# engcang/FAST-LIO-SAM-QN

Hardware: AMD Instinct MI355X
Metric: scan-pair registrations/sec on 100k-pt clouds (higher is better)
Workload: dtype f32 search / f64 accumulate

## Files before the change

fast-lio-sam-qn_amd/csrc/qn_batch.inc:

```

namespace {

template <class F> void lanes_launch(const void* tab, dim3 grid, hipStream_t s, uint32_t shmem) {
  hipLaunchKernelGGL(HIP_KERNEL_NAME(k_lanes<F>), grid, dim3(F::TB), shmem, s, (const LaneEntry<typename F::Args>*)tab);
}
template <class A> void lane_push(std::vector<LaneEntry<A>>& v, const A& a, uint32_t nbx) {
  LaneEntry<A> e; memset((void*)&e, 0, sizeof(e)); e.a = a; e.nbx = nbx; v.push_back(e);
}

struct LanePlan {
  qn_ctx* c; size_t off = 0; bool overflow = false; int flush_rc = QN_OK;
  struct Item { void (*fn)(const void*, dim3, hipStream_t, uint32_t); size_t off; dim3 grid; int family; uint32_t shmem; };
  std::vector<Item> items;
  explicit LanePlan(qn_ctx* c_) : c(c_) {}
  template <class F> void add(const std::vector<LaneEntry<typename F::Args>>& e, int family, uint32_t shmem = 0) {
    if (e.empty()) return;
    const size_t bytes = sizeof(LaneEntry<typename F::Args>) * e.size();
    const size_t a = reserve(bytes);
    if (a == SIZE_MAX) return;
    put<F>(e, a, family, shmem);
  }
  template <class F, class Fix> void add(std::vector<LaneEntry<typename F::Args>>& e, int family, const void* blob, size_t blob_bytes, Fix fix) {
    if (e.empty()) return;
    const size_t head = (blob_bytes + 255) & ~(size_t)255, bytes = head + sizeof(LaneEntry<typename F::Args>) * e.size();
// ... 53 lines not shown

int lane_set_cloud(qn_ctx* c, int which, const float* xyz, uint32_t n, uint32_t stride, bool on_device, hipStream_t s, GridLaunch* out) {
  CloudBuf& b = c->cloud[which];
  b.n = 0; b.has_grid = b.has_cov = false;
  if (n == 0) return QN_ERR_EMPTY_CLOUD;
  if (!xyz || stride < 12 || (stride & 3)) return QN_ERR_INVALID_ARG;
  if (n > c->max_points) return QN_ERR_CAPACITY;
  const char* dsrc = (const char*)xyz;
  if (!on_device) { const int rc = upload_host_cloud(c, xyz, n, stride, s, &dsrc); if (rc != QN_OK) return rc; }
  b.n = n;
  *out = prep_grid(c, b, dsrc, stride, true);
  return QN_OK;
}

bool batch_supported(const qn_ctx* c) {
  const qn_gicp_params& p = c->params;
  const int maxit = p.force_iterations > 0 ? p.force_iterations : p.max_iterations;
  return c->batch_lanes >= 2 && !c->lanes_failed && maxit > 0 && c->fused_ticks && c->fused_final && c->far_enabled && c->knn_hist && !c->verify_track && !c->clk_probe && !c->list_probe &&
         c->tick_tb == 512 && c->tick_occ >= 4 && !c->dbg_counters;
}

int lane_args_arena(qn_ctx* c) {
  if (c->args_h) return QN_OK;
  c->args_cap = (size_t)4 << 20;
  HIPCHK(c, hipHostMalloc(&c->args_h, c->args_cap, hipHostMallocDefault));
  HIPCHK(c, hipMalloc(&c->args_d, c->args_cap));
  return QN_OK;
}

int batch_ensure_lanes(qn_ctx* c) {
  HIPCHK(c, hipSetDevice(c->device));
  const int B = std::max(1, std::min(c->batch_lanes, 64));
  if (c->lanes.empty()) c->lanes.push_back(c);
  while ((int)c->lanes.size() < B) {
    qn_ctx* l = nullptr;
    const int rc = (c->fail_lane_create > 0 && (int)c->lanes.size() >= c->fail_lane_create) ? QN_ERR_HIP : ctx_create(c->device, c->max_points, c->stream, &l);
    if (rc != QN_OK) {
      c->last_error = "batch: lane context creation failed (lanes need batch_lanes x the context's device memory)";
      while (c->lanes.size() > 1) { qn_ctx_destroy(c->lanes.back()); c->lanes.pop_back(); }
      (void)hipGetLastError();
      c->lanes_failed = true;
      return rc;
    }
    c->lanes.push_back(l);
  }
  { const int rc = lane_args_arena(c); if (rc != QN_OK) return rc; }
  for (qn_ctx* l : c->lanes) {
    if (l == c) continue;
    if (l->params.k_correspondences != c->params.k_correspondences) l->cloud[0].has_cov = l->cloud[1].has_cov = false;
    l->params = c->params;
    l->cell_override = c->cell_override; l->margin_nn = c->margin_nn; l->margin_nn_t0 = c->margin_nn_t0; l->margin_knn = c->margin_knn; l->big_blocks0 = c->big_blocks0; l->fb_blocks0 = c->fb_blocks0;
    l->big_ratio = c->big_ratio; l->nn_rounds = c->nn_rounds; l->knn_rounds = c->knn_rounds; l->knn_trips = c->knn_trips; l->knn_mm = c->knn_mm; l->knn_single_all = c->knn_single_all; l->bbox_blocks = c->bbox_blocks; l->stable_cells = c->stable_cells;
    l->unseeded_cap = c->unseeded_cap; l->track_from_tick = c->track_from_tick; l->fused_from_tick = c->fused_from_tick; l->ticks_per_chunk = c->ticks_per_chunk; l->far_chunk = c->far_chunk; l->far_group = c->far_group; l->far_ranked = c->far_ranked;
    l->list_small = c->list_small; l->tick_ppt_min = c->tick_ppt_min; l->tick_rpb = c->tick_rpb; l->nn_lane = c->nn_lane;
  }
  return QN_OK;
}

int batch_register(qn_ctx* owner, const qn_pair_desc* pairs, const uint32_t* idx, uint32_t m, double thr, qn_gicp_result* results, int* valid, int* status,
                   std::vector<const float*>& last_src, std::vector<uint64_t>& last_key, const float* guesses16) {
  hipStream_t s = owner->stream;
  const auto t_call = std::chrono::steady_clock::now();
  const qn_gicp_params& p = owner->params;
  const int k = p.k_correspondences;
  LanePlan plan(owner);
  std::vector<LaneRun> L(m);
  struct AliasGuard {
    std::vector<LaneRun>& L; std::vector<CloudBuf> saved; std::vector<double*> saved_nrm; std::vector<const float*>& last_src;
    AliasGuard(std::vector<LaneRun>& L_, std::vector<const float*>& ls) : L(L_), saved(L_.size()), saved_nrm(L_.size(), nullptr), last_src(ls) {}
    void borrow(size_t l, qn_ctx* from) { qn_ctx* c = L[l].c; saved[l] = c->cloud[0]; saved_nrm[l] = c->nrm_s_sorted; c->cloud[0] = from->cloud[0]; c->nrm_s_sorted = from->nrm_s_sorted; }
    ~AliasGuard() { for (size_t l = 0; l < L.size(); l++) if (L[l].alias >= 0 && saved_nrm[l]) { qn_ctx* c = L[l].c; c->cloud[0] = saved[l]; c->nrm_s_sorted = saved_nrm[l]; c->cloud[0].has_grid = c->cloud[0].has_cov = false; c->cloud[0].n = 0; c->cloud[0].knn_tab = nullptr; last_src[l] = nullptr; } }
  } alias_guard(L, last_src);
  struct FailGuard { std::vector<LaneRun>& L; int* status; bool armed = true; ~FailGuard() { if (armed) for (const LaneRun& R : L) if (R.active) status[R.pair] = QN_ERR_HIP; } } fail_guard{L, status};
  std::vector<LaneEntry<PackBBoxK::Args>> v_pack; std::vector<LaneEntry<CellCountK::Args>> v_count; std::vector<LaneEntry<ScanLookbackK::Args>> v_scan;
  std::vector<LaneEntry<ScatterK::Args>> v_scat; std::vector<LaneEntry<StableCellsK::Args>> v_stab;
  std::vector<LaneEntry<KnnHistArgs>> v_sel, v_lst; std::vector<LaneEntry<KnnSingleK::Args>> v_single; std::vector<LaneEntry<KnnCovArgs>> v_tail; std::vector<LaneEntry<CovFromIdxK::Args>> v_cov;
  auto push_grid = [&](const GridLaunch& G) {
    lane_push(v_pack, G.pack, G.pack_nb); lane_push(v_count, G.count, G.nb); lane_push(v_scan, G.scan, G.scan_nb); lane_push(v_scat, G.scat, G.nb);
    if (G.stable) lane_push(v_stab, G.stab, G.nb);
  };
  auto push_knn = [&](const KnnLaunch& K) {
    lane_push(v_sel, K.sel, K.sel_nb); lane_push(v_lst, K.lst, K.lst_nb); lane_push(v_single, K.single, K.single_nb); lane_push(v_tail, K.tail, K.tail_nb); lane_push(v_cov, K.cov, K.cov_nb);
  };
  for (uint32_t l = 0; l < m; l++) {
    LaneRun& R = L[l]; R.c = owner->lanes[l]; R.pair = idx[l];
    qn_ctx* c = R.c;
    const qn_pair_desc& pd = pairs[R.pair];
    qn_gicp_result* out = &results[R.pair];
    valid[R.pair] = 0; memset(out, 0, sizeof(*out)); out->fitness = DBL_MAX;
    for (int i = 0; i < 4; i++) { out->T[5 * i] = 1.f; out->T64[5 * i] = 1.0; }
    c->pair_pipeline = false; c->persist_batch_off = true; c->tgt_pending = false; c->tgt_on_stream2 = false;
    const uint64_t key = ((uint64_t)pd.ns << 32) ^ ((uint64_t)pd.stride_bytes << 1) ^ (uint64_t)(pd.on_device ? 1 : 0);
    R.build_source = !(owner->batch_share_source && last_src[l] == pd.src && last_key[l] == key && pd.src != nullptr && c->cloud[0].has_grid && c->cloud[0].has_cov && c->cloud[0].n == pd.ns);
    if (R.build_source && owner->batch_share_source && pd.src != nullptr && pd.ns > 0) {
      for (uint32_t j = 0; j < l; j++) {
        const qn_pair_desc& pj = pairs[L[j].pair];
        if (L[j].active && L[j].alias < 0 && pj.src == pd.src && pj.ns == pd.ns && pj.stride_bytes == pd.stride_bytes && pj.on_device == pd.on_device) { R.alias = (int)j; break; }
      }
      if (R.alias >= 0) { alias_guard.borrow(l, L[R.alias].c); R.build_source = false; }
    }
    int rc = QN_OK; GridLaunch gs, gt;
    if (R.build_source) { last_src[l] = nullptr; rc = lane_set_cloud(c, QN_SOURCE, pd.src, pd.ns, pd.stride_bytes, pd.on_device != 0, s, &gs); }
    if (rc == QN_OK) { ScratchSwap sw(c); rc = lane_set_cloud(c, QN_TARGET, pd.dst, pd.nt, pd.stride_bytes, pd.on_device != 0, s, &gt); }
    if (rc == QN_ERR_HIP) return rc;
    status[R.pair] = rc;
    if (rc != QN_OK) {
      if (R.build_source) { c->cloud[0].has_grid = c->cloud[0].has_cov = false; c->cloud[0].n = 0; }
// ... 14 lines not shown
    else { plan.add<KnnHistK<false, 48, false>>(v_sel, QN_K_KNN_SELECT); plan.add<KnnHistK<true, 48, false>>(v_lst, QN_K_KNN_COV); }
  }
  plan.add<KnnSingleK>(v_single, QN_K_KNN_COV);
  if (k <= 16) plan.add<KnnCovK<16, true, 4>>(v_tail, QN_K_KNN_COV); else if (k <= 20) plan.add<KnnCovK<20, true, 4>>(v_tail, QN_K_KNN_COV); else if (k <= 24) plan.add<KnnCovK<24, true, 4>>(v_tail, QN_K_KNN_COV); else plan.add<KnnCovK<32, true, 4>>(v_tail, QN_K_KNN_COV);
  plan.add<CovFromIdxK>(v_cov, QN_K_KNN_COV);

  const int per_outer = p.optimizer == QN_OPT_LM ? 2 : 1;
  const int maxit = p.force_iterations > 0 ? p.force_iterations : p.max_iterations;
  const int fixed_unseeded = std::max(1, std::min(owner->track_from_tick, owner->fused_from_tick)) * per_outer;
  const bool exact_ticks = p.force_iterations > 0 && p.optimizer == QN_OPT_GN;
  {
    std::vector<LaneEntry<InitStateK::Args>> v_init; std::vector<float> g16;
    for (LaneRun& R : L) {
      if (!R.active) continue;
      qn_ctx* c = R.c;
      c->gen = 0; c->part_rows = 0; c->far_mode = 2; c->clear_far_now = true; c->unseeded_until = fixed_unseeded; c->count_far_now = false;
      c->result_host->phase = 0;
      R.ticks_left = exact_ticks ? maxit : 1 << 30;
      R.chunk = std::min(fixed_unseeded, R.ticks_left); R.chunk_start = 0; R.next = R.chunk; R.first_chunk = true;
      R.budget = (long)maxit * (p.optimizer == QN_OPT_LM ? (p.lm_max_iterations + 1) : 1) + 2;
      lane_push(v_init, InitStateK::Args{st_cur(c), c->guess_tmp, guesses16 ? 1 : 0, 0, c->far_stats}, 1u);
      if (guesses16) g16.insert(g16.end(), guesses16 + 16 * (size_t)R.pair, guesses16 + 16 * (size_t)R.pair + 16);
    }
    if (!guesses16) plan.add<InitStateK>(v_init, QN_K_SOLVE);
    else
      plan.add<InitStateK>(v_init, QN_K_SOLVE, g16.data(), sizeof(float) * g16.size(), [](std::vector<LaneEntry<InitStateK::Args>>& e, const char* d) {
        for (size_t j = 0; j < e.size(); j++) e[j].a.guess = (const float*)(d + sizeof(float) * 16 * j);
      });
  }
  auto finish_lane = [&](LaneRun& R, int rc) {
    qn_ctx* c = R.c;
    R.active = false;
    status[R.pair] = rc;
    if (rc != QN_OK) return;
    results[R.pair] = c->result_host->r;
    c->trace_len = c->result_host->trace_len; c->aligned_valid = true;
    valid[R.pair] = (results[R.pair].converged && results[R.pair].fitness < thr) ? 1 : 0;
  };
  struct ProfFlush { qn_ctx* c; ~ProfFlush() { c->prof_collect(); } } prof_flush{owner};
  int tick_no = 0;
  for (;;) {
    int stop = 1 << 30; bool any = false;
    for (const LaneRun& R : L) if (R.active) { any = true; stop = std::min(stop, R.next); }
    if (!any) break;
    for (; tick_no < stop; tick_no++) {
      {
        std::vector<LaneEntry<NnSearchArgs>> v_g, v_l; std::vector<LaneEntry<AccumulateK::Args>> v_acc;
        bool group = true, lane = true;
        for (LaneRun& R : L) {
          if (!R.active || tick_no >= R.c->unseeded_until) continue;
          qn_ctx* c = R.c;
          const int t = tick_no - R.chunk_start;
          c->count_far_now = R.first_chunk && (t / per_outer == (R.chunk - 1) / per_outer);
          const NnLaunch N = prep_nn(c, 0, c->sqd, false, tick_no / per_outer, 0);
          group = group && N.group; lane = lane && N.lane;
          lane_push(v_g, N.grid, N.grid_nb); lane_push(v_l, N.list, N.list_nb);
          const uint32_t nb = acc_blocks(c);
          lane_push(v_acc, prep_accumulate(c, 0, true), nb);
          c->count_far_now = false;
        }
        if (lane) plan.add<NnLaneK<0>>(v_g, QN_K_NN_SEARCH); else plan.add<NnSearchK<0, false, QN_NN_BLOCK>>(v_g, QN_K_NN_SEARCH);
        if (group) plan.add<NnSearchK<0, true, QN_BLOCK, true>>(v_l, QN_K_NN_FALLBACK); else plan.add<NnSearchK<0, true, QN_BLOCK>>(v_l, QN_K_NN_FALLBACK);
        plan.add<AccumulateK>(v_acc, QN_K_ACCUMULATE);
      }
      {
        std::vector<LaneEntry<TickArgs>> v_t; std::vector<LaneEntry<FarArgs>> v_f; std::vector<LaneEntry<FarReduceK::Args>> v_r;
        for (LaneRun& R : L) {
          if (!R.active || tick_no < R.c->unseeded_until) continue;
          qn_ctx* c = R.c;
          const TickArgs a = tick_args(c);
          lane_push(v_t, a, tick_blocks(c));
          if (a.far_mode == 1) { lane_push(v_f, far_args(c), (uint32_t)QN_FAR_BLOCKS); lane_push(v_r, far_reduce_args(c), 1u); }
          c->gen++; c->part_rows = -1;
        }
        plan.add<TickK<512, 4, 0, false>>(v_t, QN_K_GN_TICK_FUSED, (uint32_t)owner->tick_lds_pad); plan.add<FarK>(v_f, QN_K_FAR); plan.add<FarReduceK>(v_r, QN_K_FAR);
      }
    }
    {
      std::vector<LaneEntry<FinalizeK::Args>> v_fin; std::vector<LaneEntry<TickArgs>> v_close; std::vector<LaneEntry<FinalizeFitK::Args>> v_fit;
      for (LaneRun& R : L) {
        if (!R.active || R.next != stop) continue;
        qn_ctx* c = R.c;
        if (exact_ticks && R.ticks_left > R.chunk) lane_push(v_fin, FinalizeK::Args{st_cur(c), c->result_host, c->far_stats}, 1u);
        else {
          const TickArgs a = tick_args(c, 1);
          const uint32_t nb = tick_blocks(c);
          lane_push(v_close, a, nb);
          lane_push(v_fit, FinalizeFitK::Args{st_cur(c), c->result_host, c->far_stats, c->fit_psum, c->fit_pcnt, (int)tick_rows(c)}, 1u);
        }
      }
      plan.add<FinalizeK>(v_fin, QN_K_SOLVE); plan.add<TickK<512, 4, 1, false>>(v_close, QN_K_FITNESS); plan.add<FinalizeFitK>(v_fit, QN_K_FITNESS);
    }
    const auto tt0 = std::chrono::steady_clock::now();
    int rc = plan.run();
    if (rc != QN_OK) return rc;
    const auto tt1 = std::chrono::steady_clock::now();
    HIPCHK(owner, hipStreamSynchronize(s));
    if (owner->batch_trace) { const auto tt2 = std::chrono::steady_clock::now();
      fprintf(stderr, "qn batch %p: segment to tick %d  prep+enqueue %.0f us  sync %.0f us  (since call %.0f us)\n", (void*)owner, stop, std::chrono::duration<double, std::micro>(tt1 - tt0).count(),
              std::chrono::duration<double, std::micro>(tt2 - tt1).count(), std::chrono::duration<double, std::micro>(tt2 - t_call).count()); }
    for (LaneRun& R : L) {
      if (!R.active || R.next != stop) continue;
      qn_ctx* c = R.c;
      if (R.first_chunk && (rc = clouds_valid(c)) != QN_OK) { last_src[&R - &L[0]] = nullptr; finish_lane(R, rc); continue; }
      R.budget -= std::max(R.chunk, 1); R.ticks_left -= R.chunk;
      if (c->result_host->phase == 2) { finish_lane(R, QN_OK); continue; }
      if (R.budget <= 0) { c->last_error = "align: device state machine did not terminate"; owner->last_error = c->last_error; finish_lane(R, QN_ERR_HIP); continue; }
// ... 60 lines not shown
```

fast-lio-sam-qn_amd/csrc/qn_context.h:

```cpp
#pragma once
#include <hip/hip_runtime.h>
#include <string>
#include <vector>
#include "qn_gicp_kernels.cuh"

struct CloudBuf {
  uint32_t n = 0, ncells = 0;
  bool has_grid = false, has_cov = false;
  float4* raw = nullptr;
  float4* sorted = nullptr;
  float4* sorted_tmp = nullptr;
  uint32_t* cell_of_pt = nullptr;
  uint32_t* cell_start = nullptr;
  uint32_t* counts = nullptr;
  double* nrm = nullptr;
  qn::GridView grid{};
  qn::GridDims* dims = nullptr;
  qn::GridDims* dims_host = nullptr;
  const int32_t* knn_tab = nullptr; int knn_k = 0;
};

struct ProfSpan { int family; hipEvent_t a, b; int count; };

struct qn_ctx {
  int device = 0;
  uint32_t max_points = 0, max_cells = 0;
  hipStream_t stream = nullptr; bool owns_stream = true;
  std::vector<qn_ctx*> lanes; int batch_lanes = 8; char* args_h = nullptr; char* args_d = nullptr; size_t args_cap = 0; uint64_t batch_launches = 0, batch_pairs = 0; bool is_lane = false, batch_trace = false, batch_share_source = true;
  bool lanes_failed = false; int fail_lane_create = 0;
  void* slab = nullptr;
  qn_gicp_params params{};
  CloudBuf cloud[2];
  qn::BBoxAcc* bbox_acc = nullptr; qn::BBoxAcc* bbox_acc2 = nullptr;
  unsigned long long* scan_status = nullptr; unsigned long long* scan_status2 = nullptr; uint32_t build_epoch = 0;
  int far_group = -1;
  int far_chunk = 2;
  bool batch_look = false;
  bool far_ranked = true;
  unsigned long long* list_probe = nullptr;
  bool device_look = true;
  bool clear_far_now = false;
  char* staging2 = nullptr;
  struct PinZone { char* h = nullptr; hipEvent_t ev = nullptr; bool busy = false; } pin_up, pin_up2;
  char* staging = nullptr;
  uint32_t* scan_sums = nullptr;

  qn::GicpState* state = nullptr;
  uint32_t gen = 0; int part_rows = 0;
  double* partials = nullptr;
  uint32_t* tail_ticket = nullptr;
  double* fit_psum = nullptr; uint32_t* fit_pcnt = nullptr;
  qn_iter_trace* trace = nullptr; uint32_t trace_len = 0;
  int32_t* corr = nullptr; int32_t* nn_idx = nullptr; int32_t* knn_idx = nullptr; float4* nn_ref = nullptr; double* nrm_s_sorted = nullptr; qn::TargetRec* tgt_rec = nullptr; float* sqd = nullptr; float* sqd_fit = nullptr;
  int32_t* far_cand = nullptr; float4* far_cand_ref = nullptr; float2* far_cand_b = nullptr; unsigned long long* far_req = nullptr; uint32_t* far_stats = nullptr; double* far_rows = nullptr; int far_mode = 2; bool far_enabled = true;
  uint2* fb_list = nullptr; uint2* big_list = nullptr; uint32_t* fb_count2 = nullptr;
  float4* aligned = nullptr; bool aligned_valid = false;
  double* pose_tmp = nullptr; float* guess_tmp = nullptr;
  qn::ResultBlock* result_host = nullptr; double* scalar_host = nullptr;
  int32_t* dbg_knn_idx = nullptr; float* dbg_knn_d2 = nullptr;
  qn_quatro_params qparams{}; bool qparams_set = false, q_ready = false; double q_last_scale = 1.0;
  float4* q_normals[2] = {nullptr, nullptr}; float* q_spfh[2] = {nullptr, nullptr}; float* q_fpfh_s[2] = {nullptr, nullptr}; float* q_fpfh[2] = {nullptr, nullptr};
  unsigned long long* q_key[2] = {nullptr, nullptr};
  float* q_pair[2] = {nullptr, nullptr}; uint32_t* q_pair_hash[2] = {nullptr, nullptr};
  uint32_t* q_hit = nullptr; uint32_t* q_list = nullptr; uint32_t* q_sel = nullptr; uint2* q_pairs = nullptr; uint32_t* q_counts = nullptr; double* q_T = nullptr;
  void* q_mm_c = nullptr; void* q_mm_q = nullptr; float* q_mm_qn = nullptr; uint32_t* q_mm_L = nullptr; unsigned long long* q_mm_table = nullptr; unsigned long long* q_mm_table_q = nullptr; bool feat_query_dedupe = false;
  uint32_t q_mm_mask = 0;
  uint2* q_mm_pairs = nullptr; uint32_t* q_mm_cnt = nullptr; uint32_t q_mm_cap = 0, q_mm_ncnt = 0; bool feat_mfma = true, feat_mm_retry = false; int feat_sample = 4 ; bool feat_verify = false; int feat_min_blocks = 1536; double q_wall_ms[3] = {0, 0, 0}; unsigned long long* q_mm_vkeys = nullptr; uint32_t* q_mm_vcnt = nullptr; uint32_t feat_fallbacks = 0, feat_survivors = 0;
  bool c2f_overlap = false;
  bool c2f_lanes_fpfh = false;
  bool tgt_early = true;
  bool quatro_fused = true;
  int normals_fg = 0, fpfh_fg = 0;
  float4* c2f_src = nullptr; float4* c2f_dst = nullptr;
  float* q_mean = nullptr; double* q_mean_psum = nullptr; void* q_host = nullptr;
  double cell_override = 0.0;
  int list_small = 6000;
  float big_ratio = 2.5f;
  bool fused_ticks = true;
  int nn_rounds = 1;
  int nn_lane = -1;
  int track_from_tick = 3;
  int fused_from_tick = 3;
  int unseeded_until = 3; bool count_far_now = false; int last_extra_unseeded = 0;
  int unseeded_cap = 10;
  int single_from_tick = 2;
  bool fused_final = true;
  int knn_rounds = 2;
  int knn_mm = 1;
  int knn_trips = 3;
  int knn_hist = 1;
  int big_blocks0 = 4096, fb_blocks0 = 512;
  float margin_nn_t0 = 0.f;
  float margin_nn = 1.f, margin_knn = 0.f;
  int margin_nn_cap = 3, margin_knn_cap = 5, ticks_per_chunk = 8; bool knn_single_all = false, stable_cells = true; int bbox_blocks = 64;
  hipStream_t stream2 = nullptr; hipEvent_t ev_pair = nullptr; bool pair_pipeline = true, pair_failed = false, tgt_on_stream2 = false, tgt_pending = false, no_pipe = false;
  uint32_t* scan_sums2 = nullptr; uint2* fb_list2 = nullptr; uint2* big_list2 = nullptr; uint32_t* fb_count2b = nullptr; int32_t* knn_idx2 = nullptr;
  uint32_t tick_ppt_min = 1;
  uint32_t tick_rpb = 2;
  uint32_t tick_tb = 512;
  int batch_min_share = 4;
  int knn_lds_pad = 0;
  int tick_lds_pad = 0;
  int tick_occ = 4;
  unsigned long long* pg_rows = nullptr; unsigned long long* pg_bc = nullptr; unsigned long long* pg_fit = nullptr; uint32_t* pg_status = nullptr; uint32_t* pg_status_host = nullptr;
  unsigned long long* pg_clk = nullptr; uint32_t pg_epoch = 0; bool prof_persist = false, persist = true, persist_batch_off = false, persist_fits = true; int persist_resident_blocks = 0; uint32_t persist_launches = 0, persist_gave_up = 0; unsigned long long persist_timeout = 25000000ull;
  uint32_t* dbg_counters = nullptr;
  unsigned long long* clk_probe = nullptr; uint32_t clk_n = 0;
  bool verify_track = false; int32_t* v_corr = nullptr; int32_t* v_nn_idx = nullptr; float* v_sqd = nullptr; float4* v_nn_ref = nullptr; uint32_t* v_counters = nullptr;
  bool prof_on = false, prof_open = false; int prof_depth = 0;
  std::vector<ProfSpan> spans;
  qn_kernel_stat stats[QN_K_COUNT] = {};
  std::string last_error;

  void set_error(const char* what, hipError_t e, int line);
  void prof_begin(int family, int count = 1); void prof_end(); void prof_collect();
  int quatro_normals_width() const { const int g = normals_fg > 0 ? normals_fg : 8; return g >= 16 ? 16 : (g >= 8 ? 8 : 1); }
  int quatro_fpfh_width() const { const int g = fpfh_fg > 0 ? fpfh_fg : 8; return g >= 16 ? 16 : 8; }
};
```

fast-lio-sam-qn_amd/csrc/qn_device.cuh:

```cuda
#pragma once
#include <hip/hip_runtime.h>
#include <stdint.h>
#include "qn_eig3.cuh"
#include "qn_step_math.cuh"

namespace qn {

#define QN_TX 8
#define QN_TY 4
#define QN_TZ 4
#define QN_TILE_CELLS 128

struct GridDims {
  float ox, oy, oz, cell, inv_cell, eps;
  int nx, ny, nz, ntx, nty, ntz;
  uint32_t n;
  uint32_t ncells, nonfinite, pad;
};
struct GridView {
  const float4* pts;
  const uint32_t* cell_start;
  uint32_t* dbg;
  float ox, oy, oz, cell, inv_cell, eps;
  int nx, ny, nz;
  int ntx, nty, ntz;
  uint32_t n;
  const GridDims* dims;
};
__device__ __forceinline__ int uni(int v) { return __builtin_amdgcn_readfirstlane(v); }
__device__ __forceinline__ uint32_t uni(uint32_t v) { return (uint32_t)__builtin_amdgcn_readfirstlane((int)v); }
__device__ __forceinline__ float uni(float v) { return __int_as_float(__builtin_amdgcn_readfirstlane(__float_as_int(v))); }
__device__ __forceinline__ double uni(double v) { union { double d; int i[2]; } u; u.d = v; u.i[0] = __builtin_amdgcn_readfirstlane(u.i[0]); u.i[1] = __builtin_amdgcn_readfirstlane(u.i[1]); return u.d; }
__device__ __forceinline__ GridView grid_resolve(GridView g) {
  const GridDims d = *g.dims;
  g.ox = uni(d.ox); g.oy = uni(d.oy); g.oz = uni(d.oz); g.cell = uni(d.cell); g.inv_cell = uni(d.inv_cell); g.eps = uni(d.eps);
  g.nx = uni(d.nx); g.ny = uni(d.ny); g.nz = uni(d.nz); g.ntx = uni(d.ntx); g.nty = uni(d.nty); g.ntz = uni(d.ntz); g.n = uni(d.n);
  return g;
}

template <class A> struct alignas(16) LaneEntry { A a; uint32_t nbx; uint32_t pad_[3]; };
template <class F>
__global__ void __launch_bounds__(F::TB, F::OCC) k_lanes(const LaneEntry<typename F::Args>* __restrict__ tab) {
  const LaneEntry<typename F::Args>* e = tab + blockIdx.y;
  const uint32_t nbx = e->nbx;
  if (blockIdx.x >= nbx) return;
  F::run(e->a, blockIdx.x, nbx);
}

#define QN_INF_KEY 0xFFFFFFFFFFFFFFFFull

__device__ __forceinline__ int clampi(int v, int lo, int hi) { return v < lo ? lo : (v > hi ? hi : v); }
__device__ __forceinline__ int cell_coord(float v, float o, float inv, int n) {
  return clampi((int)floorf((v - o) * inv), 0, n - 1);
}
__device__ __forceinline__ uint32_t cell_key(const GridView& g, int x, int y, int z) {
  const uint32_t tile = ((uint32_t)(z >> 2) * g.nty + (y >> 2)) * g.ntx + (x >> 3);
  return (tile << 7) | ((z & 3) << 5) | ((y & 3) << 3) | (x & 7);
}
__device__ __forceinline__ unsigned long long pack_key(float d2, uint32_t idx) {
  return ((unsigned long long)__float_as_uint(d2) << 32) | idx;
}
__device__ __forceinline__ float key_d2(unsigned long long k) { return __uint_as_float((uint32_t)(k >> 32)); }
__device__ __forceinline__ uint32_t key_idx(unsigned long long k) { return (uint32_t)k; }

typedef float qn_f2 __attribute__((ext_vector_type(2)));
__device__ __forceinline__ float sqdist(float qx, float qy, float qz, float px, float py, float pz) {
  const qn_f2 q = {qx, qy}, p = {px, py};
  const qn_f2 d = q - p;
  const qn_f2 d2 = d * d;
  const float dz = qz - pz;
  return (d2.x + d2.y) + dz * dz;
}

__device__ __forceinline__ int rfl(int v) { return __builtin_amdgcn_readfirstlane(v); }
__device__ __forceinline__ uint32_t rflu(uint32_t v) { return (uint32_t)__builtin_amdgcn_readfirstlane((int)v); }
// ... 227 lines not shown
  __device__ __forceinline__ void consider(bool on, float d2, uint32_t idx) {
    const unsigned long long key = pack_key(d2, idx);
    if (on && key < w) { pend[cnt][threadIdx.x & 63] = key; cnt++; }
    if (__any(cnt == QN_PEND_CAP)) flush();
  }
  __device__ __forceinline__ void merge_from(int lane_xor, bool recv) {
    if (KMAX > 24) {
      unsigned long long tmp[KMAX];
#pragma unroll
      for (int j = 0; j < KMAX; j++) tmp[j] = __shfl_xor(a[j], lane_xor);
#pragma unroll 1
      for (int j = 0; j < KMAX; j++) {
        unsigned long long other = QN_INF_KEY;
#pragma unroll
        for (int u = 0; u < KMAX; u++) other = (u == j) ? tmp[u] : other;
        if (__any(j >= KMAX - k)) insert((recv && j >= KMAX - k) ? other : QN_INF_KEY);
      }
      return;
    }
#pragma unroll
    for (int j = 0; j < KMAX; j++) {
      const unsigned long long other = __shfl_xor(a[j], lane_xor);
      if (__any(j >= KMAX - k)) insert((recv && j >= KMAX - k) ? other : QN_INF_KEY);
    }
  }
  template <int S>
  __device__ __forceinline__ void finish(bool on) {
    if (__any(cnt > 0)) flush();
    if (S == 1) return;
    const int lane = threadIdx.x & 63;
    merge_from(32, on && (lane & 32) == 0);
    if (S == 4) merge_from(16, on && (lane & 48) == 0);
    refresh();
    const unsigned long long w0 = __shfl(w, lane & (64 / S - 1));
    if (on) w = w0;
  }
  __device__ __forceinline__ bool full() const { return w != QN_INF_KEY; }
  __device__ __forceinline__ float worst_d2() const { return key_d2(w); }
  __device__ __forceinline__ int found() const {
    int f = 0;
#pragma unroll
    for (int j = 0; j < KMAX; j++) f += (j >= KMAX - k && a[j] != QN_INF_KEY) ? 1 : 0;
    return f;
  }
  __device__ __forceinline__ int wanted() const { return k; }
};

__device__ __forceinline__ float tile_box_d2(const GridView& g, int tx, int ty, int tz, float qx, float qy, float qz) {
  const float xl = g.ox + (float)(tx << 3) * g.cell, xh = g.ox + (float)min((tx << 3) + 8, g.nx) * g.cell;
  const float yl = g.oy + (float)(ty << 2) * g.cell, yh = g.oy + (float)min((ty << 2) + 4, g.ny) * g.cell;
  const float zl = g.oz + (float)(tz << 2) * g.cell, zh = g.oz + (float)min((tz << 2) + 4, g.nz) * g.cell;
  const float dx = fmaxf(fmaxf(xl - qx, qx - xh) - g.eps, 0.f), dy = fmaxf(fmaxf(yl - qy, qy - yh) - g.eps, 0.f), dz = fmaxf(fmaxf(zl - qz, qz - zh) - g.eps, 0.f);
  return ((dx * dx + dy * dy) + dz * dz) * 0.999998f;
}

__device__ __forceinline__ void divmod_small(int n, int d, int& q, int& r) {
  q = (int)((float)n * __builtin_amdgcn_rcpf((float)d));
  r = n - q * d;
  if (r < 0) { q--; r += d; }
  if (r >= d) { q++; r -= d; }
}

template <class Body>
__device__ __forceinline__ uint32_t stream_box(const GridView& g, int x0, int x1, int y0, int y1, int z0, int z1, const bool tile_mode, WaveLds* lds, Body&& body,
                                               const float bqx = 0.f, const float bqy = 0.f, const float bqz = 0.f, const float ball_r2 = -1.f) {
  const int lane = threadIdx.x & 63;
  const int tx0 = x0 >> 3, ntr = (x1 >> 3) - tx0 + 1, nyr = y1 - y0 + 1;
  const int ty0 = y0 >> 2, ntyr = (y1 >> 2) - ty0 + 1;
  const int nseg = tile_mode ? ntr * ntyr * ((z1 >> 2) - (z0 >> 2) + 1) : ntr * nyr * (z1 - z0 + 1);
  uint32_t grand = 0;
  for (int sb = 0; sb < nseg; sb += 64) {
    const int sidx = sb + lane;
    uint32_t s = 0, len = 0;
    if (sidx < nseg) {
      int t, r; divmod_small(sidx, ntr, r, t);
      if (tile_mode) {
        int qz_, ry_; divmod_small(r, ntyr, qz_, ry_);
        const int tzz = (z0 >> 2) + qz_, tyy = ty0 + ry_, txx = tx0 + t;
        const uint32_t tile = ((uint32_t)tzz * g.nty + tyy) * g.ntx + txx;
        if (!(ball_r2 >= 0.f && tile_box_d2(g, txx, tyy, tzz, bqx, bqy, bqz) > ball_r2)) { s = g.cell_start[tile << 7]; len = g.cell_start[(tile + 1) << 7] - s; }
      } else {
        int qz_, ry_; divmod_small(r, nyr, qz_, ry_);
        const int ry = y0 + ry_, rz = z0 + qz_, tx = tx0 + t;
        const int xa = max(x0, tx << 3), xb = min(x1, (tx << 3) + 7);
        const uint32_t k0 = cell_key(g, xa, ry, rz);
        s = g.cell_start[k0]; len = g.cell_start[k0 + (xb - xa) + 1] - s;
      }
    }
    const uint32_t incl = wave_incl_scan_u32(len, lane);
    const uint32_t total = rdlane(incl, 63);
    if (total == 0) continue;
    wave_lds_fence();
    lds->seg_excl[lane] = incl - len; lds->seg_start[lane] = s;
    wave_lds_fence();
    for (uint32_t cb = 0; cb < total; cb += 64) {
      const uint32_t slot = cb + lane;
      const bool valid = slot < total;
      const int j = chunk_segment(lds->tile_cid, cb, incl - len, incl);
      float4 p = make_float4(0.f, 0.f, 0.f, 0.f);
      if (valid) p = g.pts[lds->seg_start[j] + (slot - lds->seg_excl[j])];
      body(p, valid, min(64u, total - cb));
    }
    grand += total;
  }
  return grand;
}

#define QN_CL_DX 8
#define QN_CL_DY 4
#define QN_CL_DZ 4

template <int S>
__device__ __forceinline__ void build_clusters(const GridView& g, WaveLds* lds, unsigned long long todo, int cx, int cy, int cz,
                                               float qx, float qy, float qz, float r, uint32_t& cid, int& ncl, uint32_t& nseg_all) {
  const int lane = threadIdx.x & 63;
  const bool mine = (todo >> lane) & 1ull;
  cid = 0xffffffffu; ncl = 0;
  for (unsigned long long rem = todo; rem != 0; ncl++) {
    const int leader = __ffsll((long long)rem) - 1;
    const int ax = rdlane(cx, leader), ay = rdlane(cy, leader), az = rdlane(cz, leader);
    const bool in = ((rem >> lane) & 1ull) && abs(cx - ax) <= QN_CL_DX && abs(cy - ay) <= QN_CL_DY && abs(cz - az) <= QN_CL_DZ;
    if (in) cid = ncl;
    rem &= ~__ballot(in);
  }
  wave_lds_fence();
  if (lane < ncl) { lds->box[lane][0] = 0x3fffffff; lds->box[lane][1] = -1; lds->box[lane][2] = 0x3fffffff; lds->box[lane][3] = -1; lds->box[lane][4] = 0x3fffffff; lds->box[lane][5] = -1; }
  wave_lds_fence();
  if (mine && lane < 64 / S) {
    atomicMin(&lds->box[cid][0], cell_coord(qx - r, g.ox, g.inv_cell, g.nx)); atomicMax(&lds->box[cid][1], cell_coord(qx + r, g.ox, g.inv_cell, g.nx));
    atomicMin(&lds->box[cid][2], cell_coord(qy - r, g.oy, g.inv_cell, g.ny)); atomicMax(&lds->box[cid][3], cell_coord(qy + r, g.oy, g.inv_cell, g.ny));
    atomicMin(&lds->box[cid][4], cell_coord(qz - r, g.oz, g.inv_cell, g.nz)); atomicMax(&lds->box[cid][5], cell_coord(qz + r, g.oz, g.inv_cell, g.nz));
  }
  wave_lds_fence();
// ... 112 lines not shown
      const int* b = lds->box[cid];
      const int ex0 = b[0], ex1 = b[1], ey0 = b[2], ey1 = b[3], ez0 = b[4], ez1 = b[5];
      const float INF = __int_as_float(0x7f800000);
      float d = INF;
      if (ex0 > 0) d = fminf(d, qx - (g.ox + ex0 * g.cell));
      if (ex1 < g.nx - 1) d = fminf(d, (g.ox + (ex1 + 1) * g.cell) - qx);
      if (ey0 > 0) d = fminf(d, qy - (g.oy + ey0 * g.cell));
      if (ey1 < g.ny - 1) d = fminf(d, (g.oy + (ey1 + 1) * g.cell) - qy);
      if (ez0 > 0) d = fminf(d, qz - (g.oz + ez0 * g.cell));
      if (ez1 < g.nz - 1) d = fminf(d, (g.oz + (ez1 + 1) * g.cell) - qz);
      if (d == INF || !(r == r)) { certified = true; d_unseen = INF; }
      else { d -= g.eps; d_unseen = d; certified = d > 0.f && sink.full() && sink.worst_d2() < d * d; }
      if (!certified) {
        if (sink.full()) r = fmaxf(sqrtf(sink.worst_d2()) * 1.000001f + g.eps, r + g.eps);
        else {
          const int f = sink.found();
          r = f > 0 ? fmaxf(r * sqrtf((float)sink.wanted() / (float)f) * 1.25f, r + g.cell) : 2.f * r + g.cell;
        }
        r = fminf(r, r_cap);
        if (round + 1 < max_rounds) { retry = true; sink.reset(); }
      }
    }
    todo = __ballot(retry);
    if (g.dbg && lane == 0 && todo) atomicAdd(&g.dbg[3], (uint32_t)__popcll(todo));
  }
  return certified;
}

struct CapBox {
  float o2[3];
  float S;
};
__device__ __forceinline__ CapBox cap_of(const GridView& g, float qx, float qy, float qz) {
  CapBox c;
  const float ox = fmaxf(fmaxf(g.ox - qx, qx - (g.ox + g.nx * g.cell)), 0.f);
  const float oy = fmaxf(fmaxf(g.oy - qy, qy - (g.oy + g.ny * g.cell)), 0.f);
  const float oz = fmaxf(fmaxf(g.oz - qz, qz - (g.oz + g.nz * g.cell)), 0.f);
  c.o2[0] = ox * ox; c.o2[1] = oy * oy; c.o2[2] = oz * oz; c.S = (c.o2[0] + c.o2[1]) + c.o2[2];
  return c;
}
__device__ __forceinline__ float cap_extent(const GridView& g, const CapBox& c, float r, int axis) {
  const float rest = c.S - c.o2[axis];
  if (rest <= 0.f) return r;
  const float v = r * r - rest * 0.999999f;
  return v > 0.f ? sqrtf(v) * 1.000001f + g.eps : g.eps;
}
__device__ __forceinline__ float cap_face_dist(const CapBox& c, float f, int axis) {
  const float rest = (c.S - c.o2[axis]) * 0.999999f;
  return rest > 0.f ? sqrtf(f * f + rest) * 0.999999f : f;
}

struct SingleStats { uint32_t rounds, cand, segs; float r_first, r_last; };
__device__ __forceinline__ void wave_search_single(const GridView& g, float qx, float qy, float qz, float r, const float r_cap,
                                                   unsigned long long& best_out, float& second_out, float& d_unseen, WaveLds* lds, SingleStats& st_out, const bool stats) {
  const int lane = threadIdx.x & 63;
  const float INF = __int_as_float(0x7f800000);
  const CapBox cap = cap_of(g, qx, qy, qz);
  if (cap.S > 0.f) r = fminf(fmaxf(r, sqrtf(cap.S) + g.cell), fmaxf(r_cap, r));
  if (stats) { st_out.rounds = 0; st_out.cand = 0; st_out.segs = 0; st_out.r_first = r; }
  float done2 = -1.f;
  int ptx0 = 0, ptx1 = -1, pty0 = 0, pty1 = -1, ptz0 = 0, ptz1 = -1;
  unsigned long long best = QN_INF_KEY; float second = INF;
  for (int round = 0;; round++) {
    const float rx = cap_extent(g, cap, r, 0), ry = cap_extent(g, cap, r, 1), rz = cap_extent(g, cap, r, 2);
    int x0 = rfl(cell_coord(qx - rx, g.ox, g.inv_cell, g.nx)), x1 = rfl(cell_coord(qx + rx, g.ox, g.inv_cell, g.nx));
    int y0 = rfl(cell_coord(qy - ry, g.oy, g.inv_cell, g.ny)), y1 = rfl(cell_coord(qy + ry, g.oy, g.inv_cell, g.ny));
    int z0 = rfl(cell_coord(qz - rz, g.oz, g.inv_cell, g.nz)), z1 = rfl(cell_coord(qz + rz, g.oz, g.inv_cell, g.nz));
    const int tx0 = x0 >> 3, ntr = (x1 >> 3) - tx0 + 1;
    int nseg = ntr * (y1 - y0 + 1) * (z1 - z0 + 1);
    const bool tile_mode = nseg > 128;
    int ty0 = 0, ntyr = 1;
    if (tile_mode) {
      x0 = (x0 >> 3) << 3; x1 = min(((x1 >> 3) << 3) + 7, g.nx - 1);
      y0 = (y0 >> 2) << 2; y1 = min(((y1 >> 2) << 2) + 3, g.ny - 1);
      z0 = (z0 >> 2) << 2; z1 = min(((z1 >> 2) << 2) + 3, g.nz - 1);
      ty0 = y0 >> 2; ntyr = (y1 >> 2) - ty0 + 1;
      nseg = ntr * ntyr * ((z1 >> 2) - (z0 >> 2) + 1);
    }
    const int nyr = y1 - y0 + 1;
    if (!tile_mode || done2 < 0.f) { best = QN_INF_KEY; second = INF; done2 = -1.f; }
    const float in2 = r * r * 1.000002f;
    for (int sb = 0; sb < nseg; sb += 64) {
      const int sidx = sb + lane;
      uint32_t s = 0, len = 0;
      if (sidx < nseg) {
        int t, rr; divmod_small(sidx, ntr, rr, t);
        if (tile_mode) {
          int qz_, ry_; divmod_small(rr, ntyr, qz_, ry_);
          const int tzz = (z0 >> 2) + qz_, tyy = ty0 + ry_, txx = tx0 + t;
          const uint32_t tile = ((uint32_t)tzz * g.nty + tyy) * g.ntx + txx;
          const float tb2 = tile_box_d2(g, txx, tyy, tzz, qx, qy, qz);
          const bool seen = tb2 <= done2 && txx >= ptx0 && txx <= ptx1 && tyy >= pty0 && tyy <= pty1 && tzz >= ptz0 && tzz <= ptz1;
          if (!(tb2 > in2) && !seen) { s = g.cell_start[tile << 7]; len = g.cell_start[(tile + 1) << 7] - s; }
        } else {
          int qz_, ry_; divmod_small(rr, nyr, qz_, ry_);
          const int ry = y0 + ry_, rz = z0 + qz_, tx = tx0 + t;
          const int xa = max(x0, tx << 3), xb = min(x1, (tx << 3) + 7);
          const uint32_t k0 = cell_key(g, xa, ry, rz);
          s = g.cell_start[k0]; len = g.cell_start[k0 + (xb - xa) + 1] - s;
        }
      }
      const uint32_t incl = wave_incl_scan_u32(len, lane);
      const uint32_t total = rdlane(incl, 63);
      if (total == 0) continue;
      if (g.dbg && lane == 0) atomicAdd(&g.dbg[11], total);
      if (stats) st_out.cand += total;
      wave_lds_fence();
      lds->seg_excl[lane] = incl - len; lds->seg_start[lane] = s;
      wave_lds_fence();
      for (uint32_t cb = 0; cb < total; cb += 64) {
        const uint32_t slot = cb + lane;
        const int j = chunk_segment(lds->tile_cid, cb, incl - len, incl);
        if (slot < total) {
          const float4 p = g.pts[lds->seg_start[j] + (slot - lds->seg_excl[j])];
          const float d2 = sqdist(qx, qy, qz, p.x, p.y, p.z);
          const unsigned long long k = pack_key(d2, __float_as_uint(p.w));
          if (k < best) { if (best != QN_INF_KEY) second = key_d2(best); best = k; }
          else if (d2 < second) second = d2;
        }
      }
    }
    if (g.dbg && lane == 0) { atomicAdd(&g.dbg[10], 1u); atomicAdd(&g.dbg[12], (uint32_t)nseg); if (round == 0) atomicAdd(&g.dbg[13], 1u); }
    if (stats) { st_out.rounds++; st_out.segs += (uint32_t)nseg; st_out.r_last = r; }
    if (tile_mode) { done2 = in2; ptx0 = tx0; ptx1 = tx0 + ntr - 1; pty0 = ty0; pty1 = ty0 + ntyr - 1; ptz0 = z0 >> 2; ptz1 = z1 >> 2; }
    const unsigned long long b = wave_min_u64(best);
    float c = (best == b) ? second : key_d2(best);
    if (best == QN_INF_KEY) c = INF;
    c = wave_min_f(c);
    float d = INF;
    if (x0 > 0) d = fminf(d, cap_face_dist(cap, qx - (g.ox + x0 * g.cell), 0));
    if (x1 < g.nx - 1) d = fminf(d, cap_face_dist(cap, (g.ox + (x1 + 1) * g.cell) - qx, 0));
    if (y0 > 0) d = fminf(d, cap_face_dist(cap, qy - (g.oy + y0 * g.cell), 1));
    if (y1 < g.ny - 1) d = fminf(d, cap_face_dist(cap, (g.oy + (y1 + 1) * g.cell) - qy, 1));
    if (z0 > 0) d = fminf(d, cap_face_dist(cap, qz - (g.oz + z0 * g.cell), 2));
    if (z1 < g.nz - 1) d = fminf(d, cap_face_dist(cap, (g.oz + (z1 + 1) * g.cell) - qz, 2));
    bool cert;
    if (tile_mode && r == r && round <= 160) d = fminf(d, r * 0.999998f + g.eps);
    if (d == INF || !(r == r) || round > 160) { cert = true; d_unseen = INF; }
    else { d -= g.eps; d_unseen = d; cert = d > 0.f && b != QN_INF_KEY && key_d2(b) < d * d; }
    if (cert) { best_out = b; second_out = c; return; }
    r = (b != QN_INF_KEY) ? fmaxf(sqrtf(key_d2(b)) * 1.000001f + g.eps, r + g.eps) : (r > 6.f * g.cell ? r + (2.f + round) * g.cell : 2.f * r + g.cell);
    r = fminf(r, r_cap);
  }
}

__device__ __forceinline__ void wave_search_single(const GridView& g, float qx, float qy, float qz, float r, const float r_cap,
                                                   unsigned long long& best_out, float& second_out, float& d_unseen, WaveLds* lds) {
  SingleStats none;
  wave_search_single(g, qx, qy, qz, r, r_cap, best_out, second_out, d_unseen, lds, none, false);
}

__device__ __forceinline__ void wave_search_far16(const GridView& g, float qx_in, float qy_in, float qz_in, bool member_in, float r_in,
                                                  unsigned long long& best_out, float& second_out, float& d_unseen_out, WaveLds* lds) {
  const int lane = threadIdx.x & 63;
  const float INF = __int_as_float(0x7f800000);
  const unsigned long long mm = __ballot(member_in) & 0xffffull;
  const int m = __popcll(mm);
  int m2 = 1; while (m2 < m) m2 <<= 1;
  const int S = 64 / m2;
  const int my_rank = __popcll(mm & ((1ull << (lane & 15)) - 1ull));
  wave_lds_fence();
  if (member_in && lane < 16) lds->seg_cid[my_rank] = (uint32_t)lane;
  wave_lds_fence();
  const int rk = lane & (m2 - 1);
  const bool has_q = rk < m;
  const int src_lane = has_q ? (int)lds->seg_cid[rk] : 0;
  const float qx = __shfl(qx_in, src_lane), qy = __shfl(qy_in, src_lane), qz = __shfl(qz_in, src_lane), r = __shfl(r_in, src_lane);
  const uint32_t sub = (uint32_t)(lane / m2);
  const float cqx = 0.5f * (wave_min_f(has_q ? qx : INF) + wave_max_f(has_q ? qx : -INF));
  const float cqy = 0.5f * (wave_min_f(has_q ? qy : INF) + wave_max_f(has_q ? qy : -INF));
  const float cqz = 0.5f * (wave_min_f(has_q ? qz : INF) + wave_max_f(has_q ? qz : -INF));
  const float off = has_q ? sqrtf(sqdist(qx, qy, qz, cqx, cqy, cqz)) * 1.000002f + 1e-30f : 0.f;
  float R = wave_max_f(has_q ? r + off : 0.f);
  const CapBox cap = cap_of(g, cqx, cqy, cqz);
  if (cap.S > 0.f) R = fmaxf(R, sqrtf(cap.S) + g.cell);
  Best1 sink; sink.init();
  bool open = has_q;
  unsigned long long fin_b = QN_INF_KEY; float fin_s = INF, fin_d = INF;
  float done2 = -1.f; int ptx0 = 0, ptx1 = -1, pty0 = 0, pty1 = -1, ptz0 = 0, ptz1 = -1;
  for (int round = 0;; round++) {
    const float rx = cap_extent(g, cap, R, 0), ry = cap_extent(g, cap, R, 1), rz = cap_extent(g, cap, R, 2);
    int x0 = rfl(cell_coord(cqx - rx, g.ox, g.inv_cell, g.nx)), x1 = rfl(cell_coord(cqx + rx, g.ox, g.inv_cell, g.nx));
    int y0 = rfl(cell_coord(cqy - ry, g.oy, g.inv_cell, g.ny)), y1 = rfl(cell_coord(cqy + ry, g.oy, g.inv_cell, g.ny));
    int z0 = rfl(cell_coord(cqz - rz, g.oz, g.inv_cell, g.nz)), z1 = rfl(cell_coord(cqz + rz, g.oz, g.inv_cell, g.nz));
    x0 = (x0 >> 3) << 3; x1 = min(((x1 >> 3) << 3) + 7, g.nx - 1);
    y0 = (y0 >> 2) << 2; y1 = min(((y1 >> 2) << 2) + 3, g.ny - 1);
    z0 = (z0 >> 2) << 2; z1 = min(((z1 >> 2) << 2) + 3, g.nz - 1);
    const int tx0 = x0 >> 3, ntr = (x1 >> 3) - tx0 + 1, ty0 = y0 >> 2, ntyr = (y1 >> 2) - ty0 + 1, tz0 = z0 >> 2;
    const int nseg = ntr * ntyr * ((z1 >> 2) - tz0 + 1);
    const float in2 = R * R * 1.000002f;
    bool left_out = false;
    for (int sb = 0; sb < nseg; sb += 64) {
      const int sidx = sb + lane;
      uint32_t s = 0, len = 0;
      if (sidx < nseg) {
        int t, rr; divmod_small(sidx, ntr, rr, t);
        int qz_, ry_; divmod_small(rr, ntyr, qz_, ry_);
        const int tzz = tz0 + qz_, tyy = ty0 + ry_, txx = tx0 + t;
        const uint32_t tile = ((uint32_t)tzz * g.nty + tyy) * g.ntx + txx;
        const float tb2 = tile_box_d2(g, txx, tyy, tzz, cqx, cqy, cqz);
        const bool seen = tb2 <= done2 && txx >= ptx0 && txx <= ptx1 && tyy >= pty0 && tyy <= pty1 && tzz >= ptz0 && tzz <= ptz1;
        if (tb2 > in2) left_out = true;
        else if (!seen) { s = g.cell_start[tile << 7]; len = g.cell_start[(tile + 1) << 7] - s; }
      }
      const uint32_t incl = wave_incl_scan_u32(len, lane);
      const uint32_t total = rdlane(incl, 63);
      if (total == 0) continue;
      if (g.dbg && lane == 0) atomicAdd(&g.dbg[11], total);
      wave_lds_fence();
      lds->seg_excl[lane] = incl - len; lds->seg_start[lane] = s;
      wave_lds_fence();
      for (uint32_t cb = 0; cb < total; cb += 64) {
        const uint32_t slot = cb + lane;
        const int j = chunk_segment(lds->tile_cid, cb, incl - len, incl);
        const uint32_t cnt = min(64u, total - cb);
        wave_lds_fence();
        if (slot < total) lds->tile[lane] = g.pts[lds->seg_start[j] + (slot - lds->seg_excl[j])];
        wave_lds_fence();
        for (uint32_t c = 0; c < cnt; c += 4u * (uint32_t)S) {
          float4 cp[4]; uint32_t ci[4];
#pragma unroll
          for (int u = 0; u < 4; u++) { ci[u] = c + (uint32_t)(u * S) + sub; cp[u] = lds->tile[ci[u] & 63u]; }
#pragma unroll
          for (int u = 0; u < 4; u++) sink.consider(open && ci[u] < cnt, sqdist(qx, qy, qz, cp[u].x, cp[u].y, cp[u].z), __float_as_uint(cp[u].w));
        }
      }
    }
    if (g.dbg && lane == 0) { atomicAdd(&g.dbg[10], 1u); atomicAdd(&g.dbg[12], (uint32_t)nseg); if (round == 0) atomicAdd(&g.dbg[13], 1u); }
    done2 = in2; ptx0 = tx0; ptx1 = tx0 + ntr - 1; pty0 = ty0; pty1 = ty0 + ntyr - 1; ptz0 = tz0; ptz1 = z1 >> 2;
    const bool everything = !__any(left_out) && x0 == 0 && x1 == g.nx - 1 && y0 == 0 && y1 == g.ny - 1 && z0 == 0 && z1 == g.nz - 1;
    unsigned long long b = sink.key;
    for (int o = m2; o < 64; o <<= 1) { const unsigned long long t = __shfl_xor(b, o); b = t < b ? t : b; }
    float sc = (sink.key == b) ? sink.second : key_d2(sink.key);
    if (sink.key == QN_INF_KEY) sc = INF;
    for (int o = m2; o < 64; o <<= 1) sc = fminf(sc, __shfl_xor(sc, o));
    float need = 0.f;
    if (open) {
      const float d = R * 0.999998f - off - g.eps;
      bool cert;
      if (everything || round > 160 || !(R == R)) { cert = true; fin_d = INF; }
      else { cert = d > 0.f && b != QN_INF_KEY && key_d2(b) < d * d; fin_d = fmaxf(d, 0.f); }
      if (cert) { fin_b = b; fin_s = sc; open = false; }
      else if (b != QN_INF_KEY) need = sqrtf(key_d2(b)) * 1.000002f + 2.f * g.eps + off;
    }
    if (!__any(open)) break;
    const float want = wave_max_f(need);
    const float grown = want > 0.f ? want : (R > 6.f * g.cell ? R + (2.f + round) * g.cell : 2.f * R + g.cell);
    R = fmaxf(grown, R * 1.0001f + g.eps);
  }
  const unsigned long long ob = __shfl(fin_b, my_rank & 63); const float os = __shfl(fin_s, my_rank & 63), od = __shfl(fin_d, my_rank & 63);
  if (member_in) { best_out = ob; second_out = os; d_unseen_out = od; }
}

template <int KMAX>
__device__ __forceinline__ void lane_ball_knn(const GridView& g, float qx, float qy, float qz, float r, BestK<KMAX>& sink) {
  for (int round = 0;; round++) {
    sink.reset();
    const int bx0 = cell_coord(qx - r, g.ox, g.inv_cell, g.nx), bx1 = cell_coord(qx + r, g.ox, g.inv_cell, g.nx);
    const int by0 = cell_coord(qy - r, g.oy, g.inv_cell, g.ny), by1 = cell_coord(qy + r, g.oy, g.inv_cell, g.ny);
    const int bz0 = cell_coord(qz - r, g.oz, g.inv_cell, g.nz), bz1 = cell_coord(qz + r, g.oz, g.inv_cell, g.nz);
    const bool all = bx0 == 0 && by0 == 0 && bz0 == 0 && bx1 == g.nx - 1 && by1 == g.ny - 1 && bz1 == g.nz - 1;
    for (int rz = bz0; rz <= bz1; rz++) for (int ry = by0; ry <= by1; ry++) for (int tx = bx0 >> 3; tx <= (bx1 >> 3); tx++) {
      const int xa = max(bx0, tx << 3), xb = min(bx1, (tx << 3) + 7);
      const uint32_t k0 = cell_key(g, xa, ry, rz);
      const uint32_t s = g.cell_start[k0], e = g.cell_start[k0 + (xb - xa) + 1];
      for (uint32_t i = s; i < e; i++) {
        const float4 p = g.pts[i];
        const unsigned long long key = pack_key(sqdist(qx, qy, qz, p.x, p.y, p.z), __float_as_uint(p.w));
        if (key < sink.w) { sink.insert(key); sink.refresh(); }
      }
    }
    if (all || round > 160) return;
    if (sink.full()) {
      const float bd = sqrtf(sink.worst_d2()) * 1.000001f + g.eps;
      if (bd <= r) return;
      r = bd;
    } else {
      r = 2.f * r + g.cell;
    }
  }
}



}
```

fast-lio-sam-qn_amd/csrc/qn_engine.hip:

```cpp
#include <hip/hip_runtime.h>
#include <cfloat>
#include <cmath>
#include <cstdio>
#include <cstring>
#include <string>
#include <vector>
#include <atomic>
#include <thread>
#include <chrono>
#include "qn_instances.h"
#include "qn_context.h"
#include "qn_selftest.cuh"
#include "qn_pool.h"

using namespace qn;

#define HIPCHK(ctx, call)                                                                 \
  do { hipError_t e_ = (call);                                                            \
       if (e_ != hipSuccess) { (ctx)->set_error(#call, e_, __LINE__); return QN_ERR_HIP; } \
  } while (0)

void qn_ctx::set_error(const char* what, hipError_t e, int line) {
  char buf[512]; snprintf(buf, sizeof(buf), "%s -> %s (qn_engine.hip:%d)", what, hipGetErrorString(e), line);
  last_error = buf;
// ... 2 lines not shown
void qn_ctx::prof_begin(int family, int count) {
  if (!prof_on) return;
  if (prof_open) { prof_depth++; return; }
  ProfSpan sp; sp.family = family; sp.count = count;
  if (hipEventCreate(&sp.a) != hipSuccess) return;
  if (hipEventCreate(&sp.b) != hipSuccess) { hipEventDestroy(sp.a); return; }
  hipEventRecord(sp.a, stream);
  spans.push_back(sp);
  prof_open = true; prof_depth = 0;
}
void qn_ctx::prof_end() {
  if (!prof_on || spans.empty() || !prof_open) return;
  if (prof_depth > 0) { prof_depth--; return; }
  prof_open = false;
  hipEventRecord(spans.back().b, stream);
}
void qn_ctx::prof_collect() {
  for (auto& sp : spans) {
    float ms = 0; if (hipEventSynchronize(sp.b) == hipSuccess && hipEventElapsedTime(&ms, sp.a, sp.b) == hipSuccess) { stats[sp.family].total_ms += ms; stats[sp.family].launches += sp.count; }
    hipEventDestroy(sp.a); hipEventDestroy(sp.b);
  }
  spans.clear(); prof_open = false; prof_depth = 0;
}
struct ProfScope { qn_ctx* c; ProfScope(qn_ctx* c_, int fam) : c(c_) { c->prof_begin(fam); } ~ProfScope() { c->prof_end(); } };

extern "C" const char* qn_status_str(int s) {
  switch (s) {
    case QN_OK: return "ok"; case QN_ERR_INVALID_ARG: return "invalid argument"; case QN_ERR_EMPTY_CLOUD: return "empty cloud";
    case QN_ERR_CAPACITY: return "cloud exceeds context capacity"; case QN_ERR_NOT_READY: return "clouds/covariances not set";
    case QN_ERR_HIP: return "HIP runtime error"; case QN_ERR_NO_DEVICE: return "no gfx950 device (no CPU fallback)";
    case QN_ERR_INTERNAL: return "internal error (a bounded loop left its bound)";
  }
  return "unknown status";
}
extern "C" const char* qn_last_error(const qn_ctx* ctx) { return ctx ? ctx->last_error.c_str() : "null context"; }

extern "C" void qn_gicp_default_params(qn_gicp_params* p) {
  if (!p) return;
  memset(p, 0, sizeof(*p));
  p->k_correspondences = 20; p->max_iterations = 64; p->max_corr_dist = (double)FLT_MAX;
  p->transformation_epsilon = 5e-4; p->rotation_epsilon = 2e-3; p->optimizer = QN_OPT_LM;
  p->lm_max_iterations = 10; p->lm_init_lambda_factor = 1e-9; p->force_iterations = 0;
  p->ransac_iterations = 0; p->ransac_outlier_threshold = 0.05; p->euclidean_fitness_epsilon = -DBL_MAX;
}

struct Slab {
  char* base = nullptr; size_t off = 0, cap = 0;
  template <class T> void take(T*& p, size_t bytes) {
    const size_t a = (off + 255) & ~(size_t)255;
    if (base) p = (T*)(base + a);
    off = a + bytes;
  }
};
static void carve_cloud(qn_ctx* c, Slab& sl, CloudBuf& b) {
  sl.take(b.raw, sizeof(float4) * c->max_points);
  sl.take(b.sorted, sizeof(float4) * c->max_points);
  sl.take(b.sorted_tmp, sizeof(float4) * c->max_points);
  sl.take(b.cell_of_pt, sizeof(uint32_t) * c->max_points);
  sl.take(b.cell_start, sizeof(uint32_t) * ((size_t)c->max_cells + 1));
  sl.take(b.counts, sizeof(uint32_t) * ((size_t)c->max_cells + 1));
  sl.take(b.nrm, sizeof(double) * 3 * c->max_points);
  sl.take(b.dims, sizeof(GridDims));
}

static int ctx_create(int device, uint32_t max_points, hipStream_t shared_stream, qn_ctx** out);
extern "C" int qn_ctx_create(int device, uint32_t max_points, qn_ctx** out) { return ctx_create(device, max_points, nullptr, out); }
static int ctx_create(int device, uint32_t max_points, hipStream_t shared_stream, qn_ctx** out) {
  if (!out || max_points == 0) return QN_ERR_INVALID_ARG;
  *out = nullptr;
  if (max_points > QN_CTX_MAX_POINTS) return QN_ERR_CAPACITY;
  int ndev = 0;
  if (hipGetDeviceCount(&ndev) != hipSuccess || ndev <= 0 || device < 0 || device >= ndev) return QN_ERR_NO_DEVICE;
  qn_ctx* c = new qn_ctx();
  c->device = device; c->max_points = max_points;
  size_t mc = (size_t)max_points * 16; if (mc < (1u << 18)) mc = 1u << 18; if (mc > (1u << 23)) mc = 1u << 23;
  c->max_cells = (uint32_t)mc;
  qn_gicp_default_params(&c->params);
  int rc = QN_OK;
  auto fail = [&](int code) { qn_ctx_destroy(c); return code; };
  if (hipSetDevice(device) != hipSuccess) return fail(QN_ERR_NO_DEVICE);
  if (shared_stream) { c->stream = shared_stream; c->owns_stream = false; c->is_lane = true; }
  else if (hipStreamCreateWithFlags(&c->stream, hipStreamNonBlocking) != hipSuccess) return fail(QN_ERR_HIP);
#define CA(call) if ((call) != hipSuccess) return fail(QN_ERR_HIP)
  auto carve = [&](Slab& sl) {
    carve_cloud(c, sl, c->cloud[0]);
    carve_cloud(c, sl, c->cloud[1]);
    sl.take(c->staging, (size_t)max_points * 32);
    sl.take(c->scan_sums, sizeof(uint32_t) * (c->max_cells / (QN_BLOCK * QN_SCAN_ITEMS) + 2));
    sl.take(c->state, 2 * sizeof(GicpState));
    sl.take(c->partials, 2 * sizeof(double) * (QN_ACC_MAX_BLOCKS + 8) * QN_NPART);
    sl.take(c->nn_idx, sizeof(int32_t) * max_points);
    sl.take(c->knn_idx, sizeof(int32_t) * (size_t)max_points * 32);
    sl.take(c->nn_ref, sizeof(float4) * max_points);
    sl.take(c->nrm_s_sorted, sizeof(double) * 3 * max_points);
    sl.take(c->tgt_rec, sizeof(TargetRec) * max_points);
    sl.take(c->fit_psum, sizeof(double) * (QN_ACC_MAX_BLOCKS + 8));
    sl.take(c->fit_pcnt, sizeof(uint32_t) * (QN_ACC_MAX_BLOCKS + 8));
    sl.take(c->trace, sizeof(qn_iter_trace) * QN_MAX_TRACE);
    sl.take(c->corr, sizeof(int32_t) * max_points);
    sl.take(c->sqd, sizeof(float) * max_points);
    sl.take(c->sqd_fit, sizeof(float) * max_points);
    sl.take(c->far_cand, sizeof(int32_t) * QN_FAR_M * (size_t)max_points);
    sl.take(c->far_cand_ref, sizeof(float4) * max_points);
    sl.take(c->far_cand_b, sizeof(float2) * max_points);
    sl.take(c->far_req, sizeof(unsigned long long) * (max_points / 64 + 2));
    sl.take(c->far_stats, 4 * sizeof(uint32_t));
    sl.take(c->far_rows, sizeof(double) * QN_FAR_BLOCKS * QN_NPART);
    sl.take(c->fb_list, sizeof(uint2) * max_points);
    sl.take(c->big_list, sizeof(uint2) * max_points);
    sl.take(c->fb_count2, 4 * sizeof(uint32_t));
    sl.take(c->aligned, sizeof(float4) * max_points);
    sl.take(c->pose_tmp, sizeof(double) * 16);
    sl.take(c->guess_tmp, sizeof(float) * 16);
    sl.take(c->scan_sums2, sizeof(uint32_t) * (c->max_cells / (QN_BLOCK * QN_SCAN_ITEMS) + 2));
    sl.take(c->fb_list2, sizeof(uint2) * max_points);
    sl.take(c->big_list2, sizeof(uint2) * max_points);
    sl.take(c->fb_count2b, 4 * sizeof(uint32_t));
    sl.take(c->knn_idx2, sizeof(int32_t) * (size_t)max_points * 32);
    sl.take(c->staging2, (size_t)max_points * 32);
    sl.take(c->bbox_acc, 2 * (QN_BBOX_MAX_BLOCKS + 1) * sizeof(BBoxAcc)); c->bbox_acc2 = c->bbox_acc ? c->bbox_acc + (QN_BBOX_MAX_BLOCKS + 1) : nullptr;
    sl.take(c->scan_status, sizeof(unsigned long long) * 2 * (c->max_cells / (QN_BLOCK * QN_SCAN_ITEMS) + 2)); c->scan_status2 = c->scan_status ? c->scan_status + (c->max_cells / (QN_BLOCK * QN_SCAN_ITEMS) + 2) : nullptr;
    sl.take(c->pg_rows, sizeof(unsigned long long) * 3 * QN_PERSIST_ROWS * QN_PERSIST_RSTRIDE);
    sl.take(c->pg_bc, sizeof(unsigned long long) * 64);
    sl.take(c->pg_fit, sizeof(unsigned long long) * (QN_PERSIST_MAX_BLOCKS + 1) * 4);
    sl.take(c->pg_status, 4 * sizeof(uint32_t));
    sl.take(c->tail_ticket, 4 * sizeof(uint32_t));
  };
  { Slab dry; carve(dry);
    Slab sl; sl.cap = (dry.off + ((size_t)2 << 20) - 1) & ~(((size_t)2 << 20) - 1);
    CA(hipMalloc(&c->slab, sl.cap)); sl.base = (char*)c->slab; carve(sl); }
  CA(hipMemsetAsync(c->far_stats, 0, 4 * sizeof(uint32_t), c->stream));
  CA(hipHostMalloc(&c->result_host, sizeof(ResultBlock), hipHostMallocDefault));
  for (int w = 0; w < 2; w++) { CA(hipHostMalloc(&c->cloud[w].dims_host, sizeof(GridDims), hipHostMallocDefault)); memset(c->cloud[w].dims_host, 0, sizeof(GridDims)); }
  CA(hipHostMalloc(&c->scalar_host, 64 * sizeof(double), hipHostMallocDefault));
  CA(hipHostMalloc(&c->pg_status_host, 4 * sizeof(uint32_t), hipHostMallocDefault));
  CA(hipMemsetAsync(c->pg_rows, 0xFF, sizeof(unsigned long long) * 3 * QN_PERSIST_ROWS * QN_PERSIST_RSTRIDE, c->stream));
  CA(hipMemsetAsync(c->pg_bc, 0, sizeof(unsigned long long) * 64, c->stream));
  CA(hipMemsetAsync(c->pg_fit, 0, sizeof(unsigned long long) * (QN_PERSIST_MAX_BLOCKS + 1) * 4, c->stream));
  CA(hipMemsetAsync(c->pg_status, 0, 4 * sizeof(uint32_t), c->stream));
// ... 63 lines not shown
  if (p->k_correspondences < 1 || p->k_correspondences > 32 || p->max_iterations < 0 || p->lm_max_iterations < 1 ||
      (p->optimizer != QN_OPT_LM && p->optimizer != QN_OPT_GN) || !(p->max_corr_dist > 0) || !(p->lm_init_lambda_factor >= 0)) return QN_ERR_INVALID_ARG;
  if (p->k_correspondences != c->params.k_correspondences) { c->cloud[0].has_cov = c->cloud[1].has_cov = false; }
  c->params = *p;
  return QN_OK;
}

extern "C" int qn_gicp_get_params(const qn_ctx* c, qn_gicp_params* p) { if (!c || !p) return QN_ERR_INVALID_ARG; *p = c->params; return QN_OK; }

static GicpConfig make_cfg(const qn_ctx* c) {
  GicpConfig g; const qn_gicp_params& p = c->params;
  g.k = p.k_correspondences; g.max_iterations = p.max_iterations; g.optimizer = p.optimizer; g.lm_max_iterations = p.lm_max_iterations;
  g.force_iterations = p.force_iterations; g.max_corr_dist_sq = p.max_corr_dist * p.max_corr_dist;
  g.transformation_epsilon = p.transformation_epsilon; g.rotation_epsilon = p.rotation_epsilon; g.lm_init_lambda_factor = p.lm_init_lambda_factor;
  return g;
}

static inline GicpState* st_cur(qn_ctx* c) { return c->state + (c->gen & 1u); }
static inline GicpState* st_nxt(qn_ctx* c) { return c->state + ((c->gen + 1u) & 1u); }
static inline double* part_cur(qn_ctx* c) { return c->partials + (size_t)(c->gen & 1u) * (QN_ACC_MAX_BLOCKS + 8) * QN_NPART; }
static inline double* part_nxt(qn_ctx* c) { return c->partials + (size_t)((c->gen + 1u) & 1u) * (QN_ACC_MAX_BLOCKS + 8) * QN_NPART; }

static bool pair_pipeline_ready(qn_ctx* c) {
  if (c->stream2) return true;
  if (c->pair_failed || !c->knn_idx2) return false;
  const bool ok = hipStreamCreateWithFlags(&c->stream2, hipStreamNonBlocking) == hipSuccess && hipEventCreateWithFlags(&c->ev_pair, hipEventDisableTiming) == hipSuccess;
  if (!ok) { c->pair_failed = true; if (c->stream2) { hipStreamDestroy(c->stream2); c->stream2 = nullptr; } (void)hipGetLastError(); }
  return ok;
}
static void swap_scratch(qn_ctx* c) {
  std::swap(c->stream, c->stream2); std::swap(c->scan_sums, c->scan_sums2); std::swap(c->fb_list, c->fb_list2); std::swap(c->big_list, c->big_list2);
  std::swap(c->fb_count2, c->fb_count2b); std::swap(c->knn_idx, c->knn_idx2);
  std::swap(c->bbox_acc, c->bbox_acc2); std::swap(c->scan_status, c->scan_status2);
  std::swap(c->pin_up, c->pin_up2);
  std::swap(c->staging, c->staging2);
}
struct TargetScope {
  qn_ctx* c; bool on;
  TargetScope(qn_ctx* c_, bool on_) : c(c_), on(on_) { if (on) swap_scratch(c); }
  ~TargetScope() { if (on) { (void)hipEventRecord(c->ev_pair, c->stream); swap_scratch(c); c->tgt_pending = true; } }
};
static int join_target(qn_ctx* c) {
  if (!c->tgt_pending) return QN_OK;
  c->tgt_pending = false;
  return hipStreamWaitEvent(c->stream, c->ev_pair, 0) == hipSuccess ? QN_OK : QN_ERR_HIP;
}

struct GridLaunch { PackBBoxK::Args pack; uint32_t pack_nb; CellCountK::Args count; ScanLookbackK::Args scan; uint32_t scan_nb; ScatterK::Args scat; StableCellsK::Args stab; bool stable; uint32_t nb; };
static GridLaunch prep_grid(qn_ctx* c, CloudBuf& b, const char* dsrc, uint32_t stride, bool lanes = false) {
  const uint32_t n = b.n;
  GridView& g = b.grid;
  memset(&g, 0, sizeof(g));
  g.pts = b.sorted; g.cell_start = b.cell_start; g.dbg = c->dbg_counters; g.n = n; g.dims = b.dims;
  GridLaunch L;
  L.nb = (n + QN_BLOCK - 1) / QN_BLOCK;
  L.scan_nb = (c->max_cells + QN_BLOCK * QN_SCAN_ITEMS - 1) / (QN_BLOCK * QN_SCAN_ITEMS);
  if (((++c->build_epoch) & 0x3fffffffu) == 0u) ++c->build_epoch;
  L.pack_nb = std::min<uint32_t>(L.nb, (uint32_t)std::min(lanes ? QN_BBOX_MAX_BLOCKS : c->bbox_blocks, QN_BBOX_MAX_BLOCKS));
  L.pack = PackBBoxK::Args{dsrc, stride, n, b.raw, c->bbox_acc, c->max_cells, c->cell_override, b.dims, b.dims_host};
  L.count = CellCountK::Args{b.raw, n, g, b.counts, b.cell_of_pt};
  L.scan = ScanLookbackK::Args{b.counts, b.dims, b.cell_start, c->scan_status, c->build_epoch, n};
  L.stable = c->stable_cells;
  L.scat = ScatterK::Args{b.raw, n, b.cell_of_pt, b.cell_start, b.counts, L.stable ? b.sorted_tmp : b.sorted};
  L.stab = StableCellsK::Args{b.sorted_tmp, n, b.cell_of_pt, b.cell_start, b.sorted};
  b.has_grid = true; b.has_cov = false; b.knn_tab = nullptr;
  return L;
}
static int build_grid(qn_ctx* c, CloudBuf& b, const char* dsrc, uint32_t stride) {
  hipStream_t s = c->stream;
  const GridLaunch L = prep_grid(c, b, dsrc, stride);
  { ProfScope ps(c, QN_K_GRID_BUILD);
    hipLaunchKernelGGL(k_pack_bbox_dims, dim3(L.pack_nb), dim3(QN_BLOCK), 0, s, L.pack.in, L.pack.stride, L.pack.n, L.pack.raw, L.pack.acc, L.pack.max_cells, L.pack.cell_override, L.pack.dims_dev, L.pack.dims_host);
    hipLaunchKernelGGL(k_cell_count, dim3(L.nb), dim3(QN_BLOCK), 0, s, L.count.pts, L.count.n, L.count.g, L.count.counts, L.count.cell_of_pt);
    hipLaunchKernelGGL(k_scan_lookback, dim3(L.scan_nb), dim3(QN_BLOCK), 0, s, L.scan.in, L.scan.dims, L.scan.out, L.scan.status, L.scan.epoch, L.scan.total);
    hipLaunchKernelGGL(k_scatter, dim3(L.nb), dim3(QN_BLOCK), 0, s, L.scat.pts, L.scat.n, L.scat.cell_of_pt, L.scat.cell_start, L.scat.counts, L.scat.sorted);
    if (L.stable) hipLaunchKernelGGL(k_stable_cells, dim3(L.nb), dim3(QN_BLOCK), 0, s, L.stab.in, L.stab.n, L.stab.cell_of_pt, L.stab.cell_start, L.stab.out); }
  HIPCHK(c, hipGetLastError());
  return QN_OK;
}
static int clouds_valid(qn_ctx* c) {
  for (int w = 0; w < 2; w++)
    if (c->cloud[w].has_grid && c->cloud[w].dims_host && c->cloud[w].dims_host->nonfinite) {
      c->last_error = w == 0 ? "source cloud contains non-finite coordinates (is_dense == false clouds are not supported)" : "target cloud contains non-finite coordinates (is_dense == false clouds are not supported)";
      c->cloud[w].has_grid = c->cloud[w].has_cov = false;
      return QN_ERR_INVALID_ARG;
    }
  return QN_OK;
}

static int upload_host_cloud(qn_ctx* c, const float* xyz, uint32_t n, uint32_t& stride, hipStream_t s, const char** dsrc) {
  hipPointerAttribute_t at;
  const bool pinned = hipPointerGetAttributes(&at, xyz) == hipSuccess && at.type == hipMemoryTypeHost;
  if (!pinned) (void)hipGetLastError();
  if (pinned) {
    if (stride <= 32) { HIPCHK(c, hipMemcpyAsync(c->staging, xyz, (size_t)(n - 1) * stride + 12, hipMemcpyHostToDevice, s)); }
    else { HIPCHK(c, hipMemcpy2DAsync(c->staging, 16, xyz, stride, 16, n, hipMemcpyHostToDevice, s)); stride = 16; }
    *dsrc = (const char*)c->staging;
    return QN_OK;
  }
  qn_ctx::PinZone& z = c->pin_up;
  if (!z.h) { HIPCHK(c, hipHostMalloc((void**)&z.h, (size_t)c->max_points * 16, hipHostMallocDefault)); HIPCHK(c, hipEventCreateWithFlags(&z.ev, hipEventDisableTiming)); }
  if (z.busy) { HIPCHK(c, hipEventSynchronize(z.ev)); z.busy = false; }
  float* o = (float*)z.h; const char* in = (const char*)xyz;
  for (uint32_t i = 0; i < n; i++, in += stride, o += 3) { const float* p = (const float*)in; o[0] = p[0]; o[1] = p[1]; o[2] = p[2]; }
  HIPCHK(c, hipMemcpyAsync(c->staging, z.h, (size_t)n * 12, hipMemcpyHostToDevice, s));
  HIPCHK(c, hipEventRecord(z.ev, s)); z.busy = true;
  stride = 12; *dsrc = (const char*)c->staging;
  return QN_OK;
}

static int set_cloud(qn_ctx* c, int which, const float* xyz, uint32_t n, uint32_t stride, bool on_device) {
  if (!c || (which != 0 && which != 1)) return QN_ERR_INVALID_ARG;
  CloudBuf& b = c->cloud[which];
  b.n = 0; b.has_grid = b.has_cov = false;
  if (n == 0) return QN_ERR_EMPTY_CLOUD;
  if (!xyz || stride < 12 || (stride & 3)) return QN_ERR_INVALID_ARG;
  if (n > c->max_points) return QN_ERR_CAPACITY;
  HIPCHK(c, hipSetDevice(c->device));
  if (which == QN_SOURCE && join_target(c) != QN_OK) return QN_ERR_HIP;
  c->tgt_on_stream2 = which == QN_TARGET ? (c->pair_pipeline && !c->prof_on && !c->no_pipe && c->cloud[0].has_grid && pair_pipeline_ready(c)) : c->tgt_on_stream2;
  TargetScope scope(c, which == QN_TARGET && c->tgt_on_stream2);
  hipStream_t s = c->stream;
  const char* dsrc = (const char*)xyz;
  if (!on_device) { const int rc = upload_host_cloud(c, xyz, n, stride, s, &dsrc); if (rc != QN_OK) return rc; }
  b.n = n;
  return build_grid(c, b, dsrc, stride);
}

extern "C" int qn_gicp_set_source(qn_ctx* c, const float* xyz, uint32_t n, uint32_t stride) { return set_cloud(c, QN_SOURCE, xyz, n, stride, false); }
// ... 45 lines not shown
    const uint32_t nb = (b.n + QN_BLOCK / 4 - 1) / (QN_BLOCK / 4);
    hipLaunchKernelGGL(HIP_KERNEL_NAME(k_knn_cov<KMAX, false, 4>), dim3(nb), dim3(QN_BLOCK), 0, s, b.grid, b.raw, k, r0, 2, b.nrm, kidx, kd2, c->fb_list, c->fb_count2);
  }
  hipLaunchKernelGGL(HIP_KERNEL_NAME(k_knn_cov<KMAX, true, 4>), dim3(std::min<uint32_t>((b.n + 63) / 64, 512)), dim3(QN_BLOCK), 0, s, b.grid, b.raw, k, r0, 64, b.nrm, kidx, kd2, c->fb_list, c->fb_count2);
  const uint32_t nbp = (b.n + QN_BLOCK - 1) / QN_BLOCK;
  hipLaunchKernelGGL(k_cov_from_idx, dim3(nbp), dim3(QN_BLOCK), 0, s, b.raw, b.sorted, b.n, k, kidx, b.nrm,
                     &b == &c->cloud[0] ? c->nrm_s_sorted : (double*)nullptr, &b == &c->cloud[0] ? (TargetRec*)nullptr : c->tgt_rec, c->fb_count2);
}
static void note_knn_table(qn_ctx* c, CloudBuf& b, const int32_t* kidx, int k) {
  for (CloudBuf& o : c->cloud) if (&o != &b && o.knn_tab == kidx) o.knn_tab = nullptr;
  b.knn_tab = kidx; b.knn_k = k;
}
static int compute_cov(qn_ctx* c, int which, int32_t* kidx, float* kd2) {
  if (!c || (which != 0 && which != 1)) return QN_ERR_INVALID_ARG;
  CloudBuf& b = c->cloud[which];
  if (!b.has_grid) return b.n == 0 ? QN_ERR_EMPTY_CLOUD : QN_ERR_NOT_READY;
  HIPCHK(c, hipSetDevice(c->device));
  const int k = c->params.k_correspondences;
  const bool on2 = which == QN_TARGET && c->tgt_on_stream2 && !c->prof_on && kidx == c->knn_idx && c->stream2 != nullptr;
  if (which == QN_TARGET && !on2 && join_target(c) != QN_OK) return QN_ERR_HIP;
  if (on2) kidx = c->knn_idx2;
  TargetScope scope(c, on2);
  if (k <= 16) launch_knn_cov<16>(c, b, k, kidx, kd2);
  else if (k <= 20) launch_knn_cov<20>(c, b, k, kidx, kd2);
  else if (k <= 24) launch_knn_cov<24>(c, b, k, kidx, kd2);
  else launch_knn_cov<32>(c, b, k, kidx, kd2);
  HIPCHK(c, hipGetLastError());
  b.has_cov = true;
  if (kidx == c->knn_idx || kidx == c->knn_idx2) note_knn_table(c, b, kidx, k);
  return QN_OK;
}
extern "C" int qn_gicp_compute_covariances(qn_ctx* c, int which) { return compute_cov(c, which, c->knn_idx, nullptr); }

struct NnLaunch { NnSearchArgs grid; uint32_t grid_nb; NnSearchArgs list; uint32_t list_nb; bool group; bool lane; };
static NnLaunch prep_nn(qn_ctx* c, int mode , float* sqd_out, bool seeded, int tick, int cond) {
  CloudBuf &S = c->cloud[0], &T = c->cloud[1];
  const uint32_t nb = (S.n + QN_NN_BLOCK / 4 - 1) / (QN_NN_BLOCK / 4);
  const uint32_t nb4 = (S.n + QN_BLOCK / 4 - 1) / (QN_BLOCK / 4);
  const double thr2 = c->params.max_corr_dist * c->params.max_corr_dist;
  GicpState* st = st_cur(c);
  uint32_t* fbc = &st->fb_count; uint32_t* bgc = &st->big_count;
  uint32_t* far_stats = (mode == 0 && !seeded && c->count_far_now) ? c->far_stats : nullptr;
  const bool wide = tick <= 2 || (mode == 0 && !seeded);
  int big_blocks = wide ? c->big_blocks0 : 1024;
  const uint32_t fbb = std::min<uint32_t>(nb4, wide ? (uint32_t)c->fb_blocks0 : 256u);
  const float r0 = -(tick == 0 && mode == 0 && c->margin_nn_t0 > 0.f ? c->margin_nn_t0 : c->margin_nn);
  const float big_ratio = c->big_ratio;
  NnOpt opt; opt.clear_ref = (mode == 0 && !seeded && c->clear_far_now) ? c->far_cand_ref : nullptr; opt.cond = cond;
  const bool batch = c->persist_batch_off;
  opt.group = c->far_group >= 0 ? c->far_group : (batch ? 2048 : 0); opt.group_min = 0;
  if (mode == 0 && opt.group > 0) big_blocks = std::min(big_blocks, std::max(64, (opt.group + QN_BLOCK / 64 - 1) / (QN_BLOCK / 64)));
  opt.probe = (mode == 0 && !seeded) ? c->list_probe : nullptr;
  opt.fb_small = (mode == 0 && !c->persist_batch_off) ? (uint32_t)c->list_small : 0u;
  NnOpt opt0; opt0.clear_ref = nullptr; opt0.cond = 0; opt0.group = 0; opt0.group_min = 0; opt0.probe = nullptr; opt0.fb_small = 0;
  c->clear_far_now = mode == 0 && !seeded ? false : c->clear_far_now;
  const NnOpt& o = mode == 0 ? opt : opt0;
  NnLaunch L;
  L.lane = (c->nn_lane > 0 || (c->nn_lane < 0 && c->persist_batch_off)) && mode == 0 && !seeded;
  L.grid_nb = L.lane ? (S.n + 255u) / 256u : nb; L.list_nb = fbb + (uint32_t)big_blocks; L.group = mode == 0 && opt.group > 0;
  L.grid = NnSearchArgs{S.grid, T.grid, st, thr2, r0, mode == 0 ? c->nn_rounds : 1, c->corr, sqd_out, c->nn_idx, c->nn_ref, c->fb_list, fbc, c->big_list, bgc, 0, big_ratio, far_stats, o};
  L.list = NnSearchArgs{S.grid, T.grid, st, thr2, r0, 64, c->corr, sqd_out, c->nn_idx, c->nn_ref, c->fb_list, fbc, c->big_list, bgc, big_blocks, big_ratio, far_stats, o};
  return L;
}
#define QN_NN_ARGS(A) A.src, A.tgt, A.st, A.thr2, A.r0, A.max_rounds, A.corr, A.sqd, A.nn_idx, A.nn_ref, A.fb_list, A.fb_count, A.big_list, A.big_count, A.big_blocks, A.big_ratio, A.far_stats, A.opt
static void enqueue_nn(qn_ctx* c, int mode , float* sqd_out, bool seeded, int tick = 0, int cond = 0) {
  hipStream_t s = c->stream;
  CloudBuf &S = c->cloud[0], &T = c->cloud[1];
  const uint32_t nbt = (S.n + QN_BLOCK - 1) / QN_BLOCK;
  const NnLaunch L = prep_nn(c, mode, sqd_out, seeded, tick, cond);
  if (L.grid.opt.probe) (void)hipMemsetAsync(c->list_probe, 0, sizeof(unsigned long long) * 4 * 16384, s);
  const NnSearchArgs& G = L.grid; const NnSearchArgs& F = L.list;
  if (mode == 0) {
    { ProfScope ps(c, QN_K_NN_SEARCH);
      if (seeded) hipLaunchKernelGGL(HIP_KERNEL_NAME(k_nn_track<0>), dim3(nbt), dim3(QN_BLOCK), 0, s, S.grid, T.grid, T.raw, G.st, G.thr2, c->corr, sqd_out, c->nn_idx, c->nn_ref, c->fb_list, G.fb_count, c->big_list, G.big_count);
      else if (L.lane) hipLaunchKernelGGL(HIP_KERNEL_NAME(k_nn_lane<0>), dim3(L.grid_nb), dim3(256), 0, s, G);
      else hipLaunchKernelGGL(HIP_KERNEL_NAME(k_nn_search<0, false, QN_NN_BLOCK>), dim3(L.grid_nb), dim3(QN_NN_BLOCK), 0, s, QN_NN_ARGS(G)); }
    { ProfScope ps(c, QN_K_NN_FALLBACK);
      if (L.group) hipLaunchKernelGGL(HIP_KERNEL_NAME(k_nn_search<0, true, QN_BLOCK, true>), dim3(L.list_nb), dim3(QN_BLOCK), 0, s, QN_NN_ARGS(F));
      else hipLaunchKernelGGL(HIP_KERNEL_NAME(k_nn_search<0, true, QN_BLOCK>), dim3(L.list_nb), dim3(QN_BLOCK), 0, s, QN_NN_ARGS(F)); }
  } else {
    ProfScope ps(c, QN_K_FITNESS);
    if (seeded) hipLaunchKernelGGL(HIP_KERNEL_NAME(k_nn_track<1>), dim3(nbt), dim3(QN_BLOCK), 0, s, S.grid, T.grid, T.raw, G.st, G.thr2, c->corr, sqd_out, c->nn_idx, c->nn_ref, c->fb_list, G.fb_count, c->big_list, G.big_count);
    else hipLaunchKernelGGL(HIP_KERNEL_NAME(k_nn_search<1, false, QN_NN_BLOCK>), dim3(L.grid_nb), dim3(QN_NN_BLOCK), 0, s, QN_NN_ARGS(G));
    hipLaunchKernelGGL(HIP_KERNEL_NAME(k_nn_search<1, true, QN_BLOCK>), dim3(L.list_nb), dim3(QN_BLOCK), 0, s, QN_NN_ARGS(F));
  }
}
static void enqueue_verify(qn_ctx* c, bool fused) {
  hipStream_t s = c->stream;
  CloudBuf &S = c->cloud[0], &T = c->cloud[1];
  const uint32_t nb = (S.n + QN_NN_BLOCK / 4 - 1) / (QN_NN_BLOCK / 4), nb4 = (S.n + QN_BLOCK / 4 - 1) / (QN_BLOCK / 4);
  const double thr2 = c->params.max_corr_dist * c->params.max_corr_dist;
  GicpState* st = st_cur(c);
  uint32_t* fbc = &st->fb_count; uint32_t* bgc = &st->big_count;
  const float r0 = -c->margin_nn;
  hipLaunchKernelGGL(k_reset_lists, dim3(1), dim3(64), 0, s, st);
  hipLaunchKernelGGL(HIP_KERNEL_NAME(k_nn_search<0, false, QN_NN_BLOCK>), dim3(nb), dim3(QN_NN_BLOCK), 0, s, S.grid, T.grid, st, thr2, r0, c->nn_rounds, c->v_corr, c->v_sqd, c->v_nn_idx, c->v_nn_ref, c->fb_list, fbc, c->big_list, bgc, 0, c->big_ratio, (uint32_t*)nullptr, NnOpt{nullptr, 0, 0, 0, nullptr, 0});
  hipLaunchKernelGGL(HIP_KERNEL_NAME(k_nn_search<0, true, QN_BLOCK>), dim3(std::min<uint32_t>(nb4, 512) + 4096), dim3(QN_BLOCK), 0, s, S.grid, T.grid, st, thr2, r0, 64, c->v_corr, c->v_sqd, c->v_nn_idx, c->v_nn_ref, c->fb_list, fbc, c->big_list, bgc, 4096, c->big_ratio, (uint32_t*)nullptr, NnOpt{nullptr, 0, 0, 0, nullptr, 0});
  hipLaunchKernelGGL(k_verify_nn, dim3((S.n + 255) / 256), dim3(256), 0, s, S.n, st, c->nn_idx, c->v_nn_idx, fused ? (const float*)nullptr : c->sqd, c->v_sqd, c->corr, c->v_corr, c->v_counters);
  hipLaunchKernelGGL(k_reset_lists, dim3(1), dim3(64), 0, s, st);
}
static uint32_t acc_blocks(const qn_ctx* c) { return std::min<uint32_t>((c->cloud[0].n + QN_BLOCK - 1) / QN_BLOCK, QN_ACC_MAX_BLOCKS); }
static uint32_t tick_ppt(const qn_ctx* c) { return std::max<uint32_t>(c->tick_ppt_min, (c->cloud[0].n + c->tick_tb * QN_ACC_MAX_BLOCKS - 1) / (c->tick_tb * QN_ACC_MAX_BLOCKS)); }
static uint32_t tick_rows(const qn_ctx* c) { const uint32_t per = c->tick_tb * tick_ppt(c); return (c->cloud[0].n + per - 1) / per; }
static uint32_t tick_rpb(const qn_ctx* c) { return c->persist_batch_off ? std::max(1u, c->tick_rpb) : 1u; }
static uint32_t tick_blocks(const qn_ctx* c) { const uint32_t rpb = tick_rpb(c); return (tick_rows(c) + rpb - 1) / rpb; }
static TailArgs tail_args(qn_ctx* c, int enabled, int rows, const LookArgs* look = nullptr) {
  TailArgs t; memset(&t, 0, sizeof(t));
// ... 153 lines not shown
  for (int w = 0; w < 2; w++) { if (c->cloud[w].n == 0) return QN_ERR_EMPTY_CLOUD; if (!c->cloud[w].has_grid || !c->cloud[w].has_cov) return QN_ERR_NOT_READY; }
  return QN_OK;
}

static int gicp_align(qn_ctx* c, const float guess[16], qn_gicp_result* out, bool alone);
extern "C" int qn_gicp_align(qn_ctx* c, const float guess[16], qn_gicp_result* out) {
  const bool alone = g_aligns_in_flight.fetch_add(1) == 0;
  int rc = gicp_align(c, guess, out, alone);
  if (rc == QN_INTERNAL_RETRY) rc = gicp_align(c, guess, out, false);
  g_aligns_in_flight.fetch_sub(1);
  return rc;
}
static int gicp_align(qn_ctx* c, const float guess[16], qn_gicp_result* out, bool alone) {
  if (c && join_target(c) != QN_OK) return QN_ERR_HIP;
  int rc = ready(c); if (rc != QN_OK) return rc;
  if (!out) return QN_ERR_INVALID_ARG;
  HIPCHK(c, hipSetDevice(c->device));
  hipStream_t s = c->stream;
  const qn_gicp_params& p = c->params;
  if (guess) HIPCHK(c, hipMemcpyAsync(c->guess_tmp, guess, sizeof(float) * 16, hipMemcpyHostToDevice, s));
  c->gen = 0; c->part_rows = 0;
  c->far_mode = 2;
  const int maxit = p.force_iterations > 0 ? p.force_iterations : p.max_iterations;
  c->clear_far_now = maxit > 0;
  if (maxit == 0) HIPCHK(c, hipMemsetAsync(c->far_cand_ref, 0, sizeof(float4) * c->cloud[0].n, s));
  hipLaunchKernelGGL(k_init_state, dim3(1), dim3(64), 0, s, st_cur(c), c->guess_tmp, guess ? 1 : 0, 0, c->far_stats);
  if (maxit == 0) hipLaunchKernelGGL(k_set_pose, dim3(1), dim3(64), 0, s, st_cur(c), c->pose_tmp, 2, 2);
  const int per_outer = p.optimizer == QN_OPT_LM ? 2 : 1;
  const bool adaptive = (!c->persist_batch_off || (c->device_look && c->batch_look)) && c->fused_ticks && c->far_enabled && c->single_from_tick > 0 && p.force_iterations > 0 && p.optimizer == QN_OPT_GN && maxit >= 8 &&
                        std::min(c->track_from_tick, c->fused_from_tick) > c->single_from_tick;
  const int fixed_unseeded = std::max(1, std::min(c->track_from_tick, c->fused_from_tick)) * per_outer;
  const int unseeded = adaptive ? std::max(1, std::min(fixed_unseeded / per_outer, c->single_from_tick)) * per_outer : fixed_unseeded;
  const bool exact_ticks = p.force_iterations > 0 && p.optimizer == QN_OPT_GN;
  int ticks_left = exact_ticks ? maxit : 1 << 30;
  int chunk = c->far_enabled ? std::min(unseeded, ticks_left) : (exact_ticks ? ticks_left : c->ticks_per_chunk);
  bool first_chunk = true;
  long budget = (long)maxit * (p.optimizer == QN_OPT_LM ? (p.lm_max_iterations + 1) : 1) + 2;
  c->result_host->phase = 0;
  c->unseeded_until = adaptive ? chunk : fixed_unseeded;
  bool seeded = false; int tick_no = 0;
  bool extending = false;
  for (;;) {
    const bool look = adaptive && first_chunk && !extending && ticks_left > chunk;
    const bool dev_look = look && c->device_look && chunk > 0;
    const bool with_persist = dev_look && persist_usable(c, alone);
    LookArgs la; memset(&la, 0, sizeof(la));
    if (dev_look) {
      la.out = c->result_host; la.far_stats = c->far_stats; la.sdims = c->cloud[0].dims; la.tdims = c->cloud[1].dims; la.enabled = 1;
      la.allow_extra = std::min(ticks_left - chunk - 1, per_outer) > 0 ? 1 : 0;
      c->result_host->look = 0;
    }
    for (int t = 0; t < chunk; t++) {
      c->count_far_now = first_chunk && (t / per_outer == (chunk - 1) / per_outer);
      enqueue_tick(c, seeded, tick_no, (dev_look && t == chunk - 1) ? &la : nullptr); tick_no++; seeded = true;
    }
    c->count_far_now = false;
    bool declined = false;
    if (dev_look) {
      c->unseeded_until = tick_no + 1;
      enqueue_nn(c, 0, c->sqd, false, tick_no / per_outer, QN_LOOK_EXTRA);
      LookArgs la2 = la; la2.enabled = 2; la2.allow_extra = 0;
      enqueue_accumulate(c, QN_LOOK_EXTRA, true, c->unseeded_cap > fixed_unseeded / per_outer ? &la2 : nullptr);
      if (with_persist && (rc = launch_persist(c, (uint32_t)(budget - chunk) + 2u, QN_LOOK_GO)) != QN_OK) return rc;
      HIPCHK(c, hipGetLastError());
      HIPCHK(c, hipStreamSynchronize(s));
      if ((rc = clouds_valid(c)) != QN_OK) return rc;
      const int extra = (c->result_host->look & QN_LOOK_EXTRA) ? per_outer : 0;
      c->last_extra_unseeded = extra;
      if (with_persist && c->result_host->phase == 2) break;
      if (with_persist && c->pg_status_host[0] != 5u) { if ((rc = persist_recover(c)) != QN_OK) return rc; return QN_INTERNAL_RETRY; }
      declined = true;
      if (with_persist) { c->gen--; c->persist_launches--; }
      tick_no += extra; budget -= extra; ticks_left -= extra;
      c->unseeded_until = tick_no;
    } else {
    if (look || (exact_ticks && ticks_left > chunk)) {
      hipLaunchKernelGGL(k_finalize, dim3(1), dim3(64), 0, s, st_cur(c), c->result_host, c->far_stats);
    } else {
      enqueue_epilogue(c, DBL_MAX, maxit > 0 && tick_no > 0);
    }
    HIPCHK(c, hipGetLastError());
    HIPCHK(c, hipStreamSynchronize(s));
    if (first_chunk && (rc = clouds_valid(c)) != QN_OK) return rc;
    }
    budget -= std::max(chunk, 1); ticks_left -= chunk;
    if (c->result_host->phase == 2) {
      if (!look) break;
      enqueue_epilogue(c, DBL_MAX, true);
      HIPCHK(c, hipGetLastError());
      HIPCHK(c, hipStreamSynchronize(s));
      if (c->result_host->phase == 2) break;
      c->last_error = "align: closing pass did not complete"; return QN_ERR_HIP;
    }
    if (c->far_enabled) {
      const qn::ResultBlock* rb = c->result_host;
      if (first_chunk) c->far_mode = rb->far_queries * 16u > c->cloud[0].n ? 1 : 2;
      else c->far_mode = (c->far_mode == 1 ? rb->far_requests : rb->far_misses / (uint32_t)std::max(1, chunk)) > 256u ? 1 : 2;
    }
    if (!exact_ticks) chunk = first_chunk ? c->ticks_per_chunk : std::max(2 * per_outer, c->ticks_per_chunk / 2);
    else chunk = c->far_mode == 1 ? std::min(ticks_left, c->far_chunk) : ticks_left;
    if (budget <= 0) { c->last_error = "align: device state machine did not terminate"; return QN_ERR_HIP; }
    if (first_chunk && (!adaptive || declined || extending) && unseeded_goes_on(c, tick_no, per_outer, ticks_left, adaptive)) {
      c->unseeded_until = tick_no + per_outer; chunk = per_outer; extending = true;
      continue;
    }
    if (look && !declined) {
      const GridDims& sg = *c->cloud[0].dims_host;
      double reach2 = 0; const double lo[3] = {sg.ox, sg.oy, sg.oz}, ext[3] = {sg.nx * (double)sg.cell, sg.ny * (double)sg.cell, sg.nz * (double)sg.cell};
      for (int d = 0; d < 3; d++) { const double m = std::max(std::fabs(lo[d]), std::fabs(lo[d] + ext[d])); reach2 += m * m; }
// ... 296 lines not shown
}
extern "C" int qn_debug_set(qn_ctx* c, const char* key, double v) {
  if (!c || !key) return QN_ERR_INVALID_ARG;
  std::string k(key);
  if (k == "cell") { c->cell_override = v; c->cloud[0].has_grid = c->cloud[1].has_grid = false; }
  else if (k == "margin_nn") c->margin_nn = (float)v;
  else if (k == "margin_nn_t0") c->margin_nn_t0 = (float)v;
  else if (k == "big_blocks0") c->big_blocks0 = v < 64 ? 64 : (int)v;
  else if (k == "fb_blocks0") c->fb_blocks0 = v < 64 ? 64 : (int)v;
  else if (k == "margin_knn") c->margin_knn = (float)v;
  else if (k == "knn_single_all") c->knn_single_all = v != 0;
  else if (k == "bbox_blocks") c->bbox_blocks = std::max(1, (int)v);
  else if (k == "device_look") c->device_look = v != 0;
  else if (k == "far_group") c->far_group = (int)v;
  else if (k == "c2f_overlap") c->c2f_overlap = v != 0;
  else if (k == "quatro_fused") c->quatro_fused = v != 0;
  else if (k == "tgt_early") c->tgt_early = v != 0;
  else if (k == "c2f_lanes_fpfh") c->c2f_lanes_fpfh = v != 0;
  else if (k == "normals_fg") c->normals_fg = (int)v;
  else if (k == "fpfh_fg") c->fpfh_fg = (int)v;
  else if (k == "list_small") c->list_small = std::max(0, (int)v);
  else if (k == "far_chunk") c->far_chunk = std::max(1, (int)v);
  else if (k == "far_ranked") c->far_ranked = v != 0;
  else if (k == "batch_look") c->batch_look = v != 0;
  else if (k == "unseeded_cap") c->unseeded_cap = (int)v;
  else if (k == "pair_pipeline") c->pair_pipeline = v != 0;
  else if (k == "persist") c->persist = v != 0;
  else if (k == "persist_timeout") c->persist_timeout = v < 1 ? 1ull : (unsigned long long)v;
  else if (k == "prof_persist") c->prof_persist = v != 0;
  else if (k == "persist_probe") {
    if (v != 0 && !c->pg_clk) { if (hipMalloc(&c->pg_clk, 8 * (64 * 16 + 16)) != hipSuccess) return QN_ERR_HIP; }
    if (c->pg_clk) (void)hipMemset(c->pg_clk, 0, 8 * (64 * 16 + 16));
    if (v == 0) { (void)hipFree(c->pg_clk); c->pg_clk = nullptr; }
  }
  else if (k == "batch_lanes") {
    const int b = std::max(1, std::min((int)v, 64));
    if (b < (int)c->lanes.size()) { if (hipStreamSynchronize(c->stream) != hipSuccess) return QN_ERR_HIP; while ((int)c->lanes.size() > std::max(b, 1)) { qn_ctx* l = c->lanes.back(); c->lanes.pop_back(); if (l != c) qn_ctx_destroy(l); } }
    c->batch_lanes = b; c->lanes_failed = false;
  }
  else if (k == "fail_lane_create") c->fail_lane_create = (int)v;
  else if (k == "batch_share_source") c->batch_share_source = v != 0;
  else if (k == "batch_trace") c->batch_trace = v != 0;
  else if (k == "batch_member") c->persist_batch_off = v != 0;
  else if (k == "stable_cells") c->stable_cells = v != 0;
  else if (k == "knn_hist") c->knn_hist = v != 0;
  else if (k == "nn_rounds") c->nn_rounds = v < 1 ? 1 : (int)v;
  else if (k == "nn_lane") c->nn_lane = v < 0 ? -1 : (v != 0 ? 1 : 0);
  else if (k == "track_from_tick") c->track_from_tick = v < 1 ? 1 : (int)v;
  else if (k == "single_from_tick") c->single_from_tick = v < 1 ? 1 : (int)v;
  else if (k == "fused_from_tick") c->fused_from_tick = v < 1 ? 1 : (int)v;
  else if (k == "knn_rounds") c->knn_rounds = v < 1 ? 1 : (int)v;
  else if (k == "knn_trips") c->knn_trips = v < 1 ? 1 : (int)v;
  else if (k == "knn_mm") c->knn_mm = v != 0;
  else if (k == "fused_ticks") c->fused_ticks = v != 0;
  else if (k == "big_ratio") c->big_ratio = (float)v;
  else if (k == "margin_nn_cap") c->margin_nn_cap = (int)v;
  else if (k == "margin_knn_cap") c->margin_knn_cap = (int)v;
  else if (k == "dbg_counters") {
    if (v != 0 && !c->dbg_counters) { if (hipMalloc(&c->dbg_counters, 16 * sizeof(uint32_t)) != hipSuccess) return QN_ERR_HIP; }
    if (c->dbg_counters) (void)hipMemset(c->dbg_counters, 0, 16 * sizeof(uint32_t));
    if (v == 0) { (void)hipFree(c->dbg_counters); c->dbg_counters = nullptr; }
    for (int w = 0; w < 2; w++) c->cloud[w].grid.dbg = c->dbg_counters;
  }
  else if (k == "ticks_per_chunk") c->ticks_per_chunk = std::max(1, (int)v);
  else if (k == "tick_occ") c->tick_occ = (int)v;
  else if (k == "far") c->far_enabled = v != 0;
  else if (k == "fused_final") c->fused_final = v != 0;
  else if (k == "feat_mfma") c->feat_mfma = v != 0;
  else if (k == "feat_sample") c->feat_sample = (int)v;
  else if (k == "feat_query_dedupe") c->feat_query_dedupe = v != 0;
  else if (k == "feat_min_blocks") c->feat_min_blocks = (int)v;
  else if (k == "feat_verify") { c->feat_verify = v != 0; if (c->q_mm_vcnt) (void)hipMemset(c->q_mm_vcnt, 0, 16); }
  else if (k == "list_probe") {
    if (v != 0 && !c->list_probe) { if (hipMalloc(&c->list_probe, sizeof(unsigned long long) * 4 * 16384) != hipSuccess) return QN_ERR_HIP; }
    if (v == 0 && c->list_probe) { (void)hipFree(c->list_probe); c->list_probe = nullptr; }
  }
  else if (k == "clk_probe") {
    if (v != 0 && !c->clk_probe) { if (hipMalloc(&c->clk_probe, 8 * 8 * 256 + 8 * 12 * 1024) != hipSuccess) return QN_ERR_HIP; }
    if (c->clk_probe) (void)hipMemset(c->clk_probe, 0, 8 * 8 * 256 + 8 * 12 * 1024);
    c->clk_n = 0; if (v == 0) { (void)hipFree(c->clk_probe); c->clk_probe = nullptr; }
  }
  else if (k == "tick_tb") c->tick_tb = v >= 512 ? 512 : 256;
  else if (k == "tick_ppt_min") c->tick_ppt_min = v < 1 ? 1u : (uint32_t)v;
  else if (k == "tick_rpb") c->tick_rpb = v < 1 ? 1u : (uint32_t)v;
  else if (k == "tick_lds_pad") c->tick_lds_pad = v < 0 ? 0 : (int)v;
  else if (k == "knn_lds_pad") c->knn_lds_pad = v < 0 ? 0 : (int)v;
  else if (k == "batch_min_share") c->batch_min_share = v < 1 ? 1 : (int)v;
  else if (k == "verify_track") {
    if (v != 0 && !c->v_counters) {
      const size_t n = c->max_points;
      if (hipMalloc(&c->v_corr, 4 * n) != hipSuccess || hipMalloc(&c->v_nn_idx, 4 * n) != hipSuccess || hipMalloc(&c->v_sqd, 4 * n) != hipSuccess ||
          hipMalloc(&c->v_nn_ref, 16 * n) != hipSuccess || hipMalloc(&c->v_counters, 16) != hipSuccess) return QN_ERR_HIP;
    }
    if (c->v_counters) (void)hipMemset(c->v_counters, 0, 16);
    c->verify_track = v != 0;
  }
  else return QN_ERR_INVALID_ARG;
  return QN_OK;
}
extern "C" int qn_debug_selftest(qn_ctx* c, uint32_t n_waves, uint32_t seed, uint32_t* mismatches) {
  if (!c || !mismatches || n_waves == 0 || n_waves > 65536) return QN_ERR_INVALID_ARG;
  HIPCHK(c, hipSetDevice(c->device));
  std::vector<uint32_t> h((size_t)n_waves * 128);
  uint64_t x = 0x9e3779b97f4a7c15ull ^ seed;
  for (auto& v : h) { x ^= x << 13; x ^= x >> 7; x ^= x << 17; v = (uint32_t)(x >> 16); }
  uint32_t* d = nullptr;
// ... 73 lines not shown
  }
  if (n == 0) return QN_OK;
  HIPCHK(c, hipSetDevice(c->device));
  double* d = nullptr;
  HIPCHK(c, hipMalloc(&d, (n_in + n_out) * sizeof(double)));
  double* d_out = d + n_in;
  int rc = QN_OK;
  if (hipMemcpyAsync(d, in, n_in * sizeof(double), hipMemcpyHostToDevice, c->stream) != hipSuccess || hipMemsetAsync(d_out, 0, n_out * sizeof(double), c->stream) != hipSuccess) rc = QN_ERR_HIP;
  if (rc == QN_OK) {
    if (qn::debug_launch_linearize(which, d, n, arg, d_out, c->stream) != hipSuccess || hipMemcpyAsync(out, d_out, n_out * sizeof(double), hipMemcpyDeviceToHost, c->stream) != hipSuccess ||
        hipStreamSynchronize(c->stream) != hipSuccess) rc = QN_ERR_HIP;
  }
  (void)hipFree(d);
  if (rc != QN_OK) { c->last_error = "debug_linearize: HIP call failed"; return rc; }
  return QN_OK;
}
namespace qn { hipError_t debug_launch_search(int which, const GridView& g, uint32_t ncells, const uint32_t* in, uint32_t n, uint32_t arg, uint32_t* out, hipStream_t stream); }
static bool ds_finite(uint32_t w) { return (w & 0x7f800000u) != 0x7f800000u; }
static float ds_f(uint32_t w) { float f; memcpy(&f, &w, 4); return f; }
static bool kmax_ok(uint32_t km) { return km == 16 || km == 20 || km == 24 || km == 32; }
extern "C" int qn_debug_search(qn_ctx* c, int which, int grid, const void* in_v, uint32_t n, uint32_t arg, void* out_v) {
  if (!c || !in_v || !out_v || which < 0 || which >= QN_DEBUG_SEARCH_WHICH || (grid != 0 && grid != 1)) return QN_ERR_INVALID_ARG;
  const uint32_t* in = static_cast<const uint32_t*>(in_v);
  const bool needs_grid = which != QN_DS_BEST1 && which != QN_DS_DIVMOD;
  GridView g{}; GridDims d{};
  if (needs_grid) {
    CloudBuf& b = c->cloud[grid];
    if (!b.has_grid || !b.dims_host) return QN_ERR_NOT_READY;
    HIPCHK(c, hipSetDevice(c->device));
    if (join_target(c) != QN_OK || hipStreamSynchronize(c->stream) != hipSuccess || (c->stream2 && hipStreamSynchronize(c->stream2) != hipSuccess)) return QN_ERR_HIP;
    d = *b.dims_host;
    if (d.nonfinite || d.n == 0 || d.n != b.n) return QN_ERR_EMPTY_CLOUD;
    if (d.ncells >= (1u << 22) || d.ncells > c->max_cells) return QN_ERR_CAPACITY;
    g = b.grid; g.dbg = nullptr;
  }
  size_t w_in = 0, w_out = 0;
  const uint32_t ncells = d.ncells;
  auto finite_rec = [&](const uint32_t* r, int a, int b_) { for (int i = a; i < b_; i++) if (!ds_finite(r[i])) return false; return true; };
  switch (which) {
    case QN_DS_DUMP:
      if (n != d.n || arg != ncells) return QN_ERR_INVALID_ARG;
      w_in = 0; w_out = (size_t)ncells + 1 + 4 * (size_t)n; break;
    case QN_DS_BEST1: {
      const uint32_t L = arg >> 16, S = arg & 7u;
      if (n == 0 || n > QN_DEBUG_SEARCH_MAX_WAVES || L > QN_DEBUG_SEARCH_MAX_STEPS || (S != 1 && S != 2 && S != 4) || (arg & 0xfef8u)) return QN_ERR_INVALID_ARG;
      w_in = ((size_t)L * 192 + 64) * n; w_out = 256 * (size_t)n; break; }
    case QN_DS_BOUNDS:
      if (n == 0 || n > QN_DEBUG_SEARCH_MAX_QUERIES || arg != 0) return QN_ERR_INVALID_ARG;
      for (uint32_t i = 0; i < n; i++) {
        const uint32_t* r = in + 8 * (size_t)i;
        if (r[0] >= (uint32_t)d.ntx || r[1] >= (uint32_t)d.nty || r[2] >= (uint32_t)d.ntz || !finite_rec(r, 3, 8) || !(ds_f(r[6]) > 0.f)) return QN_ERR_INVALID_ARG;
      }
      w_in = 8 * (size_t)n; w_out = 16 * (size_t)n; break;
    case QN_DS_DIVMOD:
      if (n != 0 || arg != 0) return QN_ERR_INVALID_ARG;
      w_in = 0; w_out = 6; break;
    case QN_DS_STREAM_BOX:
      if (n == 0 || n > QN_DEBUG_SEARCH_MAX_WAVES || arg == 0 || arg > QN_DEBUG_SEARCH_MAX_RECORDED) return QN_ERR_INVALID_ARG;
      for (uint32_t i = 0; i < n; i++) {
        const uint32_t* r = in + 12 * (size_t)i;
        const int x0 = (int)r[0], x1 = (int)r[1], y0 = (int)r[2], y1 = (int)r[3], z0 = (int)r[4], z1 = (int)r[5];
        if (x0 < 0 || x0 > x1 || x1 >= d.nx || y0 < 0 || y0 > y1 || y1 >= d.ny || z0 < 0 || z0 > z1 || z1 >= d.nz || r[6] > 2u || !finite_rec(r, 7, 11)) return QN_ERR_INVALID_ARG;
        if (r[6] != 0u) {
          if ((x0 & 7) || (y0 & 3) || (z0 & 3) || x1 != std::min((x1 | 7), d.nx - 1) || y1 != std::min((y1 | 3), d.ny - 1) || z1 != std::min((z1 | 3), d.nz - 1)) return QN_ERR_INVALID_ARG;
          if (r[6] == 2u && !(ds_f(r[10]) >= 0.f)) return QN_ERR_INVALID_ARG;
        }
      }
      w_in = 12 * (size_t)n; w_out = (4 + (size_t)arg) * n; break;
    case QN_DS_WAVE_SEARCH1:
      if (n == 0 || n > QN_DEBUG_SEARCH_MAX_QUERIES || arg < 1 || arg > 64) return QN_ERR_INVALID_ARG;
      for (uint32_t i = 0; i < n; i++) {
        const uint32_t* r = in + 8 * (size_t)i;
        if (!finite_rec(r, 0, 4) || !(ds_f(r[3]) > 0.f) || !(ds_f(r[4]) > 0.f) || r[4] > 0x7f800000u) return QN_ERR_INVALID_ARG;
      }
      w_in = 8 * (size_t)n; w_out = 8 * (size_t)n; break;
    case QN_DS_WAVE_SEARCH_SINGLE:
      if (n == 0 || n > QN_DEBUG_SEARCH_MAX_QUERIES || arg != 0) return QN_ERR_INVALID_ARG;
      for (uint32_t i = 0; i < n; i++) {
        const uint32_t* r = in + 8 * (size_t)i;
        if (!finite_rec(r, 0, 4) || !(ds_f(r[3]) > 0.f) || r[4] > 0x7f800000u || !(ds_f(r[4]) >= ds_f(r[3]))) return QN_ERR_INVALID_ARG;
      }
      w_in = 8 * (size_t)n; w_out = 8 * (size_t)n; break;
    case QN_DS_WAVE_SEARCH_FAR16:
      if (n == 0 || n > QN_DEBUG_SEARCH_MAX_QUERIES || (n & 15u) || arg != 0) return QN_ERR_INVALID_ARG;
      for (uint32_t i = 0; i < n; i++) {
        const uint32_t* r = in + 8 * (size_t)i;
        if (!finite_rec(r, 0, 4) || !(ds_f(r[3]) > 0.f)) return QN_ERR_INVALID_ARG;
      }
      w_in = 8 * (size_t)n; w_out = 8 * (size_t)n; break;
    case QN_DS_BESTK: {
      const uint32_t KM = arg & 63u, k = (arg >> 8) & 63u, S = (arg >> 14) & 7u, L = arg >> 17;
      if (n == 0 || n > QN_DEBUG_SEARCH_MAX_WAVES || L > QN_DEBUG_SEARCH_MAX_STEPS || !kmax_ok(KM) || k < 1 || k > KM || (S != 1 && S != 4) || (arg & 0xc0u)) return QN_ERR_INVALID_ARG;
      w_in = ((size_t)L * 192 + 64) * n; w_out = 64 * (size_t)(2 * k + 4) * n; break; }
    case QN_DS_WAVE_SEARCH_K: {
      const uint32_t rounds = arg & 255u, KM = (arg >> 8) & 63u, k = (arg >> 16) & 63u;
      if (n == 0 || n > QN_DEBUG_SEARCH_MAX_QUERIES || rounds < 1 || rounds > 64 || !kmax_ok(KM) || k < 1 || k > KM || (arg & 0xffc0c000u)) return QN_ERR_INVALID_ARG;
      for (uint32_t i = 0; i < n; i++) {
        const uint32_t* r = in + 8 * (size_t)i;
        if (!finite_rec(r, 0, 4) || !(ds_f(r[3]) > 0.f) || !(ds_f(r[4]) > 0.f) || r[4] > 0x7f800000u) return QN_ERR_INVALID_ARG;
      }
      w_in = 8 * (size_t)n; w_out = (size_t)(2 * k + 4) * n; break; }
    case QN_DS_STREAM_CLUSTERS: {
      const uint32_t S = arg >> 24, cap = arg & 0xffffffu;
      if (n == 0 || n > QN_DEBUG_SEARCH_MAX_WAVES || (S != 1 && S != 4) || cap == 0 || cap > QN_DEBUG_SEARCH_MAX_RECORDED) return QN_ERR_INVALID_ARG;
      for (size_t i = 0; i < (size_t)n * 64; i++) {
        const uint32_t* r = in + 8 * i;
// ... 113 lines not shown
```

fast-lio-sam-qn_amd/csrc/qn_gicp_kernels.cuh:

```cuda
#pragma once
#include "qn_device.cuh"
#include "qn_step_math.cuh"
#include "qn_linearize.cuh"
#include "qn_knn_hist.cuh"
#include "../../include/qn_engine.h"
#include "qn_util_kernels.cuh"

namespace qn {

#define QN_ACC_MAX_BLOCKS 512
#define QN_MAX_TRACE 1024

struct GicpState {
  double x0[16], xi[16], delta[16];
  double H[36], b[6], d[6];
  double y0, yi, den;
  double lambda, nu;
  double final_H[36];
  double fitness;
  int outer, inner, phase, converged, lm_failed;
  uint32_t fb_count;
  uint32_t trace_len;
  uint32_t big_count;
  int pending;
// ... 70 lines not shown
      raw[i] = p;
      if (!(isfinite(p.x) && isfinite(p.y) && isfinite(p.z))) { bad = 1; continue; }
      const int ox = f2ord(p.x), oy = f2ord(p.y), oz = f2ord(p.z);
      mn[0] = min(mn[0], ox); mn[1] = min(mn[1], oy); mn[2] = min(mn[2], oz);
      mx[0] = max(mx[0], ox); mx[1] = max(mx[1], oy); mx[2] = max(mx[2], oz);
    }
#pragma unroll
    for (int d = 0; d < 3; d++) { mn[d] = wave_min_i(mn[d]); mx[d] = wave_max_i(mx[d]); }
    bad = wave_max_i(bad);
    const int wid = threadIdx.x >> 6;
    if ((threadIdx.x & 63) == 0) { for (int d = 0; d < 3; d++) { smn[wid][d] = mn[d]; smx[wid][d] = mx[d]; } sbad[wid] = bad; }
    __syncthreads();
    __shared__ int s_last;
    if (threadIdx.x == 0) {
      for (int w = 1; w < QN_BLOCK / 64; w++) { for (int d = 0; d < 3; d++) { mn[d] = min(mn[d], smn[w][d]); mx[d] = max(mx[d], smx[w][d]); } bad |= sbad[w]; }
      BBoxAcc* mine = acc + 1 + bx;
      for (int d = 0; d < 3; d++) { __hip_atomic_store(&mine->mn[d], mn[d], __ATOMIC_RELAXED, __HIP_MEMORY_SCOPE_AGENT); __hip_atomic_store(&mine->mx[d], mx[d], __ATOMIC_RELAXED, __HIP_MEMORY_SCOPE_AGENT); }
      __hip_atomic_store(&mine->nonfinite, (uint32_t)bad, __ATOMIC_RELAXED, __HIP_MEMORY_SCOPE_AGENT);
      asm volatile("s_waitcnt vmcnt(0)" ::: "memory");
      s_last = __hip_atomic_fetch_add(&acc->ticket, 1u, __ATOMIC_RELAXED, __HIP_MEMORY_SCOPE_AGENT) == nbx - 1u ? 1 : 0;
    }
    __syncthreads();
    if (!s_last) return;
    if (threadIdx.x >= 64) return;
    for (int d = 0; d < 3; d++) { mn[d] = 0x7fffffff; mx[d] = (int)0x80000000; }
    int nf = 0;
    for (uint32_t b = threadIdx.x; b < nbx; b += 64) {
      const BBoxAcc* o = acc + 1 + b;
      for (int d = 0; d < 3; d++) { mn[d] = min(mn[d], __hip_atomic_load(&o->mn[d], __ATOMIC_RELAXED, __HIP_MEMORY_SCOPE_AGENT)); mx[d] = max(mx[d], __hip_atomic_load(&o->mx[d], __ATOMIC_RELAXED, __HIP_MEMORY_SCOPE_AGENT)); }
      nf |= (int)__hip_atomic_load(&o->nonfinite, __ATOMIC_RELAXED, __HIP_MEMORY_SCOPE_AGENT);
    }
#pragma unroll
    for (int d = 0; d < 3; d++) { mn[d] = wave_min_i(mn[d]); mx[d] = wave_max_i(mx[d]); }
    nf = wave_max_i(nf);
    if (threadIdx.x != 0) return;
    const GridDims g = grid_dims_from_bbox(mn, mx, nf != 0, n, a.max_cells, a.cell_override);
    *a.dims_dev = g; *a.dims_host = g;
    __hip_atomic_store(&acc->ticket, 0u, __ATOMIC_RELAXED, __HIP_MEMORY_SCOPE_AGENT);
  }
};
static __global__ void __launch_bounds__(QN_BLOCK) k_pack_bbox_dims(const char* __restrict__ in, uint32_t stride, uint32_t n, float4* __restrict__ raw, BBoxAcc* acc,
                                                                    uint32_t max_cells, double cell_override, GridDims* __restrict__ dims_dev, GridDims* __restrict__ dims_host) {
  const PackBBoxK::Args a{in, stride, n, raw, acc, max_cells, cell_override, dims_dev, dims_host};
  PackBBoxK::run(a, blockIdx.x, gridDim.x);
}
static __global__ void k_bbox_acc_init(BBoxAcc* acc, int count) {
  for (int i = threadIdx.x; blockIdx.x == 0 && i < count; i += blockDim.x) { BBoxAcc a; for (int d = 0; d < 3; d++) { a.mn[d] = 0x7fffffff; a.mx[d] = (int)0x80000000; } a.nonfinite = 0; a.ticket = 0; acc[i] = a; }
}

#define QN_LB_STATE_AGG 1ull
#define QN_LB_STATE_INC 2ull
struct ScanLookbackK {
  static constexpr int TB = QN_BLOCK, OCC = 1;
  struct Args { const uint32_t* in; const GridDims* dims; uint32_t* out; unsigned long long* status; uint32_t epoch, total; };
  static __device__ __forceinline__ void run(const Args& a, const uint32_t bx, const uint32_t) {
    __shared__ uint32_t wsum[QN_BLOCK / 64];
    __shared__ uint32_t s_prefix;
    const uint32_t* __restrict__ in = a.in; uint32_t* __restrict__ out = a.out; unsigned long long* status = a.status;
    const uint32_t total = a.total;
    const uint32_t m = uni(a.dims->ncells);
    const uint32_t tile = bx;
    if (tile * (uint32_t)(QN_BLOCK * QN_SCAN_ITEMS) >= m) return;
    const uint32_t base = (tile * QN_BLOCK + threadIdx.x) * QN_SCAN_ITEMS;
    uint32_t v[QN_SCAN_ITEMS], s = 0;
    if (base + QN_SCAN_ITEMS <= m) {
      const uint4* q = (const uint4*)(in + base);
#pragma unroll
      for (int j = 0; j < QN_SCAN_ITEMS / 4; j++) { const uint4 x = q[j]; v[4 * j] = x.x; v[4 * j + 1] = x.y; v[4 * j + 2] = x.z; v[4 * j + 3] = x.w; }
    } else {
#pragma unroll
      for (int j = 0; j < QN_SCAN_ITEMS; j++) v[j] = (base + j < m) ? in[base + j] : 0u;
    }
#pragma unroll
    for (int j = 0; j < QN_SCAN_ITEMS; j++) s += v[j];
    uint32_t inc = s;
    const int lane = threadIdx.x & 63, wid = threadIdx.x >> 6;
#pragma unroll
    for (int o = 1; o < 64; o <<= 1) { uint32_t t = __shfl_up(inc, o); if (lane >= o) inc += t; }
    if (lane == 63) wsum[wid] = inc;
    __syncthreads();
    uint32_t woff = 0, agg = 0;
    for (int w = 0; w < QN_BLOCK / 64; w++) { if (w < wid) woff += wsum[w]; agg += wsum[w]; }
    const unsigned long long tag = (unsigned long long)(a.epoch & 0x3fffffffu) << 34;
    if (wid == 0) {
      uint32_t prefix = 0;
      if (tile == 0) {
        if (lane == 0) __hip_atomic_store(status, tag | (QN_LB_STATE_INC << 32) | agg, __ATOMIC_RELAXED, __HIP_MEMORY_SCOPE_AGENT);
      } else {
        if (lane == 0) __hip_atomic_store(status + tile, tag | (QN_LB_STATE_AGG << 32) | agg, __ATOMIC_RELAXED, __HIP_MEMORY_SCOPE_AGENT);
        int look = (int)tile - 1;
        for (;;) {
          const int mine = look - lane;
          unsigned long long x = 0;
          if (mine >= 0) { do { x = __hip_atomic_load(status + mine, __ATOMIC_RELAXED, __HIP_MEMORY_SCOPE_AGENT); } while ((x >> 34) != (tag >> 34)); }
          const bool is_inc = mine >= 0 && ((x >> 32) & 3ull) == QN_LB_STATE_INC;
          const unsigned long long incs = __ballot(is_inc);
          const int first = incs ? __ffsll((long long)incs) - 1 : 64;
          uint32_t part = (mine >= 0 && lane <= first) ? (uint32_t)x : 0u;
#pragma unroll
          for (int o = 32; o > 0; o >>= 1) part += __shfl_xor(part, o);
          prefix += part;
          if (incs || look - 64 < 0) break;
          look -= 64;
        }
        if (lane == 0) __hip_atomic_store(status + tile, tag | (QN_LB_STATE_INC << 32) | (prefix + agg), __ATOMIC_RELAXED, __HIP_MEMORY_SCOPE_AGENT);
      }
      if (lane == 0) s_prefix = prefix;
    }
    __syncthreads();
    uint32_t run = s_prefix + woff + inc - s;
    if (base + QN_SCAN_ITEMS <= m) {
      uint4* q = (uint4*)(out + base);
#pragma unroll
      for (int j = 0; j < QN_SCAN_ITEMS / 4; j++) { uint4 x; x.x = run; run += v[4 * j]; x.y = run; run += v[4 * j + 1]; x.z = run; run += v[4 * j + 2]; x.w = run; run += v[4 * j + 3]; q[j] = x; }
    } else {
#pragma unroll
      for (int j = 0; j < QN_SCAN_ITEMS; j++) { if (base + j < m) out[base + j] = run; run += v[j]; }
    }
    if (base <= m && m < base + QN_SCAN_ITEMS) out[m] = total;
    if (m == (tile + 1u) * (uint32_t)(QN_BLOCK * QN_SCAN_ITEMS) && threadIdx.x == QN_BLOCK - 1) out[m] = total;
  }
};
static __global__ void __launch_bounds__(QN_BLOCK) k_scan_lookback(const uint32_t* __restrict__ in, const GridDims* __restrict__ dims, uint32_t* __restrict__ out,
                                                                   unsigned long long* status, uint32_t epoch, uint32_t total) {
  const ScanLookbackK::Args a{in, dims, out, status, epoch, total};
  ScanLookbackK::run(a, blockIdx.x, gridDim.x);
}

struct ScatterK {
  static constexpr int TB = QN_BLOCK, OCC = 1;
  struct Args { const float4* pts; uint32_t n; const uint32_t* cell_of_pt; const uint32_t* cell_start; uint32_t* counts; float4* sorted; };
  static __device__ __forceinline__ void run(const Args& a, const uint32_t bx, const uint32_t) {
    const uint32_t i = bx * QN_BLOCK + threadIdx.x;
    if (i >= a.n) return;
    const uint32_t c = a.cell_of_pt[i];
    const uint32_t slot = a.cell_start[c] + atomicSub(&a.counts[c], 1u) - 1u;
    float4 p = a.pts[i];
    p.w = __uint_as_float(i);
    a.sorted[slot] = p;
  }
};
static __global__ void __launch_bounds__(QN_BLOCK) k_scatter(const float4* __restrict__ pts, uint32_t n, const uint32_t* __restrict__ cell_of_pt,
                          const uint32_t* __restrict__ cell_start, uint32_t* __restrict__ counts, float4* __restrict__ sorted) {
  const ScatterK::Args a{pts, n, cell_of_pt, cell_start, counts, sorted};
  ScatterK::run(a, blockIdx.x, gridDim.x);
}

struct StableCellsK {
  static constexpr int TB = QN_BLOCK, OCC = 1;
  struct Args { const float4* in; uint32_t n; const uint32_t* cell_of_pt; const uint32_t* cell_start; float4* out; };
  static __device__ __forceinline__ void run(const Args& a, const uint32_t bx, const uint32_t) {
    const float4* __restrict__ in = a.in; float4* __restrict__ out = a.out;
    const uint32_t t = bx * QN_BLOCK + threadIdx.x;
    if (t >= a.n) return;
    const float4 p = in[t];
    const uint32_t i = __float_as_uint(p.w), c = a.cell_of_pt[i];
    const uint32_t s = a.cell_start[c], e = a.cell_start[c + 1];
    if (e - s > 256u) { out[t] = p; return; }
    uint32_t rank = 0;
    for (uint32_t u = s; u < e; u++) rank += __float_as_uint(in[u].w) < i ? 1u : 0u;
    out[s + rank] = p;
  }
};
static __global__ void __launch_bounds__(QN_BLOCK) k_stable_cells(const float4* __restrict__ in, uint32_t n, const uint32_t* __restrict__ cell_of_pt, const uint32_t* __restrict__ cell_start,
                                      float4* __restrict__ out) {
  const StableCellsK::Args a{in, n, cell_of_pt, cell_start, out};
  StableCellsK::run(a, blockIdx.x, gridDim.x);
}

struct __attribute__((aligned(64))) TargetRec { float4 p; double n[3]; double pad[3]; };
static_assert(sizeof(TargetRec) == 64, "TargetRec is one 64-byte line");
#define QN_COV_BATCH 10
#define QN_COV_REG 20
struct CovFromIdxK {
  static constexpr int TB = QN_BLOCK, OCC = 1;
  struct Args { const float4* raw; const float4* sorted; uint32_t n; int k; const int32_t* knn_idx; double* nrm; double* nrm_sorted; TargetRec* rec; uint32_t* list_counts; };
  static __device__ __forceinline__ void run(const Args& a, const uint32_t bx, const uint32_t nbx) {
    const float4* __restrict__ raw = a.raw; const int32_t* __restrict__ knn_idx = a.knn_idx;
    double* __restrict__ nrm = a.nrm; double* __restrict__ nrm_sorted = a.nrm_sorted; TargetRec* __restrict__ rec = a.rec;
    const int k = a.k;
    if (bx == 0 && threadIdx.x < 4) a.list_counts[threadIdx.x] = 0u;
    const uint32_t spos = xcd_block(bx, nbx) * QN_BLOCK + threadIdx.x;
    if (spos >= a.n) return;
    const uint32_t i = __float_as_uint(a.sorted[spos].w);
    const int32_t* nb = knn_idx + (size_t)i * k;
    int found = 0;
    double mean[3] = {0, 0, 0};
    double nv[3] = {0, 0, 0};
    auto store = [&]() __attribute__((always_inline)) {
#pragma unroll
      for (int u = 0; u < 3; u++) nrm[(size_t)i * 3 + u] = nv[u];
      if (nrm_sorted) {
#pragma unroll
        for (int u = 0; u < 3; u++) nrm_sorted[(size_t)spos * 3 + u] = nv[u];
      }
      if (rec) { TargetRec r; r.p = raw[i];
#pragma unroll
        for (int u = 0; u < 3; u++) { r.n[u] = nv[u]; r.pad[u] = 0; }
        rec[i] = r; }
    };
    double c[6] = {0, 0, 0, 0, 0, 0};
    if (k <= QN_COV_REG) {
      int32_t u[QN_COV_REG]; float4 q[QN_COV_REG];
      static_assert(QN_COV_REG % 4 == 0, "the index row is fetched four entries at a time");
      if ((k & 3) == 0) {
        const int4* __restrict__ nb4 = (const int4*)nb;
#pragma unroll
        for (int e = 0; e < QN_COV_REG; e += 4) {
          const int4 v = e < k ? nb4[e >> 2] : make_int4(-1, -1, -1, -1);
          u[e] = v.x; u[e + 1] = v.y; u[e + 2] = v.z; u[e + 3] = v.w;
        }
      } else {
#pragma unroll
        for (int e = 0; e < QN_COV_REG; e++) u[e] = e < k ? nb[e] : -1;
      }
#pragma unroll
      for (int e = 0; e < QN_COV_REG; e++) q[e] = raw[u[e] < 0 ? 0 : u[e]];
#pragma unroll
      for (int e = 0; e < QN_COV_REG; e++) if (u[e] >= 0) { mean[0] += (double)q[e].x; mean[1] += (double)q[e].y; mean[2] += (double)q[e].z; found++; }
// ... 103 lines not shown
  static constexpr int TB = QN_BLOCK, OCC = 1;
  struct Args { GridView g; int k; int32_t* knn_idx; float* knn_d2; const uint2* list; const uint32_t* count; uint2* gen_list; uint32_t* gen_count; };
  static __device__ __forceinline__ void run(const Args& a, const uint32_t bx, const uint32_t nbx) {
    __shared__ WaveLdsH1 lds[QN_BLOCK / 64];
    const GridView g = grid_resolve(a.g);
    const int k = a.k;
    int32_t* __restrict__ knn_idx = a.knn_idx; float* __restrict__ knn_d2 = a.knn_d2; const uint2* __restrict__ list = a.list; uint2* __restrict__ gen_list = a.gen_list; uint32_t* __restrict__ gen_count = a.gen_count;
    WaveLdsH1* my = &lds[threadIdx.x >> 6];
    const uint32_t nq = uni(*a.count);
    if (g.dbg && bx == 0 && threadIdx.x == 0) atomicAdd(&g.dbg[8], nq);
    const uint32_t wave0 = bx * (QN_BLOCK / 64) + (threadIdx.x >> 6), nwaves = nbx * (QN_BLOCK / 64);
    for (uint32_t e = wave0; e < nq; e += nwaves) {
      const uint2 rec = list[e];
      const float4 q = g.pts[rec.x];
      const uint32_t i = __float_as_uint(q.w);
      const int st = wave_knn_single(g, q.x, q.y, q.z, __uint_as_float(rec.y & 0x7fffffffu), k, my, knn_idx + (size_t)i * k, knn_d2 ? knn_d2 + (size_t)i * k : nullptr);
      if (st != 0 && (threadIdx.x & 63) == 0) { if (g.dbg) atomicAdd(&g.dbg[9], 1u); const uint32_t fs = atomicAdd(gen_count, 1u); gen_list[fs] = make_uint2(rec.x, rec.y & 0x7fffffffu); }
    }
  }
};
static __global__ void __launch_bounds__(QN_BLOCK) k_knn_single(GridView g, int k, int32_t* __restrict__ knn_idx, float* __restrict__ knn_d2,
                                                                const uint2* __restrict__ list, const uint32_t* __restrict__ count, uint2* __restrict__ gen_list, uint32_t* __restrict__ gen_count) {
  const KnnSingleK::Args a{g, k, knn_idx, knn_d2, list, count, gen_list, gen_count};
  KnnSingleK::run(a, blockIdx.x, gridDim.x);
}

template <int MODE>
__device__ __forceinline__ void xform_query(const float Tf[12], float x, float y, float z, float& qx, float& qy, float& qz) {
  if (MODE == 0) {
    qx = ((Tf[0] * x + Tf[1] * y) + Tf[2] * z) + Tf[3];
    qy = ((Tf[4] * x + Tf[5] * y) + Tf[6] * z) + Tf[7];
    qz = ((Tf[8] * x + Tf[9] * y) + Tf[10] * z) + Tf[11];
  } else {
    qx = Tf[0] * x + (Tf[1] * y + (Tf[2] * z + Tf[3]));
    qy = Tf[4] * x + (Tf[5] * y + (Tf[6] * z + Tf[7]));
    qz = Tf[8] * x + (Tf[9] * y + (Tf[10] * z + Tf[11]));
  }
}

__device__ __forceinline__ uint32_t late(uint32_t v) { asm volatile("" : "+v"(v)); return v; }
template <int MODE>
__device__ __forceinline__ void store_nn(unsigned long long key, uint32_t i, uint32_t t, double thr2, int32_t* __restrict__ corr, float* __restrict__ sqd, int32_t* __restrict__ nn_idx) {
  const float d2 = key_d2(key);
  if (MODE == 0) nn_idx[t] = key != QN_INF_KEY ? (int32_t)key_idx(key) : -1;
  if (MODE == 0) {
    const bool found = key != QN_INF_KEY;
    sqd[i] = found ? d2 : 0.f;
    corr[i] = (found && (double)d2 < thr2) ? (int32_t)key_idx(key) : -1;
  } else {
    sqd[i] = key != QN_INF_KEY ? d2 : __int_as_float(0x7f800000);
  }
}

struct NnOpt { float4* clear_ref; int cond; int group, group_min; unsigned long long* probe; uint32_t fb_small; };
struct NnSearchArgs { GridView src, tgt; const GicpState* st; double thr2; float r0; int max_rounds; int32_t* corr; float* sqd; int32_t* nn_idx; float4* nn_ref;
                      uint2* fb_list; uint32_t* fb_count; uint2* big_list; uint32_t* big_count; int big_blocks; float big_ratio; uint32_t* far_stats; NnOpt opt; };
template <int MODE, bool LIST, int BLOCK, bool GROUP = false>
struct NnSearchK {
  static constexpr int TB = BLOCK, OCC = GROUP ? 5 : 6;
  using Args = NnSearchArgs;
  static __device__ __forceinline__ void run(const Args& a, const uint32_t bx, const uint32_t nbx) {
    GridView src = a.src, tgt = a.tgt; const GicpState* __restrict__ st = a.st; const double thr2 = a.thr2; float r0 = a.r0; const int max_rounds = a.max_rounds;
    int32_t* __restrict__ corr = a.corr; float* __restrict__ sqd = a.sqd; int32_t* __restrict__ nn_idx = a.nn_idx; float4* __restrict__ nn_ref = a.nn_ref;
    uint2* __restrict__ fb_list = a.fb_list; uint32_t* __restrict__ fb_count = a.fb_count; uint2* __restrict__ big_list = a.big_list; uint32_t* __restrict__ big_count = a.big_count;
    const int big_blocks = a.big_blocks; const float big_ratio = a.big_ratio; uint32_t* __restrict__ far_stats = a.far_stats; const NnOpt opt = a.opt;

  __shared__ WaveLds lds[BLOCK / 64];
  if (MODE == 0 && uni(st->phase) != 0) return;
  if (MODE == 1 && uni(st->phase) != 2) return;
  if (opt.cond && !(uni(st->reserved) & opt.cond)) return;
  src = grid_resolve(src); tgt = grid_resolve(tgt); if (r0 < 0.f) r0 = -r0 * tgt.cell;
  __shared__ float sTf[12];
  if (threadIdx.x < 12) sTf[threadIdx.x] = (float)st->x0[threadIdx.x];
  __syncthreads();
  if (LIST && (int)bx >= (int)nbx - big_blocks) {
    const uint32_t nbig = uni(*big_count);
    if (tgt.dbg && bx == nbx - 1 && threadIdx.x == 0) atomicAdd(&tgt.dbg[7], nbig);
    uint32_t nfar = 0;
    const uint32_t bw0 = (bx - (nbx - big_blocks)) * (BLOCK / 64) + (threadIdx.x >> 6), nbw = big_blocks * (BLOCK / 64);
    const uint32_t E = (GROUP && opt.group && nbig >= (uint32_t)opt.group_min) ? min(16u, (nbig + (uint32_t)opt.group - 1u) / (uint32_t)opt.group) : 1u;
    if (GROUP && E > 1u) {
      const int lane = threadIdx.x & 63, qs = lane & 15;
      WaveLds* wl = &lds[threadIdx.x >> 6];
      const float INF = __int_as_float(0x7f800000);
      for (uint32_t w0 = bw0 * E; w0 < nbig; w0 += nbw * E) {
        const uint32_t slot = w0 + (uint32_t)qs;
        const bool active = (uint32_t)qs < E && slot < nbig;
        const uint2 rec = active ? big_list[slot] : make_uint2(0u, 0u);
        const float4 p = active ? src.pts[rec.x] : make_float4(0.f, 0.f, 0.f, 0.f);
        float qx, qy, qz; { float Tf[12];
#pragma unroll
          for (int j = 0; j < 12; j++) Tf[j] = sTf[j];
          xform_query<MODE>(Tf, p.x, p.y, p.z, qx, qy, qz); }
        const float v = __uint_as_float(rec.y);
        const float r = v > 0.f ? v * 1.1f + 0.5f * tgt.cell : -v;
        const bool finite_q = (qx - qx == 0.f) && (qy - qy == 0.f) && (qz - qz == 0.f) && (r - r == 0.f);
        unsigned long long key = QN_INF_KEY; float second = INF, d_unseen = INF;
        unsigned long long todo = __ballot(active);
        while (todo) {
          const int al = __ffsll((long long)todo) - 1;
          const float ax = rdlane(qx, al), ay = rdlane(qy, al), az = rdlane(qz, al), ar = rdlane(r, al);
          const bool afin = rdlane((int)finite_q, al) != 0;
          const bool open_q = (todo >> lane) & 1ull;
          const bool member = open_q && (qs == (al & 15) || (afin && finite_q && sqdist(qx, qy, qz, ax, ay, az) <= 0.25f * ar * ar));
          const unsigned long long mm = __ballot(member);
          if (__popcll(mm) <= 4) {
            unsigned long long k1; float s1, du1;
            wave_search_single(tgt, ax, ay, az, ar, INF, k1, s1, du1, wl);
            if (member) { key = k1; second = s1; d_unseen = du1; }
          } else {
            wave_search_far16(tgt, qx, qy, qz, member, r, key, second, d_unseen, wl);
          }
          todo &= ~mm;
        }
        if (active && lane < 16) {
          const uint32_t tl = late(rec.x);
          store_nn<MODE>(key, late(__float_as_uint(p.w)), tl, thr2, corr, sqd, nn_idx);
          if (MODE == 0) nn_ref[tl] = make_float4(qx, qy, qz, key != QN_INF_KEY ? sqrtf(key_d2(key)) : INF);
        }
        if (far_stats && MODE == 0) {
          const unsigned long long fm = __ballot(active && lane < 16 && key != QN_INF_KEY && key_d2(key) > 36.f * tgt.cell * tgt.cell);
          if (lane == 0) nfar += (uint32_t)__popcll(fm);
        }
      }
      if (far_stats && MODE == 0 && (threadIdx.x & 63) == 0 && nfar) atomicAdd(&far_stats[3], nfar);
      return;
    }
    unsigned long long pr_sum = 0, pr_max = 0, pr_a = 0, pr_b = 0; uint32_t pr_n = 0;
    const uint32_t nfb_all = uni(*fb_count);
    const uint32_t nfb1 = (opt.fb_small && nfb_all <= opt.fb_small) ? nfb_all : 0u;
    for (uint32_t w = bw0; w < nbig + nfb1; w += nbw) {
      const uint2 rec = w < nbig ? big_list[w] : fb_list[w - nbig];
      const float4 p = src.pts[rec.x];
      float qx, qy, qz; { float Tf[12];
#pragma unroll
          for (int j = 0; j < 12; j++) Tf[j] = sTf[j];
          xform_query<MODE>(Tf, p.x, p.y, p.z, qx, qy, qz); }
      const float v = __uint_as_float(rec.y);
      const float r = v > 0.f ? v * 1.1f + 0.5f * tgt.cell : -v;
      unsigned long long key; float second, d_unseen;
      const unsigned long long pt0 = opt.probe ? wall_clock64() : 0ull;
      SingleStats sst;
      wave_search_single(tgt, qx, qy, qz, r, __int_as_float(0x7f800000), key, second, d_unseen, &lds[threadIdx.x >> 6], sst, opt.probe != nullptr);
      if (opt.probe) { const unsigned long long dt = wall_clock64() - pt0; pr_sum += dt; pr_n++;
        if (dt > pr_max) { pr_max = dt; pr_a = ((unsigned long long)sst.rounds << 48) | ((unsigned long long)min(sst.segs, 0xffffffu) << 24) | (unsigned long long)min(sst.cand, 0xffffffu);
          pr_b = ((unsigned long long)__float_as_uint(sst.r_first) << 32) | __float_as_uint(key != QN_INF_KEY ? sqrtf(key_d2(key)) : -1.f); } }
      if ((threadIdx.x & 63) == 0) {
        const uint32_t tl = late(rec.x);
        store_nn<MODE>(key, late(__float_as_uint(p.w)), tl, thr2, corr, sqd, nn_idx);
        if (MODE == 0) nn_ref[tl] = make_float4(qx, qy, qz, fminf(sqrtf(second), d_unseen));
        if (key != QN_INF_KEY && key_d2(key) > 36.f * tgt.cell * tgt.cell) nfar++;
      }
    }
    if (far_stats && MODE == 0 && (threadIdx.x & 63) == 0 && nfar) atomicAdd(&far_stats[3], nfar);
    if (opt.probe && (threadIdx.x & 63) == 0 && bw0 < 16384u) { opt.probe[4 * bw0] = (pr_max << 32) | pr_n; opt.probe[4 * bw0 + 1] = pr_sum; opt.probe[4 * bw0 + 2] = pr_a; opt.probe[4 * bw0 + 3] = pr_b; }
    return;
  }
  const uint32_t nq = LIST ? uni(*fb_count) : src.n;
  if (LIST && opt.fb_small && nq <= opt.fb_small) return;
  if (LIST && tgt.dbg && bx == 0 && threadIdx.x == 0) atomicAdd(&tgt.dbg[5], nq);
  const uint32_t wave0 = bx * (BLOCK / 64) + (threadIdx.x >> 6), nwaves = (nbx - (LIST ? big_blocks : 0)) * (BLOCK / 64);
  for (uint32_t base = wave0 * 16; base < nq; base += nwaves * 16) {
    const uint32_t slot = base + (threadIdx.x & 15);
    const bool active = slot < nq;
    uint32_t t = slot; float r = r0, r_cap = __int_as_float(0x7f800000);
    if (LIST && active) {
      const uint2 rec = fb_list[slot]; t = rec.x;
      const float v = __uint_as_float(rec.y);
      if (v < 0.f) r = -v; else { r_cap = v; r = fminf(v, r0); }
    }
    const float4 p = active ? src.pts[t] : make_float4(0, 0, 0, 0);
    float qx, qy, qz; { float Tf[12];
#pragma unroll
          for (int j = 0; j < 12; j++) Tf[j] = sTf[j];
          xform_query<MODE>(Tf, p.x, p.y, p.z, qx, qy, qz); }
    Best1 sink; sink.init();
    float d_unseen;
    const bool cert = wave_search<4>(tgt, qx, qy, qz, active, r, r_cap, max_rounds, sink, &lds[threadIdx.x >> 6], d_unseen);
    const bool mine = active && (threadIdx.x & 48) == 0;
    const bool done = cert || LIST;
    if (!LIST && MODE == 0 && opt.clear_ref && mine) opt.clear_ref[t] = make_float4(0.f, 0.f, 0.f, 0.f);
    if (mine && done) {
      const uint32_t tl = late(t);
      store_nn<MODE>(sink.key, late(__float_as_uint(p.w)), tl, thr2, corr, sqd, nn_idx);
      if (MODE == 0) nn_ref[tl] = make_float4(qx, qy, qz, fminf(sqrtf(sink.second), d_unseen));
    }
    if (!LIST) {
      const float rn = r;
      const bool far = rn > big_ratio * r0;
      wave_append(big_list, big_count, mine && !done && far, make_uint2(t, __float_as_uint(-rn)));
      wave_append(fb_list, fb_count, mine && !done && !far, make_uint2(t, __float_as_uint(-rn)));
    }
  }
  }
};
template <int MODE, bool LIST, int BLOCK, bool GROUP = false>
// ... 546 lines not shown
```

fast-lio-sam-qn_amd/csrc/qn_search_debug.hip:

```cpp
#include <hip/hip_runtime.h>
#include <stdint.h>
#include "qn_ball_walk.cuh"

namespace qn {

#define QN_DS_INF __int_as_float(0x7f800000)
__device__ __forceinline__ float dsf(uint32_t w) { return __uint_as_float(w); }
__device__ __forceinline__ uint32_t dsu(float f) { return __float_as_uint(f); }

static __global__ void __launch_bounds__(256) k_dbg_dump(GridView g0, uint32_t ncells, uint32_t npts, uint32_t* __restrict__ out) {
  const uint32_t i = blockIdx.x * 256u + threadIdx.x;
  if (i <= ncells) out[i] = g0.cell_start[i];
  if (i < npts) { const float4 p = g0.pts[i]; uint32_t* o = out + (ncells + 1) + 4 * (size_t)i; o[0] = dsu(p.x); o[1] = dsu(p.y); o[2] = dsu(p.z); o[3] = dsu(p.w); }
}

static __global__ void __launch_bounds__(64) k_dbg_best1(const uint32_t* __restrict__ in, int L, int unique, int S, uint32_t* __restrict__ out) {
  const int lane = threadIdx.x;
  const uint32_t* w = in + (size_t)blockIdx.x * ((size_t)L * 192 + 64);
  Best1 s; s.init();
  for (int e = 0; e < L; e++) {
    const uint32_t* r = w + ((size_t)e * 64 + lane) * 3;
    if (unique) s.consider<true>(r[0] != 0u, dsf(r[1]), r[2]); else s.consider<false>(r[0] != 0u, dsf(r[1]), r[2]);
  }
  const bool on = w[(size_t)L * 192 + lane] != 0u;
// ... 162 lines not shown
  lane_ball_knn<KMAX>(g, dsf(r[0]), dsf(r[1]), dsf(r[2]), dsf(r[3]), sink);
  if (qi >= n) return;
  uint32_t* o = out + (size_t)qi * (size_t)(2 * k + 4);
  store_bestk<KMAX>(sink, o);
  o[2 * k] = (uint32_t)sink.found(); o[2 * k + 1] = 0u; o[2 * k + 2] = 0u; o[2 * k + 3] = 0u;
}

template <int S>
static __global__ void __launch_bounds__(64) k_dbg_stream_clusters(GridView g0, const uint32_t* __restrict__ in, uint32_t cap, uint32_t* __restrict__ out) {
  __shared__ WaveLds lds;
  const GridView g = grid_resolve(g0);
  const int lane = threadIdx.x;
  const uint32_t* r = in + ((size_t)blockIdx.x * 64 + lane) * 8;
  uint32_t* hdr = out + (size_t)blockIdx.x * (8 + 64 * (4 + 2 * (size_t)cap));
  uint32_t* o = hdr + 8 + (size_t)lane * (4 + 2 * (size_t)cap);
  const float qx = dsf(r[0]), qy = dsf(r[1]), qz = dsf(r[2]), rad = dsf(r[3]);
  const unsigned long long todo = __ballot(r[4] != 0u);
  const bool mine = (todo >> lane) & 1ull;
  const int cx = cell_coord(qx, g.ox, g.inv_cell, g.nx), cy = cell_coord(qy, g.oy, g.inv_cell, g.ny), cz = cell_coord(qz, g.oz, g.inv_cell, g.nz);
  uint32_t cid; int ncl; uint32_t nseg_all;
  build_clusters<S>(g, &lds, todo, cx, cy, cz, qx, qy, qz, rad, cid, ncl, nseg_all);
  const uint32_t tmode = mine ? lds.cl_tile_mode[cid & 63u] : 0u;
  uint32_t n1 = 0, n2 = 0, over = 0;
  const uint32_t ret1 = stream_clusters<S>(g, &lds, ncl, nseg_all, [&](const float4& cp, bool in_tile, uint32_t ccid) __attribute__((always_inline)) {
    if (mine && in_tile && ccid == cid) { if (n1 < cap) o[4 + n1] = dsu(cp.w); else over = 1u; n1++; }
  });
  const uint32_t ret2 = stream_clusters<S, true>(g, &lds, ncl, nseg_all, [&](const float4& cp, bool in_tile, uint32_t ccid) __attribute__((always_inline)) {
    if (mine && in_tile && ccid == cid) { if (n2 < cap) o[4 + cap + n2] = dsu(cp.w); else over = 1u; n2++; }
  }, ret1);
  o[0] = cid; o[1] = tmode; o[2] = n1; o[3] = n2;
  const bool any_over = __any(over != 0u);
  if (lane == 0) { hdr[0] = (uint32_t)ncl; hdr[1] = nseg_all; hdr[2] = ret1; hdr[3] = ret2; hdr[4] = any_over ? 1u : 0u; hdr[5] = 0u; hdr[6] = 0u; hdr[7] = 0u; }
}

template <int VARIANT>
static __global__ void __launch_bounds__(64) k_dbg_ball_cells(GridView g0, const uint32_t* __restrict__ in, uint32_t n, uint32_t cap, uint32_t* __restrict__ out) {
  constexpr int FG = VARIANT == 0 ? 1 : (VARIANT == 3 ? 16 : 8);
  __shared__ uint2 seg_tab[VARIANT == 0 ? 1 : 64 / FG][QN_SEG_CAP];
  const GridView g = grid_resolve(g0);
  const uint32_t lane_all = blockIdx.x * 64u + threadIdx.x;
  const uint32_t qi = lane_all / FG;
  const int gl = (int)(threadIdx.x % FG);
  const bool have = qi < n;
  const uint32_t* r = in + 8 * (size_t)(have ? qi : 0u);
  const bool on = have && r[4] != 0u;
  uint32_t* o = out + (size_t)lane_all * (2 + (size_t)cap);
  uint32_t cnt = 0, over = 0;
  auto body = [&](uint32_t u, float4) __attribute__((always_inline)) { if (cnt < cap) o[2 + cnt] = u; else over = 1u; cnt++; };
  const float qx = dsf(r[0]), qy = dsf(r[1]), qz = dsf(r[2]), rad = dsf(r[3]);
  if (VARIANT == 0) { if (on) for_each_in_ball_cells(g, qx, qy, qz, rad, body); }
  else if (VARIANT == 1) { if (on) for_each_in_ball_cells_group<8>(g, qx, qy, qz, rad, gl, body); }
  else for_each_in_ball_cells_group_pre<FG>(g, on, qx, qy, qz, rad, gl, seg_tab[VARIANT == 0 ? 0 : threadIdx.x / FG], body);
  o[0] = cnt; o[1] = over;
}

#define QN_DS_BY_KMAX(KM, CALL) do { if ((KM) == 16) { CALL(16); } else if ((KM) == 20) { CALL(20); } else if ((KM) == 24) { CALL(24); } else { CALL(32); } } while (0)

hipError_t debug_launch_search(int which, const GridView& g, uint32_t ncells, const uint32_t* in, uint32_t n, uint32_t arg, uint32_t* out, hipStream_t stream) {
  switch (which) {
    case 0: { const uint32_t m = (ncells + 1 > n ? ncells + 1 : n); hipLaunchKernelGGL(k_dbg_dump, dim3((m + 255) / 256), dim3(256), 0, stream, g, ncells, n, out); break; }
    case 1: hipLaunchKernelGGL(k_dbg_best1, dim3(n), dim3(64), 0, stream, in, (int)(arg >> 16), (int)((arg >> 8) & 1u), (int)(arg & 7u), out); break;
    case 2: hipLaunchKernelGGL(k_dbg_bounds, dim3((n + 63) / 64), dim3(64), 0, stream, g, in, n, out); break;
    case 3: hipLaunchKernelGGL(k_dbg_divmod, dim3(2048), dim3(256), 0, stream, reinterpret_cast<unsigned long long*>(out)); break;
    case 4: hipLaunchKernelGGL(k_dbg_stream_box, dim3(n), dim3(64), 0, stream, g, in, arg, out); break;
    case 5: hipLaunchKernelGGL(k_dbg_wave_search1, dim3((n + 15) / 16), dim3(64), 0, stream, g, in, n, (int)arg, out); break;
    case 6: hipLaunchKernelGGL(k_dbg_wave_search_single, dim3(n), dim3(64), 0, stream, g, in, out); break;
    case 7: hipLaunchKernelGGL(k_dbg_wave_search_far16, dim3(n / 16), dim3(64), 0, stream, g, in, out); break;
    case 8: {
      const int KM = (int)(arg & 63u), k = (int)((arg >> 8) & 63u), S = (int)((arg >> 14) & 7u), L = (int)(arg >> 17);
#define QN_DS_CALL(K_) hipLaunchKernelGGL(k_dbg_bestk<K_>, dim3(n), dim3(64), 0, stream, in, L, k, S, out)
      QN_DS_BY_KMAX(KM, QN_DS_CALL);
#undef QN_DS_CALL
      break; }
    case 9: {
      const int rounds = (int)(arg & 255u), KM = (int)((arg >> 8) & 63u), k = (int)((arg >> 16) & 63u);
#define QN_DS_CALL(K_) hipLaunchKernelGGL(k_dbg_wave_search_k<K_>, dim3((n + 15) / 16), dim3(64), 0, stream, g, in, n, rounds, k, out)
      QN_DS_BY_KMAX(KM, QN_DS_CALL);
#undef QN_DS_CALL
      break; }
    case 10: {
      const int KM = (int)(arg & 63u), k = (int)((arg >> 8) & 63u);
#define QN_DS_CALL(K_) hipLaunchKernelGGL(k_dbg_lane_ball_knn<K_>, dim3((n + 63) / 64), dim3(64), 0, stream, g, in, n, k, out)
      QN_DS_BY_KMAX(KM, QN_DS_CALL);
#undef QN_DS_CALL
      break; }
    case 11:
      if ((arg >> 24) == 1u) hipLaunchKernelGGL(k_dbg_stream_clusters<1>, dim3(n), dim3(64), 0, stream, g, in, arg & 0xffffffu, out);
      else hipLaunchKernelGGL(k_dbg_stream_clusters<4>, dim3(n), dim3(64), 0, stream, g, in, arg & 0xffffffu, out);
      break;
    default: {
      const uint32_t v = arg >> 24, cap = arg & 0xffffffu, fg = v == 0u ? 1u : (v == 3u ? 16u : 8u);
      const dim3 grid((unsigned)(((size_t)n * fg + 63) / 64));
      if (v == 0u) hipLaunchKernelGGL(k_dbg_ball_cells<0>, grid, dim3(64), 0, stream, g, in, n, cap, out);
      else if (v == 1u) hipLaunchKernelGGL(k_dbg_ball_cells<1>, grid, dim3(64), 0, stream, g, in, n, cap, out);
      else if (v == 2u) hipLaunchKernelGGL(k_dbg_ball_cells<2>, grid, dim3(64), 0, stream, g, in, n, cap, out);
      else hipLaunchKernelGGL(k_dbg_ball_cells<3>, grid, dim3(64), 0, stream, g, in, n, cap, out);
      break; }
  }
  return hipGetLastError();
}

}
```

fast-lio-sam-qn_amd/qn_amd/engine.py:

```python
import ctypes as C
import math
import os
import numpy as np
from . import build as _build

QN_OK, QN_ERR_INVALID_ARG, QN_ERR_EMPTY_CLOUD, QN_ERR_CAPACITY, QN_ERR_NOT_READY, QN_ERR_HIP, QN_ERR_NO_DEVICE, QN_ERR_INTERNAL = range(8)
QN_SOURCE, QN_TARGET = 0, 1
QN_VERIFY_SRC, QN_VERIFY_DST, QN_VERIFY_COARSE, QN_VERIFY_FINAL = 0, 1, 2, 3
FLOAT_MAX = 3.4028234663852886e38
KERNEL_FAMILIES = ["grid_build", "knn_cov", "nn_search", "nn_fallback", "accumulate", "solve", "fitness", "transform",
                   "fpfh_normals", "fpfh_spfh", "fpfh_fpfh", "feat_match", "gn_tick_fused", "knn_select", "match_tail", "far_refresh", "align_persist"]


class GicpParams(C.Structure):
    _fields_ = [("k_correspondences", C.c_int32), ("max_iterations", C.c_int32), ("max_corr_dist", C.c_double),
                ("transformation_epsilon", C.c_double), ("rotation_epsilon", C.c_double), ("optimizer", C.c_int32),
                ("lm_max_iterations", C.c_int32), ("lm_init_lambda_factor", C.c_double), ("force_iterations", C.c_int32),
                ("ransac_iterations", C.c_int32), ("ransac_outlier_threshold", C.c_double),
                ("euclidean_fitness_epsilon", C.c_double)]


class GicpResult(C.Structure):
    _fields_ = [("T", C.c_float * 16), ("T64", C.c_double * 16), ("H", C.c_double * 36), ("fitness", C.c_double),
                ("iterations", C.c_int32), ("converged", C.c_int32), ("lm_failed", C.c_int32), ("reserved", C.c_int32)]
# ... 86 lines not shown
    def debug_get(self, key):
        v = C.c_double()
        self.check(self._l.qn_debug_get(self.h, key.encode(), C.byref(v)))
        return v.value

    def debug_eig3(self, which, a6):
        a = np.ascontiguousarray(a6, dtype=np.float64).reshape(-1, 6)
        n = len(a)
        if n == 0:
            a = np.zeros((1, 6))
        w = np.zeros((max(n, 1), 3)); V = np.zeros((max(n, 1), 3, 3))
        self._l.qn_debug_eig3.argtypes = [C.c_void_p, C.c_int, C.c_void_p, C.c_uint32, C.c_void_p, C.c_void_p]
        self.check(self._l.qn_debug_eig3(self.h, C.c_int(which), _p(a), C.c_uint32(n), _p(w), _p(V)))
        return w[:n], V[:n]

    STEP_MATH_STRIDES = ((43, 7), (43, 6), (59, 39), (3, 9), (9, 9), (18, 3))

    def debug_step_math(self, which, records):
        if not 0 <= which < len(self.STEP_MATH_STRIDES):
            raise ValueError("debug_step_math: which = %r" % (which,))
        si, so = self.STEP_MATH_STRIDES[which]
        a = np.ascontiguousarray(records, dtype=np.float64).reshape(-1, si)
        n = len(a)
        if n == 0:
            a = np.zeros((1, si))
        out = np.zeros((max(n, 1), so))
        self._l.qn_debug_step_math.argtypes = [C.c_void_p, C.c_int, C.c_void_p, C.c_uint32, C.c_void_p]
        self.check(self._l.qn_debug_step_math(self.h, C.c_int(which), _p(a), C.c_uint32(n), _p(out)))
        return out[:n]

    LIN_POINT, LIN_EMIT, LIN_ROWS = 0, 1, 2
    LIN_POINT_STRIDE, LIN_HEAD, LIN_LANE, LIN_BLOCK, LIN_NPART = 37, 25, 13, 256, 28

    def debug_linearize(self, which, data, arg=0):
        if which == self.LIN_POINT:
            si, shape = self.LIN_POINT_STRIDE, lambda n: (n, self.LIN_NPART)
        elif which == self.LIN_EMIT:
            if arg not in (1, 2, 3, 4):
                raise ValueError("debug_linearize: %r trips" % (arg,))
            si, shape = self.LIN_HEAD + arg * self.LIN_BLOCK * self.LIN_LANE, lambda n: (n, 5, self.LIN_NPART)
        elif which == self.LIN_ROWS:
            si, shape = self.LIN_NPART, lambda n: (min(n, 1) * self.LIN_NPART,)
        else:
            raise ValueError("debug_linearize: which = %r" % (which,))
        a = np.ascontiguousarray(data, dtype=np.float64).reshape(-1, si)
        n = len(a)
        if n == 0:
            a = np.zeros((1, si))
        out = np.zeros(max(int(np.prod(shape(n))), 1))
        self._l.qn_debug_linearize.argtypes = [C.c_void_p, C.c_int, C.c_void_p, C.c_uint32, C.c_uint32, C.c_void_p]
        self.check(self._l.qn_debug_linearize(self.h, C.c_int(which), _p(a), C.c_uint32(n), C.c_uint32(arg), _p(out)))
        return out[:int(np.prod(shape(n)))].reshape(shape(n))

    DS_DUMP, DS_BEST1, DS_BOUNDS, DS_DIVMOD, DS_STREAM_BOX, DS_WAVE_SEARCH1, DS_WAVE_SEARCH_SINGLE, DS_WAVE_SEARCH_FAR16, DS_BESTK, DS_WAVE_SEARCH_K, DS_LANE_BALL_KNN, DS_STREAM_CLUSTERS, DS_BALL_CELLS = range(13)

    def debug_search(self, which, grid, words, n, arg, n_out):
        a = np.ascontiguousarray(words, dtype=np.uint32).reshape(-1)
        if a.size == 0:
            a = np.zeros(1, dtype=np.uint32)
        out = np.zeros(max(int(n_out), 1), dtype=np.uint32)
        self._l.qn_debug_search.argtypes = [C.c_void_p, C.c_int, C.c_int, C.c_void_p, C.c_uint32, C.c_uint32, C.c_void_p]
        self.check(self._l.qn_debug_search(self.h, C.c_int(which), C.c_int(grid), _p(a), C.c_uint32(n), C.c_uint32(arg), _p(out)))
        return out[:int(n_out)]

    def grid_info(self, which):
        out = np.zeros(8)
        self.check(self._l.qn_debug_get_grid(self.h, C.c_int(which), _p(out)))
        return dict(origin=out[:3], cell=out[3], dims=out[4:7].astype(int), eps=out[7])

    def prof_enable(self, on=True):
        self.check(self._l.qn_prof_enable(self.h, C.c_int(1 if on else 0)))

    def prof_reset(self):
        self.check(self._l.qn_prof_reset(self.h))

    def prof_stats(self):
        out = {}
        for i, name in enumerate(KERNEL_FAMILIES):
            ks = KernelStat()
            self.check(self._l.qn_prof_get(self.h, C.c_int(i), C.byref(ks)))
            out[name] = (ks.total_ms, ks.launches)
        return out


def _cloud_arg(xyz):
    a = np.ascontiguousarray(xyz, dtype=np.float32)
    if a.ndim != 2 or a.shape[1] < 3:
        raise ValueError("cloud must be (n, >=3) float32")
    return a, a.shape[0], a.shape[1] * 4


class NanoGICP:

    def __init__(self, ctx):
        self.ctx = ctx
        self._l = ctx._l
        self.p = GicpParams()
        self._l.qn_gicp_default_params(C.byref(self.p))
        self._res = None
        self._n = [0, 0]
        self._push()

    def _push(self):
        self.ctx.check(self._l.qn_gicp_set_params(self.ctx.h, C.byref(self.p)))

    def bind(self):
        self._push()
# ... 1507 lines not shown
```

include/qn_engine.h:

```cpp
#ifndef QN_ENGINE_H
#define QN_ENGINE_H

#include <stdint.h>

#ifdef __cplusplus
extern "C" {
#endif

typedef struct qn_ctx qn_ctx;

enum {
  QN_OK = 0,
  QN_ERR_INVALID_ARG = 1,
  QN_ERR_EMPTY_CLOUD = 2,
  QN_ERR_CAPACITY = 3,
  QN_ERR_NOT_READY = 4,
  QN_ERR_HIP = 5,
  QN_ERR_NO_DEVICE = 6,
  QN_ERR_INTERNAL = 7
};

enum { QN_SOURCE = 0, QN_TARGET = 1 };
enum { QN_OPT_LM = 0, QN_OPT_GN = 1 };

// ... 357 lines not shown
} qn_sim_prim;
typedef struct {
  uint32_t n_beams, n_cols;
  const double *cos_el, *sin_el;
  const double *cos_az, *sin_az;
  double min_range, max_range, sigma;
} qn_sim_sensor;
int  qn_sim_lidar_to_store(qn_kf_store*, const qn_sim_prim* prims, uint32_t n_prims, const qn_sim_sensor* sensor, const double* poses16,
                           const uint32_t* seeds, uint32_t n_scans, int32_t* ids_out, uint32_t* n_out);

#define QN_SC_MAX_RINGS 64u
#define QN_SC_MAX_SECTORS 360u
#define QN_SC_MAX_BINS 8192u
#define QN_SC_MAX_PREFILTER 1024u
#define QN_SC_MAX_TOP_K 1024u
#define QN_SC_MAX_RESULTS (1u << 26)
typedef struct {
  uint32_t n_rings;
  uint32_t n_sectors;
  double max_radius;
  double lidar_height;
  uint32_t ringkey_prefilter;
  uint32_t pad_;
} qn_sc_params;
int  qn_kf_sc_set_params(qn_kf_store*, const qn_sc_params* p);
int  qn_kf_sc_get_params(qn_kf_store*, qn_sc_params* p);
int  qn_kf_sc_describe(qn_kf_store*, const int32_t* ids, uint32_t count);
int  qn_kf_sc_get(qn_kf_store*, int32_t id, float* desc , double* ringkey , double* colnorm );
int  qn_kf_sc_query(qn_kf_store*, const int32_t* query_ids, uint32_t nq, const double* stamps, uint32_t n_stamps, double tdiff, uint32_t top_k,
                    int32_t* ids_out, double* dist_out, int32_t* shift_out, uint32_t* n_out);

int  qn_gicp_get_covariances(qn_ctx*, int which, double* cov9_out);
int  qn_gicp_knn(qn_ctx*, int which, int k, int32_t* idx_out, float* d2_out);
int  qn_gicp_linearize(qn_ctx*, const double T[16], double H[36], double b[6], double* err,
                       int32_t* corr_out, float* sqd_out);
int  qn_gicp_compute_error(qn_ctx*, const double T[16], double* err);

int  qn_prof_enable(qn_ctx*, int on);
int  qn_prof_reset(qn_ctx*);
int  qn_prof_get(qn_ctx*, int kernel_family, qn_kernel_stat* out);
int  qn_debug_set(qn_ctx*, const char* key, double value);
int  qn_debug_get_counters(qn_ctx*, uint32_t out[16]);
int  qn_debug_selftest(qn_ctx*, uint32_t n_waves, uint32_t seed, uint32_t* mismatches);
#define QN_DEBUG_EIG3_MAX (1u << 24)
int  qn_debug_eig3(qn_ctx*, int which, const double* a6, uint32_t n, double* w_out, double* v_out);
#define QN_DEBUG_STEP_MATH_WHICH 6
#define QN_DEBUG_STEP_MATH_MAX (1u << 20)
int  qn_debug_step_math(qn_ctx*, int which, const double* in, uint32_t n, double* out);
#define QN_DEBUG_LINEARIZE_WHICH 3
#define QN_DEBUG_LINEARIZE_MAX_POINTS (1u << 20)
#define QN_DEBUG_LINEARIZE_MAX_BLOCKS (1u << 11)
#define QN_DEBUG_LINEARIZE_MAX_ROWS (1u << 16)
int  qn_debug_linearize(qn_ctx*, int which, const double* in, uint32_t n, uint32_t arg, double* out);
#define QN_DEBUG_SEARCH_WHICH 13
#define QN_DS_DUMP 0
#define QN_DS_BEST1 1
#define QN_DS_BOUNDS 2
#define QN_DS_DIVMOD 3
#define QN_DS_STREAM_BOX 4
#define QN_DS_WAVE_SEARCH1 5
#define QN_DS_WAVE_SEARCH_SINGLE 6
#define QN_DS_WAVE_SEARCH_FAR16 7
#define QN_DS_BESTK 8
#define QN_DS_WAVE_SEARCH_K 9
#define QN_DS_LANE_BALL_KNN 10
#define QN_DS_STREAM_CLUSTERS 11
#define QN_DS_BALL_CELLS 12
#define QN_DEBUG_SEARCH_MAX_WAVES (1u << 12)
#define QN_DEBUG_SEARCH_MAX_QUERIES (1u << 16)
#define QN_DEBUG_SEARCH_MAX_STEPS 64u
#define QN_DEBUG_SEARCH_MAX_RECORDED (1u << 16)
#define QN_DEBUG_SEARCH_MAX_WORDS (1u << 26)
int  qn_debug_search(qn_ctx*, int which, int grid, const void* in, uint32_t n, uint32_t arg, void* out);
#define QN_DEBUG_MAP_PRIMS_WHICH 8
#define QN_DEBUG_MAP_PRIMS_MAX_BLOCKS (1u << 16)
#define QN_DEBUG_MAP_PRIMS_MAX_NODES (1u << 20)
#define QN_DEBUG_MAP_PRIMS_MAX_EDGES (1u << 20)
int  qn_kf_debug_map_prims(qn_kf_store*, int which, const void* in, uint32_t n, uint32_t arg, void* out);
int  qn_debug_get(qn_ctx*, const char* key, double* value);
int  qn_debug_get_grid(qn_ctx*, int which, double out[8]);
int  qn_debug_get_partials(qn_ctx*, double* out, uint32_t* rows_per_buffer, double* state);
int  qn_debug_get_list_probe(qn_ctx*, unsigned long long* out );
int  qn_debug_get_persist_clk(qn_ctx*, unsigned long long* out );
int  qn_debug_get_clk(qn_ctx*, unsigned long long* out , uint32_t* n);

#ifdef __cplusplus
}
#endif
#endif
```

Measured before the change: 4564.

## Prune far NN search with per-tile point bounding boxes and banded two-stage scan

While building the target grid, the code now computes a tight per-tile axis-aligned bounding box of the actual points, using wave reductions and float atomics in the stable-cells and scan kernels. The far-search paths (wave_search_single and far16) use these boxes to get tighter tile distance bounds. They scan tiles in two stages: first the tiles within a band of the nearest one, then only the tiles that can still beat the current best. Skipped tiles feed into the unseen-distance bound. The goal is fewer candidate points visited per query, at the cost of extra grid-build work, atomics, extra wave reductions and a more complex search loop.

```diff
diff --git a/fast-lio-sam-qn_amd/csrc/qn_batch.inc b/fast-lio-sam-qn_amd/csrc/qn_batch.inc
--- a/fast-lio-sam-qn_amd/csrc/qn_batch.inc
+++ b/fast-lio-sam-qn_amd/csrc/qn_batch.inc
@@ -129,7 +129,7 @@
     l->cell_override = c->cell_override; l->margin_nn = c->margin_nn; l->margin_nn_t0 = c->margin_nn_t0; l->margin_knn = c->margin_knn; l->big_blocks0 = c->big_blocks0; l->fb_blocks0 = c->fb_blocks0;
     l->big_ratio = c->big_ratio; l->nn_rounds = c->nn_rounds; l->knn_rounds = c->knn_rounds; l->knn_trips = c->knn_trips; l->knn_mm = c->knn_mm; l->knn_single_all = c->knn_single_all; l->bbox_blocks = c->bbox_blocks; l->stable_cells = c->stable_cells;
     l->unseeded_cap = c->unseeded_cap; l->track_from_tick = c->track_from_tick; l->fused_from_tick = c->fused_from_tick; l->ticks_per_chunk = c->ticks_per_chunk; l->far_chunk = c->far_chunk; l->far_group = c->far_group; l->far_ranked = c->far_ranked;
-    l->list_small = c->list_small; l->tick_ppt_min = c->tick_ppt_min; l->tick_rpb = c->tick_rpb; l->nn_lane = c->nn_lane;
+    l->list_small = c->list_small; l->tick_ppt_min = c->tick_ppt_min; l->tick_rpb = c->tick_rpb; l->nn_lane = c->nn_lane; l->far_tight = c->far_tight; l->far_band = c->far_band;
   }
   return QN_OK;
 }
@@ -250,7 +250,9 @@
           qn_ctx* c = R.c;
           const int t = tick_no - R.chunk_start;
           c->count_far_now = R.first_chunk && (t / per_outer == (R.chunk - 1) / per_outer);
+          c->prune_far_now = per_outer == 1 && tick_no + 1 < R.next && tick_no + 1 < c->unseeded_until;
           const NnLaunch N = prep_nn(c, 0, c->sqd, false, tick_no / per_outer, 0);
+          c->prune_far_now = false;
           group = group && N.group; lane = lane && N.lane;
           lane_push(v_g, N.grid, N.grid_nb); lane_push(v_l, N.list, N.list_nb);
           const uint32_t nb = acc_blocks(c);
diff --git a/fast-lio-sam-qn_amd/csrc/qn_context.h b/fast-lio-sam-qn_amd/csrc/qn_context.h
--- a/fast-lio-sam-qn_amd/csrc/qn_context.h
+++ b/fast-lio-sam-qn_amd/csrc/qn_context.h
@@ -13,6 +13,7 @@
   uint32_t* cell_of_pt = nullptr;
   uint32_t* cell_start = nullptr;
   uint32_t* counts = nullptr;
+  float* tile_box = nullptr;
   double* nrm = nullptr;
   qn::GridView grid{};
   qn::GridDims* dims = nullptr;
@@ -81,6 +82,7 @@
   int nn_lane = -1;
   int track_from_tick = 3;
   int fused_from_tick = 3;
+  int far_tight = 1; float far_band = 0.5f; bool prune_far_now = false;
   int unseeded_until = 3; bool count_far_now = false; int last_extra_unseeded = 0;
   int unseeded_cap = 10;
   int single_from_tick = 2;
diff --git a/fast-lio-sam-qn_amd/csrc/qn_device.cuh b/fast-lio-sam-qn_amd/csrc/qn_device.cuh
--- a/fast-lio-sam-qn_amd/csrc/qn_device.cuh
+++ b/fast-lio-sam-qn_amd/csrc/qn_device.cuh
@@ -21,6 +21,7 @@
   const float4* pts;
   const uint32_t* cell_start;
   uint32_t* dbg;
+  const float* tile_box;
   float ox, oy, oz, cell, inv_cell, eps;
   int nx, ny, nz;
   int ntx, nty, ntz;
@@ -354,6 +355,12 @@
   const float zl = g.oz + (float)(tz << 2) * g.cell, zh = g.oz + (float)min((tz << 2) + 4, g.nz) * g.cell;
   const float dx = fmaxf(fmaxf(xl - qx, qx - xh) - g.eps, 0.f), dy = fmaxf(fmaxf(yl - qy, qy - yh) - g.eps, 0.f), dz = fmaxf(fmaxf(zl - qz, qz - zh) - g.eps, 0.f);
   return ((dx * dx + dy * dy) + dz * dz) * 0.999998f;
+}
+__device__ __forceinline__ float tile_pts_d2(const GridView& g, uint32_t tile, float qx, float qy, float qz) {
+  const float2* __restrict__ b = reinterpret_cast<const float2*>(g.tile_box) + 3 * (size_t)tile;
+  const float2 b0 = b[0], b1 = b[1], b2 = b[2];
+  const float dx = fmaxf(fmaxf(b0.x - qx, qx - b1.y), 0.f), dy = fmaxf(fmaxf(b0.y - qy, qy - b2.x), 0.f), dz = fmaxf(fmaxf(b1.x - qz, qz - b2.y), 0.f);
+  return (dx * dx + dy * dy) + dz * dz;
 }
 
 __device__ __forceinline__ void divmod_small(int n, int d, int& q, int& r) {
@@ -380,7 +387,7 @@
         int qz_, ry_; divmod_small(r, ntyr, qz_, ry_);
         const int tzz = (z0 >> 2) + qz_, tyy = ty0 + ry_, txx = tx0 + t;
         const uint32_t tile = ((uint32_t)tzz * g.nty + tyy) * g.ntx + txx;
-        if (!(ball_r2 >= 0.f && tile_box_d2(g, txx, tyy, tzz, bqx, bqy, bqz) > ball_r2)) { s = g.cell_start[tile << 7]; len = g.cell_start[(tile + 1) << 7] - s; }
+        if (!(ball_r2 >= 0.f && (g.tile_box ? tile_pts_d2(g, tile, bqx, bqy, bqz) : tile_box_d2(g, txx, tyy, tzz, bqx, bqy, bqz)) > ball_r2)) { s = g.cell_start[tile << 7]; len = g.cell_start[(tile + 1) << 7] - s; }
       } else {
         int qz_, ry_; divmod_small(r, nyr, qz_, ry_);
         const int ry = y0 + ry_, rz = z0 + qz_, tx = tx0 + t;
@@ -599,9 +606,12 @@
 
 struct SingleStats { uint32_t rounds, cand, segs; float r_first, r_last; };
 __device__ __forceinline__ void wave_search_single(const GridView& g, float qx, float qy, float qz, float r, const float r_cap,
-                                                   unsigned long long& best_out, float& second_out, float& d_unseen, WaveLds* lds, SingleStats& st_out, const bool stats) {
+                                                   unsigned long long& best_out, float& second_out, float& d_unseen, WaveLds* lds, SingleStats& st_out, const bool stats,
+                                                   const bool prune = false, const float band = 0.f) {
   const int lane = threadIdx.x & 63;
   const float INF = __int_as_float(0x7f800000);
+  const bool tight = prune && g.tile_box != nullptr && (qx - qx == 0.f) && (qy - qy == 0.f) && (qz - qz == 0.f);
+  float skip2 = INF;
   const CapBox cap = cap_of(g, qx, qy, qz);
   if (cap.S > 0.f) r = fminf(fmaxf(r, sqrtf(cap.S) + g.cell), fmaxf(r_cap, r));
   if (stats) { st_out.rounds = 0; st_out.cand = 0; st_out.segs = 0; st_out.r_first = r; }
@@ -625,20 +635,22 @@
       nseg = ntr * ntyr * ((z1 >> 2) - (z0 >> 2) + 1);
     }
     const int nyr = y1 - y0 + 1;
-    if (!tile_mode || done2 < 0.f) { best = QN_INF_KEY; second = INF; done2 = -1.f; }
+    if (!tile_mode || done2 < 0.f) { best = QN_INF_KEY; second = INF; done2 = -1.f; skip2 = INF; }
     const float in2 = r * r * 1.000002f;
+    const bool two_stage = tile_mode && tight;
     for (int sb = 0; sb < nseg; sb += 64) {
       const int sidx = sb + lane;
-      uint32_t s = 0, len = 0;
+      uint32_t s = 0, len = 0, tile = 0; float tb2 = 0.f; bool cand = false;
       if (sidx < nseg) {
         int t, rr; divmod_small(sidx, ntr, rr, t);
         if (tile_mode) {
           int qz_, ry_; divmod_small(rr, ntyr, qz_, ry_);
           const int tzz = (z0 >> 2) + qz_, tyy = ty0 + ry_, txx = tx0 + t;
-          const uint32_t tile = ((uint32_t)tzz * g.nty + tyy) * g.ntx + txx;
-          const float tb2 = tile_box_d2(g, txx, tyy, tzz, qx, qy, qz);
+          tile = ((uint32_t)tzz * g.nty + tyy) * g.ntx + txx;
+          tb2 = tight ? tile_pts_d2(g, tile, qx, qy, qz) : tile_box_d2(g, txx, tyy, tzz, qx, qy, qz);
           const bool seen = tb2 <= done2 && txx >= ptx0 && txx <= ptx1 && tyy >= pty0 && tyy <= pty1 && tzz >= ptz0 && tzz <= ptz1;
-          if (!(tb2 > in2) && !seen) { s = g.cell_start[tile << 7]; len = g.cell_start[(tile + 1) << 7] - s; }
+          cand = !(tb2 > in2) && !seen;
+          if (cand && !tight) { s = g.cell_start[tile << 7]; len = g.cell_start[(tile + 1) << 7] - s; }
         } else {
           int qz_, ry_; divmod_small(rr, nyr, qz_, ry_);
           const int ry = y0 + ry_, rz = z0 + qz_, tx = tx0 + t;
@@ -646,6 +658,16 @@
           const uint32_t k0 = cell_key(g, xa, ry, rz);
           s = g.cell_start[k0]; len = g.cell_start[k0 + (xb - xa) + 1] - s;
         }
+      }
+#pragma nounroll
+      for (int stage = 0; stage < (two_stage ? 2 : 1); stage++) {
+      if (two_stage) {
+        const float b2 = key_d2(wave_min_u64(best));
+        bool take = cand && !(tb2 > b2);
+        if (stage == 0) { const float lim = sqrtf(wave_min_f(take ? tb2 : INF)) + band; take = take && tb2 <= lim * lim; }
+        else if (cand && !take) skip2 = fminf(skip2, tb2);
+        s = 0; len = 0;
+        if (take) { s = g.cell_start[tile << 7]; len = g.cell_start[(tile + 1) << 7] - s; cand = false; }
       }
       const uint32_t incl = wave_incl_scan_u32(len, lane);
       const uint32_t total = rdlane(incl, 63);
@@ -666,6 +688,7 @@
           else if (d2 < second) second = d2;
         }
       }
+      }
     }
     if (g.dbg && lane == 0) { atomicAdd(&g.dbg[10], 1u); atomicAdd(&g.dbg[12], (uint32_t)nseg); if (round == 0) atomicAdd(&g.dbg[13], 1u); }
     if (stats) { st_out.rounds++; st_out.segs += (uint32_t)nseg; st_out.r_last = r; }
@@ -685,7 +708,7 @@
     if (tile_mode && r == r && round <= 160) d = fminf(d, r * 0.999998f + g.eps);
     if (d == INF || !(r == r) || round > 160) { cert = true; d_unseen = INF; }
     else { d -= g.eps; d_unseen = d; cert = d > 0.f && b != QN_INF_KEY && key_d2(b) < d * d; }
-    if (cert) { best_out = b; second_out = c; return; }
+    if (cert) { best_out = b; second_out = c; if (tight) d_unseen = fminf(d_unseen, sqrtf(wave_min_f(skip2))); return; }
     r = (b != QN_INF_KEY) ? fmaxf(sqrtf(key_d2(b)) * 1.000001f + g.eps, r + g.eps) : (r > 6.f * g.cell ? r + (2.f + round) * g.cell : 2.f * r + g.cell);
     r = fminf(r, r_cap);
   }
@@ -698,7 +721,8 @@
 }
 
 __device__ __forceinline__ void wave_search_far16(const GridView& g, float qx_in, float qy_in, float qz_in, bool member_in, float r_in,
-                                                  unsigned long long& best_out, float& second_out, float& d_unseen_out, WaveLds* lds) {
+                                                  unsigned long long& best_out, float& second_out, float& d_unseen_out, WaveLds* lds,
+                                                  const bool prune = false, const float band = 0.f) {
   const int lane = threadIdx.x & 63;
   const float INF = __int_as_float(0x7f800000);
   const unsigned long long mm = __ballot(member_in) & 0xffffull;
@@ -725,6 +749,8 @@
   bool open = has_q;
   unsigned long long fin_b = QN_INF_KEY; float fin_s = INF, fin_d = INF;
   float done2 = -1.f; int ptx0 = 0, ptx1 = -1, pty0 = 0, pty1 = -1, ptz0 = 0, ptz1 = -1;
+  const bool tight = prune && g.tile_box != nullptr && (cqx - cqx == 0.f) && (cqy - cqy == 0.f) && (cqz - cqz == 0.f);
+  float skip2 = INF;
   for (int round = 0;; round++) {
     const float rx = cap_extent(g, cap, R, 0), ry = cap_extent(g, cap, R, 1), rz = cap_extent(g, cap, R, 2);
     int x0 = rfl(cell_coord(cqx - rx, g.ox, g.inv_cell, g.nx)), x1 = rfl(cell_coord(cqx + rx, g.ox, g.inv_cell, g.nx));
@@ -739,16 +765,29 @@
     bool left_out = false;
     for (int sb = 0; sb < nseg; sb += 64) {
       const int sidx = sb + lane;
-      uint32_t s = 0, len = 0;
+      uint32_t s = 0, len = 0, tile = 0; float tb2 = 0.f; bool cand = false;
       if (sidx < nseg) {
         int t, rr; divmod_small(sidx, ntr, rr, t);
         int qz_, ry_; divmod_small(rr, ntyr, qz_, ry_);
         const int tzz = tz0 + qz_, tyy = ty0 + ry_, txx = tx0 + t;
-        const uint32_t tile = ((uint32_t)tzz * g.nty + tyy) * g.ntx + txx;
-        const float tb2 = tile_box_d2(g, txx, tyy, tzz, cqx, cqy, cqz);
+        tile = ((uint32_t)tzz * g.nty + tyy) * g.ntx + txx;
+        tb2 = tight ? tile_pts_d2(g, tile, cqx, cqy, cqz) : tile_box_d2(g, txx, tyy, tzz, cqx, cqy, cqz);
         const bool seen = tb2 <= done2 && txx >= ptx0 && txx <= ptx1 && tyy >= pty0 && tyy <= pty1 && tzz >= ptz0 && tzz <= ptz1;
-        if (tb2 > in2) left_out = true;
-        else if (!seen) { s = g.cell_start[tile << 7]; len = g.cell_start[(tile + 1) << 7] - s; }
+        if (tb2 > in2) { if (!tight || tb2 < INF) left_out = true; }
+        else if (!seen) { cand = true; if (!tight) { s = g.cell_start[tile << 7]; len = g.cell_start[(tile + 1) << 7] - s; } }
+      }
+#pragma nounroll
+      for (int stage = 0; stage < (tight ? 2 : 1); stage++) {
+      if (tight) {
+        float bd2 = sink.key != QN_INF_KEY ? key_d2(sink.key) : INF;
+        for (int o = m2; o < 64; o <<= 1) bd2 = fminf(bd2, __shfl_xor(bd2, o));
+        const float thr = wave_max_f(open ? sqrtf(bd2) * 1.000002f + 2.f * g.eps + off * 1.000002f : 0.f);
+        const float thr2 = thr * thr * 1.000002f;
+        bool take = cand && !(tb2 > thr2);
+        if (stage == 0) { const float lim = sqrtf(wave_min_f(take ? tb2 : INF)) + band; take = take && tb2 <= lim * lim; }
+        else if (cand && !take) skip2 = fminf(skip2, tb2);
+        s = 0; len = 0;
+        if (take) { s = g.cell_start[tile << 7]; len = g.cell_start[(tile + 1) << 7] - s; cand = false; }
       }
       const uint32_t incl = wave_incl_scan_u32(len, lane);
       const uint32_t total = rdlane(incl, 63);
@@ -772,6 +811,7 @@
           for (int u = 0; u < 4; u++) sink.consider(open && ci[u] < cnt, sqdist(qx, qy, qz, cp[u].x, cp[u].y, cp[u].z), __float_as_uint(cp[u].w));
         }
       }
+      }
     }
     if (g.dbg && lane == 0) { atomicAdd(&g.dbg[10], 1u); atomicAdd(&g.dbg[12], (uint32_t)nseg); if (round == 0) atomicAdd(&g.dbg[13], 1u); }
     done2 = in2; ptx0 = tx0; ptx1 = tx0 + ntr - 1; pty0 = ty0; pty1 = ty0 + ntyr - 1; ptz0 = tz0; ptz1 = z1 >> 2;
@@ -795,6 +835,7 @@
     const float grown = want > 0.f ? want : (R > 6.f * g.cell ? R + (2.f + round) * g.cell : 2.f * R + g.cell);
     R = fmaxf(grown, R * 1.0001f + g.eps);
   }
+  if (tight) fin_d = fminf(fin_d, fmaxf(sqrtf(wave_min_f(skip2)) * 0.999998f - off - g.eps, 0.f));
   const unsigned long long ob = __shfl(fin_b, my_rank & 63); const float os = __shfl(fin_s, my_rank & 63), od = __shfl(fin_d, my_rank & 63);
   if (member_in) { best_out = ob; second_out = os; d_unseen_out = od; }
 }
diff --git a/fast-lio-sam-qn_amd/csrc/qn_engine.hip b/fast-lio-sam-qn_amd/csrc/qn_engine.hip
--- a/fast-lio-sam-qn_amd/csrc/qn_engine.hip
+++ b/fast-lio-sam-qn_amd/csrc/qn_engine.hip
@@ -78,7 +78,7 @@
     off = a + bytes;
   }
 };
-static void carve_cloud(qn_ctx* c, Slab& sl, CloudBuf& b) {
+static void carve_cloud(qn_ctx* c, Slab& sl, CloudBuf& b, bool tile_boxes) {
   sl.take(b.raw, sizeof(float4) * c->max_points);
   sl.take(b.sorted, sizeof(float4) * c->max_points);
   sl.take(b.sorted_tmp, sizeof(float4) * c->max_points);
@@ -87,6 +87,7 @@
   sl.take(b.counts, sizeof(uint32_t) * ((size_t)c->max_cells + 1));
   sl.take(b.nrm, sizeof(double) * 3 * c->max_points);
   sl.take(b.dims, sizeof(GridDims));
+  if (tile_boxes) sl.take(b.tile_box, sizeof(float) * 6 * ((size_t)c->max_cells / QN_TILE_CELLS));
 }
 
 static int ctx_create(int device, uint32_t max_points, hipStream_t shared_stream, qn_ctx** out);
@@ -109,8 +110,8 @@
   else if (hipStreamCreateWithFlags(&c->stream, hipStreamNonBlocking) != hipSuccess) return fail(QN_ERR_HIP);
 #define CA(call) if ((call) != hipSuccess) return fail(QN_ERR_HIP)
   auto carve = [&](Slab& sl) {
-    carve_cloud(c, sl, c->cloud[0]);
-    carve_cloud(c, sl, c->cloud[1]);
+    carve_cloud(c, sl, c->cloud[0], false);
+    carve_cloud(c, sl, c->cloud[1], true);
     sl.take(c->staging, (size_t)max_points * 32);
     sl.take(c->scan_sums, sizeof(uint32_t) * (c->max_cells / (QN_BLOCK * QN_SCAN_ITEMS) + 2));
     sl.take(c->state, 2 * sizeof(GicpState));
@@ -280,6 +281,8 @@
   GridView& g = b.grid;
   memset(&g, 0, sizeof(g));
   g.pts = b.sorted; g.cell_start = b.cell_start; g.dbg = c->dbg_counters; g.n = n; g.dims = b.dims;
+  float* const tbox = (c->stable_cells && c->far_tight != 0) ? b.tile_box : nullptr;
+  g.tile_box = tbox;
   GridLaunch L;
   L.nb = (n + QN_BLOCK - 1) / QN_BLOCK;
   L.scan_nb = (c->max_cells + QN_BLOCK * QN_SCAN_ITEMS - 1) / (QN_BLOCK * QN_SCAN_ITEMS);
@@ -287,10 +290,10 @@
   L.pack_nb = std::min<uint32_t>(L.nb, (uint32_t)std::min(lanes ? QN_BBOX_MAX_BLOCKS : c->bbox_blocks, QN_BBOX_MAX_BLOCKS));
   L.pack = PackBBoxK::Args{dsrc, stride, n, b.raw, c->bbox_acc, c->max_cells, c->cell_override, b.dims, b.dims_host};
   L.count = CellCountK::Args{b.raw, n, g, b.counts, b.cell_of_pt};
-  L.scan = ScanLookbackK::Args{b.counts, b.dims, b.cell_start, c->scan_status, c->build_epoch, n};
+  L.scan = ScanLookbackK::Args{b.counts, b.dims, b.cell_start, c->scan_status, c->build_epoch, n, tbox};
   L.stable = c->stable_cells;
   L.scat = ScatterK::Args{b.raw, n, b.cell_of_pt, b.cell_start, b.counts, L.stable ? b.sorted_tmp : b.sorted};
-  L.stab = StableCellsK::Args{b.sorted_tmp, n, b.cell_of_pt, b.cell_start, b.sorted};
+  L.stab = StableCellsK::Args{b.sorted_tmp, n, b.cell_of_pt, b.cell_start, b.sorted, tbox};
   b.has_grid = true; b.has_cov = false; b.knn_tab = nullptr;
   return L;
 }
@@ -300,9 +303,9 @@
   { ProfScope ps(c, QN_K_GRID_BUILD);
     hipLaunchKernelGGL(k_pack_bbox_dims, dim3(L.pack_nb), dim3(QN_BLOCK), 0, s, L.pack.in, L.pack.stride, L.pack.n, L.pack.raw, L.pack.acc, L.pack.max_cells, L.pack.cell_override, L.pack.dims_dev, L.pack.dims_host);
     hipLaunchKernelGGL(k_cell_count, dim3(L.nb), dim3(QN_BLOCK), 0, s, L.count.pts, L.count.n, L.count.g, L.count.counts, L.count.cell_of_pt);
-    hipLaunchKernelGGL(k_scan_lookback, dim3(L.scan_nb), dim3(QN_BLOCK), 0, s, L.scan.in, L.scan.dims, L.scan.out, L.scan.status, L.scan.epoch, L.scan.total);
+    hipLaunchKernelGGL(k_scan_lookback, dim3(L.scan_nb), dim3(QN_BLOCK), 0, s, L.scan.in, L.scan.dims, L.scan.out, L.scan.status, L.scan.epoch, L.scan.total, L.scan.tile_box);
     hipLaunchKernelGGL(k_scatter, dim3(L.nb), dim3(QN_BLOCK), 0, s, L.scat.pts, L.scat.n, L.scat.cell_of_pt, L.scat.cell_start, L.scat.counts, L.scat.sorted);
-    if (L.stable) hipLaunchKernelGGL(k_stable_cells, dim3(L.nb), dim3(QN_BLOCK), 0, s, L.stab.in, L.stab.n, L.stab.cell_of_pt, L.stab.cell_start, L.stab.out); }
+    if (L.stable) hipLaunchKernelGGL(k_stable_cells, dim3(L.nb), dim3(QN_BLOCK), 0, s, L.stab.in, L.stab.n, L.stab.cell_of_pt, L.stab.cell_start, L.stab.out, L.stab.tile_box); }
   HIPCHK(c, hipGetLastError());
   return QN_OK;
 }
@@ -454,7 +457,8 @@
   if (mode == 0 && opt.group > 0) big_blocks = std::min(big_blocks, std::max(64, (opt.group + QN_BLOCK / 64 - 1) / (QN_BLOCK / 64)));
   opt.probe = (mode == 0 && !seeded) ? c->list_probe : nullptr;
   opt.fb_small = (mode == 0 && !c->persist_batch_off) ? (uint32_t)c->list_small : 0u;
-  NnOpt opt0; opt0.clear_ref = nullptr; opt0.cond = 0; opt0.group = 0; opt0.group_min = 0; opt0.probe = nullptr; opt0.fb_small = 0;
+  opt.prune = (mode == 0 && !seeded && T.grid.tile_box && (c->far_tight >= 2 || (c->far_tight == 1 && c->prune_far_now))) ? 1 : 0; opt.band = c->far_band;
+  NnOpt opt0; opt0.clear_ref = nullptr; opt0.cond = 0; opt0.group = 0; opt0.group_min = 0; opt0.probe = nullptr; opt0.fb_small = 0; opt0.prune = 0; opt0.band = 0.f;
   c->clear_far_now = mode == 0 && !seeded ? false : c->clear_far_now;
   const NnOpt& o = mode == 0 ? opt : opt0;
   NnLaunch L;
@@ -714,9 +718,10 @@
     }
     for (int t = 0; t < chunk; t++) {
       c->count_far_now = first_chunk && (t / per_outer == (chunk - 1) / per_outer);
+      c->prune_far_now = per_outer == 1 && t + 1 < chunk && tick_no + 1 < c->unseeded_until;
       enqueue_tick(c, seeded, tick_no, (dev_look && t == chunk - 1) ? &la : nullptr); tick_no++; seeded = true;
     }
-    c->count_far_now = false;
+    c->count_far_now = false; c->prune_far_now = false;
     bool declined = false;
     if (dev_look) {
       c->unseeded_until = tick_no + 1;
@@ -1119,6 +1124,8 @@
   else if (k == "knn_rounds") c->knn_rounds = v < 1 ? 1 : (int)v;
   else if (k == "knn_trips") c->knn_trips = v < 1 ? 1 : (int)v;
   else if (k == "knn_mm") c->knn_mm = v != 0;
+  else if (k == "far_tight") { c->far_tight = v < 0 ? 0 : (v > 2 ? 2 : (int)v); c->cloud[1].has_grid = false; }
+  else if (k == "far_band") c->far_band = v < 0 ? 0.f : (float)v;
   else if (k == "fused_ticks") c->fused_ticks = v != 0;
   else if (k == "big_ratio") c->big_ratio = (float)v;
   else if (k == "margin_nn_cap") c->margin_nn_cap = (int)v;
@@ -1298,6 +1305,14 @@
         if (r[0] >= (uint32_t)d.ntx || r[1] >= (uint32_t)d.nty || r[2] >= (uint32_t)d.ntz || !finite_rec(r, 3, 8) || !(ds_f(r[6]) > 0.f)) return QN_ERR_INVALID_ARG;
       }
       w_in = 8 * (size_t)n; w_out = 16 * (size_t)n; break;
+    case QN_DS_TILE_PTS:
+      if (n == 0 || n > QN_DEBUG_SEARCH_MAX_QUERIES || arg != 0) return QN_ERR_INVALID_ARG;
+      if (!g.tile_box) return QN_ERR_NOT_READY;
+      for (uint32_t i = 0; i < n; i++) {
+        const uint32_t* r = in + 8 * (size_t)i;
+        if (r[0] >= (uint32_t)d.ntx || r[1] >= (uint32_t)d.nty || r[2] >= (uint32_t)d.ntz || !finite_rec(r, 3, 6)) return QN_ERR_INVALID_ARG;
+      }
+      w_in = 8 * (size_t)n; w_out = 8 * (size_t)n; break;
     case QN_DS_DIVMOD:
       if (n != 0 || arg != 0) return QN_ERR_INVALID_ARG;
       w_in = 0; w_out = 6; break;
diff --git a/fast-lio-sam-qn_amd/csrc/qn_gicp_kernels.cuh b/fast-lio-sam-qn_amd/csrc/qn_gicp_kernels.cuh
--- a/fast-lio-sam-qn_amd/csrc/qn_gicp_kernels.cuh
+++ b/fast-lio-sam-qn_amd/csrc/qn_gicp_kernels.cuh
@@ -146,7 +146,7 @@
 #define QN_LB_STATE_INC 2ull
 struct ScanLookbackK {
   static constexpr int TB = QN_BLOCK, OCC = 1;
-  struct Args { const uint32_t* in; const GridDims* dims; uint32_t* out; unsigned long long* status; uint32_t epoch, total; };
+  struct Args { const uint32_t* in; const GridDims* dims; uint32_t* out; unsigned long long* status; uint32_t epoch, total; float* tile_box; };
   static __device__ __forceinline__ void run(const Args& a, const uint32_t bx, const uint32_t) {
     __shared__ uint32_t wsum[QN_BLOCK / 64];
     __shared__ uint32_t s_prefix;
@@ -156,6 +156,11 @@
     const uint32_t tile = bx;
     if (tile * (uint32_t)(QN_BLOCK * QN_SCAN_ITEMS) >= m) return;
     const uint32_t base = (tile * QN_BLOCK + threadIdx.x) * QN_SCAN_ITEMS;
+    if (a.tile_box && base < m && (base & (QN_TILE_CELLS - 1u)) == 0u) {
+      float* b = a.tile_box + 6 * (size_t)(base / QN_TILE_CELLS);
+      const float inf = __int_as_float(0x7f800000);
+      b[0] = inf; b[1] = inf; b[2] = inf; b[3] = -inf; b[4] = -inf; b[5] = -inf;
+    }
     uint32_t v[QN_SCAN_ITEMS], s = 0;
     if (base + QN_SCAN_ITEMS <= m) {
       const uint4* q = (const uint4*)(in + base);
@@ -216,8 +221,8 @@
   }
 };
 static __global__ void __launch_bounds__(QN_BLOCK) k_scan_lookback(const uint32_t* __restrict__ in, const GridDims* __restrict__ dims, uint32_t* __restrict__ out,
-                                                                   unsigned long long* status, uint32_t epoch, uint32_t total) {
-  const ScanLookbackK::Args a{in, dims, out, status, epoch, total};
+                                                                   unsigned long long* status, uint32_t epoch, uint32_t total, float* __restrict__ tile_box) {
+  const ScanLookbackK::Args a{in, dims, out, status, epoch, total, tile_box};
   ScanLookbackK::run(a, blockIdx.x, gridDim.x);
 }
 
@@ -240,15 +245,33 @@
   ScatterK::run(a, blockIdx.x, gridDim.x);
 }
 
+__device__ __forceinline__ void atomic_min_f32(float* a, float v) { if (__float_as_int(v) >= 0) atomicMin(reinterpret_cast<int*>(a), __float_as_int(v)); else atomicMax(reinterpret_cast<unsigned int*>(a), __float_as_uint(v)); }
+__device__ __forceinline__ void atomic_max_f32(float* a, float v) { if (__float_as_int(v) >= 0) atomicMax(reinterpret_cast<int*>(a), __float_as_int(v)); else atomicMin(reinterpret_cast<unsigned int*>(a), __float_as_uint(v)); }
 struct StableCellsK {
   static constexpr int TB = QN_BLOCK, OCC = 1;
-  struct Args { const float4* in; uint32_t n; const uint32_t* cell_of_pt; const uint32_t* cell_start; float4* out; };
+  struct Args { const float4* in; uint32_t n; const uint32_t* cell_of_pt; const uint32_t* cell_start; float4* out; float* tile_box; };
   static __device__ __forceinline__ void run(const Args& a, const uint32_t bx, const uint32_t) {
     const float4* __restrict__ in = a.in; float4* __restrict__ out = a.out;
     const uint32_t t = bx * QN_BLOCK + threadIdx.x;
-    if (t >= a.n) return;
-    const float4 p = in[t];
-    const uint32_t i = __float_as_uint(p.w), c = a.cell_of_pt[i];
+    const bool have = t < a.n;
+    const float4 p = have ? in[t] : make_float4(0.f, 0.f, 0.f, 0.f);
+    const uint32_t i = __float_as_uint(p.w), c = have ? a.cell_of_pt[i] : 0u;
+    if (a.tile_box) {
+      const float INF = __int_as_float(0x7f800000);
+      const uint32_t tile = c >> 7;
+      for (unsigned long long todo = __ballot(have); todo != 0;) {
+        const uint32_t lt = rdlane(tile, __ffsll((long long)todo) - 1);
+        const bool in_t = have && tile == lt;
+        const float lx = wave_min_f(in_t ? p.x : INF), ly = wave_min_f(in_t ? p.y : INF), lz = wave_min_f(in_t ? p.z : INF);
+        const float hx = wave_max_f(in_t ? p.x : -INF), hy = wave_max_f(in_t ? p.y : -INF), hz = wave_max_f(in_t ? p.z : -INF);
+        if ((threadIdx.x & 63) == 0) {
+          float* b = a.tile_box + 6 * (size_t)lt;
+          atomic_min_f32(b, lx); atomic_min_f32(b + 1, ly); atomic_min_f32(b + 2, lz); atomic_max_f32(b + 3, hx); atomic_max_f32(b + 4, hy); atomic_max_f32(b + 5, hz);
+        }
+        todo &= ~__ballot(in_t);
+      }
+    }
+    if (!have) return;
     const uint32_t s = a.cell_start[c], e = a.cell_start[c + 1];
     if (e - s > 256u) { out[t] = p; return; }
     uint32_t rank = 0;
@@ -257,8 +280,8 @@
   }
 };
 static __global__ void __launch_bounds__(QN_BLOCK) k_stable_cells(const float4* __restrict__ in, uint32_t n, const uint32_t* __restrict__ cell_of_pt, const uint32_t* __restrict__ cell_start,
-                                      float4* __restrict__ out) {
-  const StableCellsK::Args a{in, n, cell_of_pt, cell_start, out};
+                                      float4* __restrict__ out, float* __restrict__ tile_box) {
+  const StableCellsK::Args a{in, n, cell_of_pt, cell_start, out, tile_box};
   StableCellsK::run(a, blockIdx.x, gridDim.x);
 }
 
@@ -468,7 +491,7 @@
   }
 }
 
-struct NnOpt { float4* clear_ref; int cond; int group, group_min; unsigned long long* probe; uint32_t fb_small; };
+struct NnOpt { float4* clear_ref; int cond; int group, group_min; unsigned long long* probe; uint32_t fb_small; int prune; float band; };
 struct NnSearchArgs { GridView src, tgt; const GicpState* st; double thr2; float r0; int max_rounds; int32_t* corr; float* sqd; int32_t* nn_idx; float4* nn_ref;
                       uint2* fb_list; uint32_t* fb_count; uint2* big_list; uint32_t* big_count; int big_blocks; float big_ratio; uint32_t* far_stats; NnOpt opt; };
 template <int MODE, bool LIST, int BLOCK, bool GROUP = false>
@@ -522,10 +545,11 @@
           const unsigned long long mm = __ballot(member);
           if (__popcll(mm) <= 4) {
             unsigned long long k1; float s1, du1;
-            wave_search_single(tgt, ax, ay, az, ar, INF, k1, s1, du1, wl);
+            SingleStats none;
+            wave_search_single(tgt, ax, ay, az, ar, INF, k1, s1, du1, wl, none, false, opt.prune != 0, opt.band * tgt.cell);
             if (member) { key = k1; second = s1; d_unseen = du1; }
           } else {
-            wave_search_far16(tgt, qx, qy, qz, member, r, key, second, d_unseen, wl);
+            wave_search_far16(tgt, qx, qy, qz, member, r, key, second, d_unseen, wl, opt.prune != 0, opt.band * tgt.cell);
           }
           todo &= ~mm;
         }
@@ -557,7 +581,7 @@
       unsigned long long key; float second, d_unseen;
       const unsigned long long pt0 = opt.probe ? wall_clock64() : 0ull;
       SingleStats sst;
-      wave_search_single(tgt, qx, qy, qz, r, __int_as_float(0x7f800000), key, second, d_unseen, &lds[threadIdx.x >> 6], sst, opt.probe != nullptr);
+      wave_search_single(tgt, qx, qy, qz, r, __int_as_float(0x7f800000), key, second, d_unseen, &lds[threadIdx.x >> 6], sst, opt.probe != nullptr, opt.prune != 0, opt.band * tgt.cell);
       if (opt.probe) { const unsigned long long dt = wall_clock64() - pt0; pr_sum += dt; pr_n++;
         if (dt > pr_max) { pr_max = dt; pr_a = ((unsigned long long)sst.rounds << 48) | ((unsigned long long)min(sst.segs, 0xffffffu) << 24) | (unsigned long long)min(sst.cand, 0xffffffu);
           pr_b = ((unsigned long long)__float_as_uint(sst.r_first) << 32) | __float_as_uint(key != QN_INF_KEY ? sqrtf(key_d2(key)) : -1.f); } }
diff --git a/fast-lio-sam-qn_amd/csrc/qn_search_debug.hip b/fast-lio-sam-qn_amd/csrc/qn_search_debug.hip
--- a/fast-lio-sam-qn_amd/csrc/qn_search_debug.hip
+++ b/fast-lio-sam-qn_amd/csrc/qn_search_debug.hip
@@ -238,6 +238,18 @@
   else if (VARIANT == 1) { if (on) for_each_in_ball_cells_group<8>(g, qx, qy, qz, rad, gl, body); }
   else for_each_in_ball_cells_group_pre<FG>(g, on, qx, qy, qz, rad, gl, seg_tab[VARIANT == 0 ? 0 : threadIdx.x / FG], body);
   o[0] = cnt; o[1] = over;
+}
+
+static __global__ void __launch_bounds__(64) k_dbg_tile_pts(GridView g0, const uint32_t* __restrict__ in, uint32_t n, uint32_t* __restrict__ out) {
+  const GridView g = grid_resolve(g0);
+  const uint32_t i = blockIdx.x * 64u + threadIdx.x;
+  if (i >= n) return;
+  const uint32_t* r = in + 8 * (size_t)i;
+  uint32_t* o = out + 8 * (size_t)i;
+  const uint32_t tile = (r[2] * (uint32_t)g.nty + r[1]) * (uint32_t)g.ntx + r[0];
+  o[0] = dsu(tile_pts_d2(g, tile, dsf(r[3]), dsf(r[4]), dsf(r[5])));
+  for (int j = 0; j < 6; j++) o[1 + j] = dsu(g.tile_box[6 * (size_t)tile + j]);
+  o[7] = 0u;
 }
 
 #define QN_DS_BY_KMAX(KM, CALL) do { if ((KM) == 16) { CALL(16); } else if ((KM) == 20) { CALL(20); } else if ((KM) == 24) { CALL(24); } else { CALL(32); } } while (0)
@@ -274,6 +286,7 @@
       if ((arg >> 24) == 1u) hipLaunchKernelGGL(k_dbg_stream_clusters<1>, dim3(n), dim3(64), 0, stream, g, in, arg & 0xffffffu, out);
       else hipLaunchKernelGGL(k_dbg_stream_clusters<4>, dim3(n), dim3(64), 0, stream, g, in, arg & 0xffffffu, out);
       break;
+    case 13: hipLaunchKernelGGL(k_dbg_tile_pts, dim3((n + 63) / 64), dim3(64), 0, stream, g, in, n, out); break;
     default: {
       const uint32_t v = arg >> 24, cap = arg & 0xffffffu, fg = v == 0u ? 1u : (v == 3u ? 16u : 8u);
       const dim3 grid((unsigned)(((size_t)n * fg + 63) / 64));
diff --git a/fast-lio-sam-qn_amd/qn_amd/engine.py b/fast-lio-sam-qn_amd/qn_amd/engine.py
--- a/fast-lio-sam-qn_amd/qn_amd/engine.py
+++ b/fast-lio-sam-qn_amd/qn_amd/engine.py
@@ -162,7 +162,7 @@
         self.check(self._l.qn_debug_linearize(self.h, C.c_int(which), _p(a), C.c_uint32(n), C.c_uint32(arg), _p(out)))
         return out[:int(np.prod(shape(n)))].reshape(shape(n))
 
-    DS_DUMP, DS_BEST1, DS_BOUNDS, DS_DIVMOD, DS_STREAM_BOX, DS_WAVE_SEARCH1, DS_WAVE_SEARCH_SINGLE, DS_WAVE_SEARCH_FAR16, DS_BESTK, DS_WAVE_SEARCH_K, DS_LANE_BALL_KNN, DS_STREAM_CLUSTERS, DS_BALL_CELLS = range(13)
+    DS_DUMP, DS_BEST1, DS_BOUNDS, DS_DIVMOD, DS_STREAM_BOX, DS_WAVE_SEARCH1, DS_WAVE_SEARCH_SINGLE, DS_WAVE_SEARCH_FAR16, DS_BESTK, DS_WAVE_SEARCH_K, DS_LANE_BALL_KNN, DS_STREAM_CLUSTERS, DS_BALL_CELLS, DS_TILE_PTS = range(14)
 
     def debug_search(self, which, grid, words, n, arg, n_out):
         a = np.ascontiguousarray(words, dtype=np.uint32).reshape(-1)
diff --git a/include/qn_engine.h b/include/qn_engine.h
--- a/include/qn_engine.h
+++ b/include/qn_engine.h
@@ -433,7 +433,7 @@
 #define QN_DEBUG_LINEARIZE_MAX_BLOCKS (1u << 11)
 #define QN_DEBUG_LINEARIZE_MAX_ROWS (1u << 16)
 int  qn_debug_linearize(qn_ctx*, int which, const double* in, uint32_t n, uint32_t arg, double* out);
-#define QN_DEBUG_SEARCH_WHICH 13
+#define QN_DEBUG_SEARCH_WHICH 14
 #define QN_DS_DUMP 0
 #define QN_DS_BEST1 1
 #define QN_DS_BOUNDS 2
@@ -447,6 +447,7 @@
 #define QN_DS_LANE_BALL_KNN 10
 #define QN_DS_STREAM_CLUSTERS 11
 #define QN_DS_BALL_CELLS 12
+#define QN_DS_TILE_PTS 13
 #define QN_DEBUG_SEARCH_MAX_WAVES (1u << 12)
 #define QN_DEBUG_SEARCH_MAX_QUERIES (1u << 16)
 #define QN_DEBUG_SEARCH_MAX_STEPS 64u
```

Result: no change. 4565, median of 2 (+0.0%).
